# InternRobotics/InternNav

Hardware: NVIDIA H100
Metric: InternVLA-N1 policy-steps/sec (batch RGB-D+text->action) (higher is better)
Workload: dtype bf16

## Files before the change

### include/n1b200.h

```cpp
#ifndef N1B200_H_
#define N1B200_H_

#include <stddef.h>
#include <stdint.h>

#ifdef __cplusplus
extern "C" {
#endif

typedef struct n1_ctx* n1_handle;

enum {
  N1_OK = 0,
  N1_ERR_UNKNOWN = -1,
  N1_ERR_ARG = -2,
  N1_ERR_CUDA = -3,
  N1_ERR_NO_DEVICE = -4,
  N1_ERR_TMA = -5,
  N1_ERR_WEIGHT = -6,
  N1_ERR_WORKSPACE = -7,
  N1_ERR_KV_PAGES = -8
};

enum { N1_F32 = 0, N1_BF16 = 1 };

typedef struct {
  const char* name;
  const void* data;
  int32_t dtype;
  int32_t ndim;
  int64_t shape[4];
} n1_tensor_desc;

typedef struct {
  int32_t token_dim;
  int32_t heads;
  int32_t layers;
  int32_t predict_size;
  int32_t memory_size;
  int32_t vlm_token_dim;
  int32_t n_query;
} n1_s1_dims;

typedef struct {
  int32_t token_dim;
  int32_t heads;
  int32_t layers;
  int32_t predict_size;
  int32_t memory_size;
  int32_t depth_frames;
  int32_t goal_slots;
  int32_t ddpm_steps;
} n1_navdp_policy_dims;

const char* n1_version(void);
int n1_device_ok(int device);
int n1_create(n1_handle* out, int device);
void n1_destroy(n1_handle h);
const char* n1_last_error(void);

int n1_s1_load(n1_handle h, const n1_s1_dims* dims, const n1_tensor_desc* tensors, int n, void* stream);

enum { N1_OP_RGBD = 1, N1_OP_GOAL = 2, N1_OP_DENOISE = 3 };
size_t n1_workspace_bytes(n1_handle h, int op, int B, int Ns, int T);

int n1_rgbd_encode(n1_handle h, void* ws, size_t ws_bytes, const float* rgb, const float* depth, void* out_bf16, int B,
                   void* stream);

int n1_goal_compress(n1_handle h, void* ws, size_t ws_bytes, const void* latents_bf16, void* goal_bf16, int B,
                     void* stream);

int n1_navdp_eps(n1_handle h, void* ws, size_t ws_bytes, const float* x_t, const int32_t* timesteps, int t_scalar,
                 const void* goal_bf16, const void* rgbd_bf16, float* eps, int B, int Ns, int T, void* stream);

int n1_navdp_sample(n1_handle h, void* ws, size_t ws_bytes, const void* goal_bf16, const void* rgbd_bf16,
                    const float* x_init, const float* step_noise, float* traj_out, int B, int Ns, int T, int K,
                    void* stream);

int n1_navdp_policy_load(n1_handle h, const n1_navdp_policy_dims* dims, const n1_tensor_desc* tensors, int n, void* stream);
int n1_navdp_critic(n1_handle h, void* ws, size_t ws_bytes, const float* traj, const void* rgbd_bf16, float* critic, int B,
                    int Ns, int T, void* stream);
int n1_ddpm_tables(int K, float* out_host );

typedef struct {
  int32_t v_depth, v_hidden, v_heads, v_inter, v_patch, v_tpatch, v_merge, v_window, v_out;
  int32_t n_fullatt, fullatt[16];
  int32_t layers, hidden, heads, kv_heads, head_dim, inter, vocab;
  float rms_eps, rope_theta;
  int32_t mrope[3];
  int32_t n_query;
} n1_s2_dims;

typedef struct n1_vit_plan_s* n1_vit_plan;
typedef struct n1_llm_plan_s* n1_llm_plan;
typedef struct n1_kv_pool_s* n1_kv_pool;

int n1_s2_load(n1_handle h, const n1_s2_dims* dims, const n1_tensor_desc* tensors, int n, void* stream);
int n1_s2_has_latent_queries(n1_handle h);
int n1_s2_has_lm_head(n1_handle h);

int n1_vit_plan_create(n1_handle h, const int32_t* grid_thw_host, int n_img, n1_vit_plan* out, void* stream);
void n1_vit_plan_destroy(n1_vit_plan p);
int64_t n1_vit_plan_patches(n1_vit_plan p);
int n1_llm_plan_create(n1_handle h, const int32_t* input_ids_host, const int32_t* lens_host, int B,
                       const int32_t* grid_thw_host, int n_img, int max_new_tokens, n1_kv_pool pool,
                       const int32_t* reused_host, const int32_t* slots_host, n1_llm_plan* out, void* stream);
void n1_llm_plan_destroy(n1_llm_plan p);
int64_t n1_llm_plan_tokens(n1_llm_plan p);
int64_t n1_llm_plan_image_tokens(n1_llm_plan p);
int n1_llm_plan_positions(n1_llm_plan p, int32_t* pos3_host, int32_t* delta_host);

size_t n1_vit_workspace_bytes(n1_handle h, n1_vit_plan p);
size_t n1_llm_workspace_bytes(n1_handle h, n1_llm_plan p);

int n1_qwen_vit(n1_handle h, n1_vit_plan p, void* ws, size_t ws_bytes, const void* pixels_bf16, void* out_bf16,
                int64_t out_rows, const int32_t* dst_rows_host, int64_t n_rows, void* stream);
int n1_llm_prefill(n1_handle h, n1_llm_plan p, void* ws, size_t ws_bytes, const void* image_feats_bf16,
                   void* latents_bf16, void* stream);

int n1_llm_generate(n1_handle h, n1_llm_plan p, void* ws, size_t ws_bytes, const void* feats_bf16, int64_t feat_rows,
                    const int32_t* image_rows_host, int64_t n_rows, const int32_t* eos_ids_host, int n_eos, int32_t pad_id,
                    int32_t* tokens_host, int32_t* lens_host, void* latents_bf16, int32_t* passes_host, void* stream);

int n1_kv_pool_create(n1_handle h, int slots, int capacity, n1_kv_pool* out);
void n1_kv_pool_destroy(n1_kv_pool p);
size_t n1_kv_pool_bytes(n1_kv_pool p);
int n1_kv_pool_valid(n1_kv_pool p, int slot);
int n1_kv_pool_create_paged(n1_handle h, int slots, int pages, int max_tokens_per_slot, n1_kv_pool* out);
int n1_kv_pool_release(n1_kv_pool p, int slot);
int n1_kv_pool_free_pages(n1_kv_pool p);
int n1_kv_pool_slot_pages(n1_kv_pool p, int slot);
int n1_kv_pool_read(n1_kv_pool p, int layer, int slot, int row, int n, void* k_out, void* v_out, void* stream);
int n1_image_digest(const void* pixels_bf16, int64_t cols, const int64_t* row_off_dev, int n_img, uint64_t* digest_dev,
                    void* stream);

int n1_rope_index(const int32_t* input_ids_host, int len, const int32_t* grid_thw_host, int n_img, int merge,
                  int32_t* pos3_host , int32_t* delta_host);
int n1_plan_rows_host(const int32_t* input_ids_host, const int32_t* lens_host, int B, const int32_t* grid_thw_host,
                      int n_img, int merge, int vocab, int n_query, int max_new_tokens, int pool_slots, int pool_capacity,
                      const int32_t* reused_host, const int32_t* slots_host, int cap_rows, int32_t* n_rows,
                      int32_t* cu_host, int32_t* kind_host, int32_t* src_host, int32_t* dest_host, int32_t* k_len_host);
typedef struct n1_kv_pages_s* n1_kv_pages;
int n1_kv_pages_create(int slots, int max_tokens_per_slot, int pages, n1_kv_pages* out);
void n1_kv_pages_destroy(n1_kv_pages a);
int n1_kv_pages_prepare(n1_kv_pages a, int B, const int32_t* slots_host, const int32_t* keep_rows_host,
                        const int32_t* need_rows_host, int32_t* changed_host);
int n1_kv_pages_trim(n1_kv_pages a, int slot, int rows);
int n1_kv_pages_table(n1_kv_pages a, int32_t* table_host, int32_t* held_host, int32_t* free_host);
int n1_vit_window_index(const int32_t* grid_thw_host, int n_img, int merge, int window, int32_t* window_index_host,
                        int32_t* cu_window_host, int32_t* n_cu, int32_t* pos_hw_host );

typedef struct n1_resize_plan_s* n1_resize_plan;
int n1_resize_plan_create(int in_h, int in_w, int out_h, int out_w, n1_resize_plan* out, void* stream);
void n1_resize_plan_destroy(n1_resize_plan p);
size_t n1_resize_workspace_bytes(n1_resize_plan p, int n_frames, int is_float);
int n1_resize_rgb_u8(n1_resize_plan p, const void* src_u8, int n_frames, void* dst_f32, void* dst_u8, void* ws,
                     size_t ws_bytes, void* stream);
int n1_resize_f32(n1_resize_plan p, const void* src_f32, int n_frames, float mul, float clip_max, void* dst_f32,
                  void* ws, size_t ws_bytes, void* stream);
int n1_resize_coeffs(int in_size, int out_size, int capacity_k, int32_t* bounds_host, double* weights_host,
                     int32_t* fixed_host, int32_t* ksize);

typedef struct {
  const void* src_u8;
  int32_t h, w;
  int64_t row0;
} n1_vl_image;
size_t n1_vl_patchify_workspace_bytes(int n_img);
int n1_vl_patchify(const n1_vl_image* images_host, int n_img, const void* lut_bf16, void* out_bf16, int64_t n_rows,
                   void* ws, size_t ws_bytes, void* stream);

size_t n1_rgb_tokens_workspace_bytes(n1_handle h, int B);
int n1_rgb_tokens(n1_handle h, void* ws, size_t ws_bytes, const float* rgb, void* mem_bf16, int B, void* stream);
int n1_s2_set_latent_queries(n1_handle h, const void* latent_queries_bf16, void* stream);
size_t n1_s2_train_workspace_bytes(n1_handle h, n1_llm_plan plan);
int n1_s2_train_forward(n1_handle h, n1_llm_plan plan, void* ws, size_t ws_bytes, const void* image_feats_bf16,
                        void* states_bf16, void* stream);
int n1_s2_train_backward(n1_handle h, n1_llm_plan plan, void* ws, size_t ws_bytes, const void* grad_states_bf16,
                         void* grad_latent_queries_f32, void* stream);
int n1_op_transpose(const void* in_bf16, int rows, int cols, int ld_in, void* out_bf16, int ld_out, int rows_pad, void* stream);
int n1_op_colsum(const void* a_bf16, const void* b_bf16_or_null, int rows, int cols, int ld_a, int ld_b, void* out_f32,
                 int accumulate, void* stream);
int n1_op_norm_bwd(const void* dy_bf16, int ld_dy, const void* x_bf16, int ld_x, const void* w_f32, const void* residual_grad,
                   int ld_rg, void* dx_bf16, int ld_dx, void* dw_f32, void* db_f32, int rows, int D, float eps, int rms,
                   int accumulate, void* stream);
int n1_op_act_fwd(const void* pre_bf16, void* out_bf16, int64_t n, int act, void* stream);
int n1_op_act_bwd(const void* pre_bf16, const void* dy_bf16, void* out_bf16, int64_t n, int act, void* stream);
int n1_op_swiglu_bwd(const void* pre_bf16, const void* dact_bf16, void* dpre_bf16, int64_t rows, int inter, void* stream);
int n1_op_rope_transposed(void* x_bf16, int ld, const void* cos_sin_f32x2, int64_t rows, int heads, int head_dim, void* stream);
int n1_op_attention_bwd(const void* q, const void* k, const void* v, const void* o, const void* dout, void* dq, void* dk_f32,
                        void* dv_f32, int ldq, int ldk, int ldv, int ldo, int lddo, int lddq, int heads_q, int heads_kv,
                        int head_dim, int batch, int seq_q, int seq_k, const void* cu_q, const void* cu_k, int max_seq_q,
                        int kv_div, int causal, float scale, const void* k_len, int k_slot, void* stream);
int n1_traj_to_actions(const void* traj_f32, int B, int Ns, int T, double turn_angle_rad, double step_size, int lookahead,
                       int max_actions, int cap, int32_t* ids, int32_t* count, double* mean_path, void* stream);
int n1_traj_mean_path(const void* traj_f32, int B, int Ns, int T, double* mean_path, void* stream);
int n1_op_sgemm(const void* A_f32, int lda, int trans_a, const void* B_f32, int ldb, int trans_b, void* C_f32, int ldc, int M,
                int N, int K, int accumulate, void* stream);
size_t n1_op_wgrad_workspace_bytes(int M, int No, int Ko);
int n1_op_wgrad(const void* dy_bf16, int ld_dy, const void* x_bf16, int ld_x, int M, int No, int Ko, void* out_f32,
                int accumulate, void* ws, size_t ws_bytes, void* stream);
int n1_op_scale_cols(const void* x_bf16, int ld_x, const void* gamma_f32, const void* add_bf16_or_null, int ld_add,
                     void* out_bf16, int ld_out, int64_t rows, int cols, void* stream);
int n1_op_patchify_depth(const void* img_f32, void* out_bf16, int n_img, int ldk, void* stream);
int n1_op_adamw(void* master_f32, void* working_bf16_or_null, const void* grad_f32, void* m_f32, void* v_f32, int64_t n,
                float lr, float beta1, float beta2, float eps, float weight_decay, int step, void* stream);

void n1_prof_enable(int on);
void n1_prof_add(int64_t gemm_launches, int64_t total_launches);
int n1_prof_read(double* gemm_ms, double* gemm_flops, int64_t* gemm_launches, int64_t* total_launches);
int n1_prof_read_shapes(int32_t* mnk, int64_t* count, double* ms, int cap);

int n1_op_gemm(const void* A_bf16, int lda, const void* W_bf16, int ldw, void* out, int ldo, int M, int N, int K,
               const float* bias, const float* gamma, const void* residual_bf16, int ldr, int act, int out_fp32,
               void* stream);
int n1_op_ff_block(const void* x_bf16, int ldx, const float* ln_w, const float* ln_b, float eps, const void* w1_bf16,
                   const float* b1, const void* w2_bf16, const float* b2, void* out_bf16, int ldo, int M, void* stream);
int n1_op_dec_sa_block(void* x_bf16, int ldx, const float* ln_w, const float* ln_b, float eps, const void* w_qkv_bf16,
                       const float* b_qkv, const void* w_o_bf16, const float* b_o, int B, int Ns, int T, int causal,
                       void* stream);
int n1_op_dec_ca_block(void* x_bf16, int ldx, const float* ln_w, const float* ln_b, float eps, const void* w_q_bf16,
                       const float* b_q, const void* w_o_bf16, const float* b_o, const void* kv_bf16, int ldkv, int mtok,
                       int B, int Ns, int T, void* stream);
int n1_op_layernorm(const void* x_bf16, int ldx, void* y_bf16, int ldy, const float* w, const float* b, int rows, int D,
                    float eps, int rms, void* stream);
int n1_op_mod_norm(const void* x_bf16, int ldx, const float* w, const void* mod_bf16, int ld_mod, int rows_per_group,
                   const void* res_bf16, int ldr, void* out_bf16, int ldo, int64_t rows, int D, float eps, int mode,
                   void* stream);
int n1_op_add(const void* a_bf16, const void* b_bf16, void* out_bf16, int64_t n, void* stream);
int n1_op_action_embed(const float* lat, const float* w, const float* b, const float* pos, void* out_bf16, int64_t rows,
                       int T, int D, void* stream);
int n1_op_cfg_euler(const void* pred_bf16, int ld, int64_t n, int cfg, float scale, float dt, float* lat, void* stream);
int n1_op_attention(const void* q, const void* k, const void* v, void* o, int ldq, int ldk, int ldv, int ldo, int heads_q,
                    int heads_kv, int head_dim, int batch, int seq_q, int seq_k, const int32_t* cu_q,
                    const int32_t* cu_k, int max_seq_q, int kv_div, int causal, float scale, void* stream);

int n1_op_attention_ex(const void* q, const void* k, const void* v, void* o, int ldq, int ldk, int ldv, int ldo, int heads_q,
                       int heads_kv, int head_dim, int batch, const int32_t* cu_seqlens, int max_seq, int64_t total_rows,
                       int causal, float scale, int* used_tcgen05, void* stream);

int n1_op_attention_cache(const void* q, int ldq, int64_t q_rows, const void* k, const void* v, int ldkv, int64_t kv_rows,
                          void* o, int ldo, const int32_t* cu_q, const int32_t* ctx, const int32_t* row0, int batch,
                          int max_chunk, int heads_q, int heads_kv, float scale, void* stream);
int n1_op_attention_cache_paged(const void* q, int ldq, int64_t q_rows, const void* k, const void* v, int ldkv,
                                int64_t kv_rows, void* o, int ldo, const int32_t* cu_q, const int32_t* ctx,
                                const int32_t* row0, const int32_t* pages, int batch, int max_chunk, int heads_q,
                                int heads_kv, float scale, void* stream);

#ifdef __cplusplus
}
#endif
#endif
```

### internnav_b200/_lib.py

```python
import ctypes
import os
import threading

import torch

_HERE = os.path.dirname(os.path.abspath(__file__))
LIB_PATH = os.path.join(_HERE, "libn1b200.so")

_lib = None
_lock = threading.Lock()

c_void_p, c_int, c_size_t, c_float, c_char_p = (
    ctypes.c_void_p, ctypes.c_int, ctypes.c_size_t, ctypes.c_float, ctypes.c_char_p)
c_int32, c_int64, c_double = ctypes.c_int32, ctypes.c_int64, ctypes.c_double
i32p = ctypes.POINTER(c_int32)


class N1Error(RuntimeError):
    def __init__(self, code, msg):
        super().__init__("n1b200 error %d: %s" % (code, msg))
        self.code = code


class TensorDesc(ctypes.Structure):
    _fields_ = [("name", c_char_p), ("data", c_void_p), ("dtype", ctypes.c_int32), ("ndim", ctypes.c_int32),
                ("shape", ctypes.c_int64 * 4)]


class S1Dims(ctypes.Structure):
    _fields_ = [("token_dim", ctypes.c_int32), ("heads", ctypes.c_int32), ("layers", ctypes.c_int32),
                ("predict_size", ctypes.c_int32), ("memory_size", ctypes.c_int32),
                ("vlm_token_dim", ctypes.c_int32), ("n_query", ctypes.c_int32)]


class NavdpPolicyDims(ctypes.Structure):
    _fields_ = [(n, ctypes.c_int32) for n in ("token_dim", "heads", "layers", "predict_size", "memory_size", "depth_frames",
                                              "goal_slots", "ddpm_steps")]


class S2Dims(ctypes.Structure):
    _fields_ = [(n, ctypes.c_int32) for n in ("v_depth", "v_hidden", "v_heads", "v_inter", "v_patch", "v_tpatch",
                                              "v_merge", "v_window", "v_out", "n_fullatt")] + \
               [("fullatt", ctypes.c_int32 * 16)] + \
               [(n, ctypes.c_int32) for n in ("layers", "hidden", "heads", "kv_heads", "head_dim", "inter", "vocab")] + \
               [("rms_eps", ctypes.c_float), ("rope_theta", ctypes.c_float), ("mrope", ctypes.c_int32 * 3),
                ("n_query", ctypes.c_int32)]


class VlImage(ctypes.Structure):
    _fields_ = [("src_u8", c_void_p), ("h", ctypes.c_int32), ("w", ctypes.c_int32), ("row0", ctypes.c_int64)]


SYMBOLS = {
    "n1_version": (c_char_p, []),
    "n1_device_ok": (c_int, [c_int]),
    "n1_create": (c_int, [ctypes.POINTER(c_void_p), c_int]),
    "n1_destroy": (None, [c_void_p]),
    "n1_last_error": (c_char_p, []),
    "n1_s1_load": (c_int, [c_void_p, ctypes.POINTER(S1Dims), ctypes.POINTER(TensorDesc), c_int, c_void_p]),
    "n1_workspace_bytes": (c_size_t, [c_void_p, c_int, c_int, c_int, c_int]),
    "n1_rgbd_encode": (c_int, [c_void_p, c_void_p, c_size_t, c_void_p, c_void_p, c_void_p, c_int, c_void_p]),
    "n1_goal_compress": (c_int, [c_void_p, c_void_p, c_size_t, c_void_p, c_void_p, c_int, c_void_p]),
    "n1_navdp_eps": (c_int, [c_void_p, c_void_p, c_size_t, c_void_p, c_void_p, c_int, c_void_p, c_void_p, c_void_p,
                             c_int, c_int, c_int, c_void_p]),
    "n1_navdp_sample": (c_int, [c_void_p, c_void_p, c_size_t, c_void_p, c_void_p, c_void_p, c_void_p, c_void_p,
                                c_int, c_int, c_int, c_int, c_void_p]),
    "n1_navdp_policy_load": (c_int, [c_void_p, ctypes.POINTER(NavdpPolicyDims), ctypes.POINTER(TensorDesc), c_int,
                                     c_void_p]),
    "n1_navdp_critic": (c_int, [c_void_p, c_void_p, c_size_t, c_void_p, c_void_p, c_void_p, c_int, c_int, c_int, c_void_p]),
    "n1_ddpm_tables": (c_int, [c_int, ctypes.POINTER(c_float)]),
    "n1_s2_load": (c_int, [c_void_p, ctypes.POINTER(S2Dims), ctypes.POINTER(TensorDesc), c_int, c_void_p]),
    "n1_s2_has_latent_queries": (c_int, [c_void_p]),
    "n1_s2_has_lm_head": (c_int, [c_void_p]),
    "n1_vit_plan_create": (c_int, [c_void_p, i32p, c_int, ctypes.POINTER(c_void_p), c_void_p]),
    "n1_vit_plan_destroy": (None, [c_void_p]),
    "n1_vit_plan_patches": (c_int64, [c_void_p]),
    "n1_llm_plan_create": (c_int, [c_void_p, i32p, i32p, c_int, i32p, c_int, c_int, c_void_p, i32p, i32p,
                                   ctypes.POINTER(c_void_p), c_void_p]),
    "n1_llm_plan_destroy": (None, [c_void_p]),
    "n1_llm_plan_tokens": (c_int64, [c_void_p]),
    "n1_llm_plan_image_tokens": (c_int64, [c_void_p]),
    "n1_llm_plan_positions": (c_int, [c_void_p, i32p, i32p]),
    "n1_vit_workspace_bytes": (c_size_t, [c_void_p, c_void_p]),
    "n1_llm_workspace_bytes": (c_size_t, [c_void_p, c_void_p]),
    "n1_qwen_vit": (c_int, [c_void_p, c_void_p, c_void_p, c_size_t, c_void_p, c_void_p, c_int64, i32p, c_int64, c_void_p]),
    "n1_llm_prefill": (c_int, [c_void_p, c_void_p, c_void_p, c_size_t, c_void_p, c_void_p, c_void_p]),
    "n1_llm_generate": (c_int, [c_void_p, c_void_p, c_void_p, c_size_t, c_void_p, c_int64, i32p, c_int64, i32p, c_int,
                                c_int32, i32p, i32p, c_void_p, i32p, c_void_p]),
    "n1_kv_pool_create": (c_int, [c_void_p, c_int, c_int, ctypes.POINTER(c_void_p)]),
    "n1_kv_pool_destroy": (None, [c_void_p]),
    "n1_kv_pool_bytes": (c_size_t, [c_void_p]),
    "n1_kv_pool_valid": (c_int, [c_void_p, c_int]),
    "n1_kv_pool_read": (c_int, [c_void_p, c_int, c_int, c_int, c_int, c_void_p, c_void_p, c_void_p]),
    "n1_kv_pool_create_paged": (c_int, [c_void_p, c_int, c_int, c_int, ctypes.POINTER(c_void_p)]),
    "n1_kv_pool_release": (c_int, [c_void_p, c_int]),
    "n1_kv_pool_free_pages": (c_int, [c_void_p]),
    "n1_kv_pool_slot_pages": (c_int, [c_void_p, c_int]),
    "n1_kv_pages_create": (c_int, [c_int, c_int, c_int, ctypes.POINTER(c_void_p)]),
    "n1_kv_pages_destroy": (None, [c_void_p]),
    "n1_kv_pages_prepare": (c_int, [c_void_p, c_int, i32p, i32p, i32p, i32p]),
    "n1_kv_pages_trim": (c_int, [c_void_p, c_int, c_int]),
    "n1_kv_pages_table": (c_int, [c_void_p, i32p, i32p, i32p]),
    "n1_image_digest": (c_int, [c_void_p, c_int64, c_void_p, c_int, c_void_p, c_void_p]),
    "n1_rope_index": (c_int, [i32p, c_int, i32p, c_int, c_int, i32p, i32p]),
    "n1_plan_rows_host": (c_int, [i32p, i32p, c_int, i32p, c_int, c_int, c_int, c_int, c_int, c_int, c_int, i32p, i32p,
                                  c_int, i32p, i32p, i32p, i32p, i32p, i32p]),
    "n1_vit_window_index": (c_int, [i32p, c_int, c_int, c_int, i32p, i32p, i32p, i32p]),
    "n1_s2_set_latent_queries": (c_int, [c_void_p, c_void_p, c_void_p]),
    "n1_s2_train_workspace_bytes": (c_size_t, [c_void_p, c_void_p]),
    "n1_s2_train_forward": (c_int, [c_void_p, c_void_p, c_void_p, c_size_t, c_void_p, c_void_p, c_void_p]),
    "n1_s2_train_backward": (c_int, [c_void_p, c_void_p, c_void_p, c_size_t, c_void_p, c_void_p, c_void_p]),
    "n1_resize_plan_create": (c_int, [c_int, c_int, c_int, c_int, ctypes.POINTER(c_void_p), c_void_p]),
    "n1_resize_plan_destroy": (None, [c_void_p]),
    "n1_resize_workspace_bytes": (c_size_t, [c_void_p, c_int, c_int]),
    "n1_resize_rgb_u8": (c_int, [c_void_p, c_void_p, c_int, c_void_p, c_void_p, c_void_p, c_size_t, c_void_p]),
    "n1_resize_f32": (c_int, [c_void_p, c_void_p, c_int, c_float, c_float, c_void_p, c_void_p, c_size_t, c_void_p]),
    "n1_resize_coeffs": (c_int, [c_int, c_int, c_int, i32p, ctypes.POINTER(c_double), i32p, i32p]),
    "n1_vl_patchify_workspace_bytes": (c_size_t, [c_int]),
    "n1_vl_patchify": (c_int, [ctypes.POINTER(VlImage), c_int, c_void_p, c_void_p, c_int64, c_void_p, c_size_t, c_void_p]),
    "n1_op_transpose": (c_int, [c_void_p, c_int, c_int, c_int, c_void_p, c_int, c_int, c_void_p]),
    "n1_op_colsum": (c_int, [c_void_p, c_void_p, c_int, c_int, c_int, c_int, c_void_p, c_int, c_void_p]),
    "n1_op_norm_bwd": (c_int, [c_void_p, c_int, c_void_p, c_int, c_void_p, c_void_p, c_int, c_void_p, c_int, c_void_p,
                               c_void_p, c_int, c_int, c_float, c_int, c_int, c_void_p]),
    "n1_op_act_fwd": (c_int, [c_void_p, c_void_p, c_int64, c_int, c_void_p]),
    "n1_op_act_bwd": (c_int, [c_void_p, c_void_p, c_void_p, c_int64, c_int, c_void_p]),
    "n1_op_swiglu_bwd": (c_int, [c_void_p, c_void_p, c_void_p, c_int64, c_int, c_void_p]),
    "n1_op_rope_transposed": (c_int, [c_void_p, c_int, c_void_p, c_int64, c_int, c_int, c_void_p]),
    "n1_op_attention_bwd": (c_int, [c_void_p] * 8 + [c_int] * 12 + [c_void_p, c_void_p, c_int, c_int, c_int, c_float,
                                                                   c_void_p, c_int, c_void_p]),
    "n1_op_sgemm": (c_int, [c_void_p, c_int, c_int, c_void_p, c_int, c_int, c_void_p, c_int, c_int, c_int, c_int, c_int,
                            c_void_p]),
    "n1_op_wgrad_workspace_bytes": (c_size_t, [c_int, c_int, c_int]),
    "n1_op_wgrad": (c_int, [c_void_p, c_int, c_void_p, c_int, c_int, c_int, c_int, c_void_p, c_int, c_void_p, c_size_t,
                            c_void_p]),
    "n1_op_scale_cols": (c_int, [c_void_p, c_int, c_void_p, c_void_p, c_int, c_void_p, c_int, c_int64, c_int, c_void_p]),
    "n1_op_patchify_depth": (c_int, [c_void_p, c_void_p, c_int, c_int, c_void_p]),
    "n1_op_adamw": (c_int, [c_void_p, c_void_p, c_void_p, c_void_p, c_void_p, c_int64, c_float, c_float, c_float, c_float,
                            c_float, c_int, c_void_p]),
    "n1_rgb_tokens_workspace_bytes": (c_size_t, [c_void_p, c_int]),
    "n1_rgb_tokens": (c_int, [c_void_p, c_void_p, c_size_t, c_void_p, c_void_p, c_int, c_void_p]),
    "n1_traj_to_actions": (c_int, [c_void_p, c_int, c_int, c_int, ctypes.c_double, ctypes.c_double, c_int, c_int, c_int,
                                   c_void_p, c_void_p, c_void_p, c_void_p]),
    "n1_traj_mean_path": (c_int, [c_void_p, c_int, c_int, c_int, c_void_p, c_void_p]),
    "n1_prof_enable": (None, [c_int]),
    "n1_prof_add": (None, [ctypes.c_int64, ctypes.c_int64]),
    "n1_prof_read": (c_int, [ctypes.POINTER(ctypes.c_double), ctypes.POINTER(ctypes.c_double),
                             ctypes.POINTER(ctypes.c_int64), ctypes.POINTER(ctypes.c_int64)]),
    "n1_prof_read_shapes": (c_int, [ctypes.POINTER(ctypes.c_int32), ctypes.POINTER(ctypes.c_int64),
                                    ctypes.POINTER(ctypes.c_double), c_int]),
    "n1_op_gemm": (c_int, [c_void_p, c_int, c_void_p, c_int, c_void_p, c_int, c_int, c_int, c_int, c_void_p, c_void_p,
                           c_void_p, c_int, c_int, c_int, c_void_p]),
    "n1_op_ff_block": (c_int, [c_void_p, c_int, c_void_p, c_void_p, c_float, c_void_p, c_void_p, c_void_p, c_void_p, c_void_p,
                               c_int, c_int, c_void_p]),
    "n1_op_dec_sa_block": (c_int, [c_void_p, c_int, c_void_p, c_void_p, c_float, c_void_p, c_void_p, c_void_p, c_void_p,
                                   c_int, c_int, c_int, c_int, c_void_p]),
    "n1_op_dec_ca_block": (c_int, [c_void_p, c_int, c_void_p, c_void_p, c_float, c_void_p, c_void_p, c_void_p, c_void_p,
                                   c_void_p, c_int, c_int, c_int, c_int, c_int, c_void_p]),
    "n1_op_layernorm": (c_int, [c_void_p, c_int, c_void_p, c_int, c_void_p, c_void_p, c_int, c_int, c_float, c_int,
                                c_void_p]),
    "n1_op_mod_norm": (c_int, [c_void_p, c_int, c_void_p, c_void_p, c_int, c_int, c_void_p, c_int, c_void_p, c_int,
                               ctypes.c_int64, c_int, c_float, c_int, c_void_p]),
    "n1_op_add": (c_int, [c_void_p, c_void_p, c_void_p, ctypes.c_int64, c_void_p]),
    "n1_op_action_embed": (c_int, [c_void_p, c_void_p, c_void_p, c_void_p, c_void_p, ctypes.c_int64, c_int, c_int, c_void_p]),
    "n1_op_cfg_euler": (c_int, [c_void_p, c_int, ctypes.c_int64, c_int, c_float, c_float, c_void_p, c_void_p]),
    "n1_op_attention_ex": (c_int, [c_void_p, c_void_p, c_void_p, c_void_p, c_int, c_int, c_int, c_int, c_int, c_int, c_int,
                                   c_int, c_void_p, c_int, ctypes.c_int64, c_int, c_float, ctypes.POINTER(c_int), c_void_p]),
    "n1_op_attention": (c_int, [c_void_p, c_void_p, c_void_p, c_void_p, c_int, c_int, c_int, c_int, c_int, c_int, c_int,
                                c_int, c_int, c_int, c_void_p, c_void_p, c_int, c_int, c_int, c_float, c_void_p]),
    "n1_op_attention_cache": (c_int, [c_void_p, c_int, ctypes.c_int64, c_void_p, c_void_p, c_int, ctypes.c_int64, c_void_p,
                                      c_int, c_void_p, c_void_p, c_void_p, c_int, c_int, c_int, c_int, c_float, c_void_p]),
    "n1_op_attention_cache_paged": (c_int, [c_void_p, c_int, ctypes.c_int64, c_void_p, c_void_p, c_int, ctypes.c_int64,
                                            c_void_p, c_int, c_void_p, c_void_p, c_void_p, c_void_p, c_int, c_int, c_int,
                                            c_int, c_float, c_void_p]),
}

OP_RGBD, OP_GOAL, OP_DENOISE = 1, 2, 3
ACT_NONE, ACT_GELU, ACT_RELU, ACT_SWIGLU, ACT_GELU_TANH, ACT_SILU = 0, 1, 2, 3, 4, 5


def lib():
    global _lib
    with _lock:
        if _lib is None:
            if not os.path.exists(LIB_PATH):
                raise ImportError(
                    "%s not found: build it with `python -m internnav_b200.build` (nvcc, sm_90a). "
                    "There is no CPU/PyTorch fallback for the n1b200 hot path." % LIB_PATH)
            L = ctypes.CDLL(LIB_PATH)
            for name, (res, args) in SYMBOLS.items():
                fn = getattr(L, name)
                fn.restype = res
                fn.argtypes = args
            _lib = L
    return _lib


def check(code):
    if code != 0:
        raise N1Error(code, lib().n1_last_error().decode("utf-8", "replace"))


def ptr(t):
    if t is None:
        return None
    assert t.is_cuda and t.is_contiguous(), "n1b200 takes contiguous CUDA tensors"
    return c_void_p(t.data_ptr())


def stream_ptr():
    return c_void_p(torch.cuda.current_stream().cuda_stream)


def dtype_code(t):
    if t.dtype == torch.float32:
        return 0
    if t.dtype == torch.bfloat16:
        return 1
    raise TypeError("n1b200 takes fp32 or bf16 tensors, got %s" % t.dtype)


def prof_enable(on):
    lib().n1_prof_enable(1 if on else 0)


def prof_read():
    a, b = ctypes.c_double(), ctypes.c_double()
    c, d = ctypes.c_int64(), ctypes.c_int64()
    check(lib().n1_prof_read(ctypes.byref(a), ctypes.byref(b), ctypes.byref(c), ctypes.byref(d)))
    return {"gemm_ms": a.value, "gemm_flops": b.value, "gemm_launches": c.value, "total_launches": d.value}


def prof_read_shapes(cap=256):
    mnk = (ctypes.c_int32 * (3 * cap))()
    cnt = (ctypes.c_int64 * cap)()
    ms = (ctypes.c_double * cap)()
    n = lib().n1_prof_read_shapes(mnk, cnt, ms, cap)
    if n < 0:
        raise N1Error(n, lib().n1_last_error().decode("utf-8", "replace"))
    return [dict(M=mnk[3 * i], N=mnk[3 * i + 1], K=mnk[3 * i + 2], count=int(cnt[i]), ms=float(ms[i])) for i in range(n)]


def gemm(a, w, bias=None, gamma=None, residual=None, act=ACT_NONE, out_fp32=False, out=None):
    assert a.dtype == torch.bfloat16 and w.dtype == torch.bfloat16 and a.dim() == 2 and w.dim() == 2
    M, K = a.shape
    N = w.shape[0]
    n_out = N // 2 if act == ACT_SWIGLU else N
    if out is None:
        out = torch.empty(M, n_out, device=a.device, dtype=torch.float32 if out_fp32 else torch.bfloat16)
    assert a.stride(1) == 1 and w.stride(1) == 1 and out.stride(1) == 1
    check(lib().n1_op_gemm(c_void_p(a.data_ptr()), a.stride(0), c_void_p(w.data_ptr()), w.stride(0),
                           c_void_p(out.data_ptr()), out.stride(0), M, N, K, ptr(bias), ptr(gamma),
                           c_void_p(residual.data_ptr()) if residual is not None else None,
                           residual.stride(0) if residual is not None else 0, act, 1 if out_fp32 else 0, stream_ptr()))
    return out


def gemm_tile(a, w, out, bias=None, gamma=None, residual=None, act=ACT_NONE, rows_per_group=0, group_stride=0,
              group_offset=0, row_add=None, tile_n=0):
    fn = lib().n1_test_gemm
    fn.restype = c_int
    fn.argtypes = [c_void_p, c_int, c_void_p, c_int, c_void_p, c_int, c_int, c_int, c_int, c_void_p, c_void_p, c_void_p,
                   c_int, c_int, c_int, c_int, c_int, c_int, c_void_p, c_int, c_void_p]
    vp = lambda t: c_void_p(t.data_ptr()) if t is not None else None
    check(fn(vp(a), a.stride(0), vp(w), w.stride(0), vp(out), out.stride(0), a.shape[0], w.shape[0], a.shape[1],
             vp(bias), vp(gamma), vp(residual), residual.stride(0) if residual is not None else 0, act,
             1 if out.dtype == torch.float32 else 0, rows_per_group, group_stride, group_offset, vp(row_add), tile_n,
             stream_ptr()))
    return out


def layernorm(x, w, b=None, eps=1e-5, rms=False, out=None):
    assert x.dtype == torch.bfloat16 and x.dim() == 2 and x.stride(1) == 1
    y = torch.empty(x.shape, device=x.device, dtype=torch.bfloat16) if out is None else out
    assert y.stride(1) == 1 and y.shape == x.shape
    check(lib().n1_op_layernorm(c_void_p(x.data_ptr()), x.stride(0), c_void_p(y.data_ptr()), y.stride(0), ptr(w), ptr(b), x.shape[0],
                                x.shape[1], eps, 1 if rms else 0, stream_ptr()))
    return y


MOD_RMS_SCALE, MOD_LN_SCALE, MOD_GATED_RESIDUAL = 0, 1, 2


def mod_norm(x, w, mod, rows_per_group, eps, mode, residual=None, out=None):
    assert x.dtype == torch.bfloat16 and x.dim() == 2 and x.stride(1) == 1
    if out is None:
        out = torch.empty(x.shape, device=x.device, dtype=torch.bfloat16)
    if mod is not None:
        assert mod.dtype == torch.bfloat16 and mod.stride(1) == 1 and mod.shape[1] == x.shape[1]
        assert mod.shape[0] * rows_per_group == x.shape[0]
    check(lib().n1_op_mod_norm(c_void_p(x.data_ptr()), x.stride(0), ptr(w), c_void_p(mod.data_ptr()) if mod is not None else None,
                               mod.stride(0) if mod is not None else 0, int(rows_per_group),
                               c_void_p(residual.data_ptr()) if residual is not None else None,
                               residual.stride(0) if residual is not None else 0, c_void_p(out.data_ptr()), out.stride(0),
                               x.shape[0], x.shape[1], float(eps), int(mode), stream_ptr()))
    return out


def add(a, b, out=None):
    assert a.dtype == torch.bfloat16 and b.dtype == torch.bfloat16 and a.is_contiguous() and b.is_contiguous() and a.shape == b.shape
    if out is None:
        out = torch.empty_like(a)
    check(lib().n1_op_add(ptr(a), ptr(b), ptr(out), a.numel(), stream_ptr()))
    return out


def action_embed(lat, w, b, pos, out=None):
    assert lat.dtype == torch.float32 and lat.is_contiguous() and lat.shape[-1] == 3
    rows, (T, D) = lat.numel() // 3, pos.shape
    if out is None:
        out = torch.empty(rows, D, device=lat.device, dtype=torch.bfloat16)
    check(lib().n1_op_action_embed(ptr(lat), ptr(w), ptr(b), ptr(pos), ptr(out), rows, T, D, stream_ptr()))
    return out


def cfg_euler(pred, n, cfg, scale, dt, lat):
    assert pred.dtype == torch.bfloat16 and pred.stride(1) == 1 and lat.dtype == torch.float32 and lat.is_contiguous()
    assert pred.shape[0] == (2 if cfg else 1) * n and lat.numel() == 3 * n
    check(lib().n1_op_cfg_euler(c_void_p(pred.data_ptr()), pred.stride(0), n, 1 if cfg else 0, float(scale), float(dt), ptr(lat),
                                stream_ptr()))
    return lat


def attention(q, k, v, heads_q, heads_kv, head_dim, batch, seq_q, seq_k, cu_q=None, cu_k=None, max_seq_q=0, kv_div=1,
              causal=False, scale=None):
    assert q.dtype == torch.bfloat16 and q.stride(1) == 1 and k.stride(1) == 1 and v.stride(1) == 1
    o = torch.empty(q.shape[0], heads_q * head_dim, device=q.device, dtype=torch.bfloat16)
    if scale is None:
        scale = head_dim ** -0.5
    check(lib().n1_op_attention(c_void_p(q.data_ptr()), c_void_p(k.data_ptr()), c_void_p(v.data_ptr()), ptr(o),
                                q.stride(0), k.stride(0), v.stride(0), o.stride(0), heads_q, heads_kv, head_dim, batch,
                                seq_q, seq_k, ptr(cu_q), ptr(cu_k), max_seq_q, kv_div, 1 if causal else 0,
                                float(scale), stream_ptr()))
    return o


def attention_varlen(q, k, v, heads_q, heads_kv, head_dim, cu_seqlens, max_seq, causal=True, scale=None):
    assert q.dtype == torch.bfloat16 and q.stride(1) == 1 and k.stride(1) == 1 and v.stride(1) == 1
    o = torch.empty(q.shape[0], heads_q * head_dim, device=q.device, dtype=torch.bfloat16)
    if scale is None:
        scale = head_dim ** -0.5
    used = c_int(0)
    check(lib().n1_op_attention_ex(c_void_p(q.data_ptr()), c_void_p(k.data_ptr()), c_void_p(v.data_ptr()), ptr(o),
                                   q.stride(0), k.stride(0), v.stride(0), o.stride(0), heads_q, heads_kv, head_dim,
                                   cu_seqlens.numel() - 1, ptr(cu_seqlens), int(max_seq), q.shape[0], 1 if causal else 0,
                                   float(scale), ctypes.byref(used), stream_ptr()))
    return o, bool(used.value)


ATTN_KERNELS = {1: "short", 2: "generic", 3: "wgmma"}


def attention_test(q, k, v, o, heads_q, heads_kv, head_dim, batch, seq_q=0, seq_k=0, cu_q=None, cu_k=None, max_seq_q=0,
                   kv_div=1, causal=False, scale=None, k_len=None, k_slot=0, k_row0=None, total_rows=0):
    for t in (q, k, v, o):
        assert t.dtype == torch.bfloat16 and t.stride(1) == 1
    fn = lib().n1_test_attention
    fn.restype = c_int
    fn.argtypes = [c_void_p, c_void_p, c_void_p, c_void_p, c_int, c_int, c_int, c_int, c_int, c_int, c_int, c_int, c_int,
                   c_int, c_void_p, c_void_p, c_int, c_int, c_int, ctypes.c_float, c_void_p, c_int, c_void_p,
                   ctypes.c_int64, c_void_p, c_void_p]
    route = (c_int * 4)()
    vp = lambda t: c_void_p(t.data_ptr())
    check(fn(vp(q), vp(k), vp(v), vp(o), q.stride(0), k.stride(0), v.stride(0), o.stride(0), heads_q, heads_kv, head_dim,
             batch, seq_q, seq_k, ptr(cu_q), ptr(cu_k), int(max_seq_q), kv_div, 1 if causal else 0,
             float(head_dim ** -0.5 if scale is None else scale), ptr(k_len), int(k_slot), ptr(k_row0), int(total_rows),
             route, stream_ptr()))
    return ATTN_KERNELS[route[0]], route[1], route[2], route[3]


def attention_paged_test(q, k, v, o, heads_q, heads_kv, batch, seq_q, k_len, k_row0, pages, k_slot=0, scale=None):
    for t in (q, k, v, o):
        assert t.dtype == torch.bfloat16 and t.stride(1) == 1
    assert k.stride(0) == v.stride(0)
    fn = lib().n1_test_attention_paged
    fn.restype = c_int
    fn.argtypes = [c_void_p, c_void_p, c_void_p, c_void_p, c_int, c_int, c_int, c_int, c_int, c_int, c_int, c_void_p, c_int,
                   c_void_p, c_void_p, ctypes.c_float, c_void_p]
    vp = lambda t: c_void_p(t.data_ptr())
    check(fn(vp(q), vp(k), vp(v), vp(o), q.stride(0), k.stride(0), o.stride(0), heads_q, heads_kv, batch, seq_q,
             ptr(k_len), int(k_slot), ptr(k_row0), ptr(pages), float(128 ** -0.5 if scale is None else scale),
             stream_ptr()))


def attention_cache(q, k, v, heads_q, heads_kv, cu_q, ctx, row0, max_chunk, scale=None, out=None, pages=None):
    assert q.dtype == k.dtype == v.dtype == torch.bfloat16 and q.stride(1) == 1 and k.stride(1) == 1 and v.stride(1) == 1
    assert k.stride(0) == v.stride(0) and k.shape[0] == v.shape[0]
    for t in (cu_q, ctx, row0):
        assert t.dtype == torch.int32 and t.is_cuda and t.is_contiguous()
    o = torch.empty(q.shape[0], heads_q * 128, device=q.device, dtype=torch.bfloat16) if out is None else out
    assert o.dtype == torch.bfloat16 and o.stride(1) == 1 and o.is_cuda
    scale = float(128 ** -0.5 if scale is None else scale)
    if pages is None:
        check(lib().n1_op_attention_cache(c_void_p(q.data_ptr()), q.stride(0), q.shape[0], c_void_p(k.data_ptr()),
                                          c_void_p(v.data_ptr()), k.stride(0), k.shape[0], c_void_p(o.data_ptr()), o.stride(0), ptr(cu_q),
                                          ptr(ctx), ptr(row0), cu_q.numel() - 1, int(max_chunk), heads_q, heads_kv,
                                          scale, stream_ptr()))
        return o
    assert pages.dtype == torch.int32 and pages.is_cuda and pages.is_contiguous()
    check(lib().n1_op_attention_cache_paged(c_void_p(q.data_ptr()), q.stride(0), q.shape[0], c_void_p(k.data_ptr()),
                                            c_void_p(v.data_ptr()), k.stride(0), k.shape[0], c_void_p(o.data_ptr()),
                                            o.stride(0), ptr(cu_q), ptr(ctx), ptr(row0), ptr(pages), cu_q.numel() - 1,
                                            int(max_chunk), heads_q, heads_kv, scale, stream_ptr()))
    return o


def ff_block(x, ln_w, ln_b, w1, b1, w2, b2, eps=1e-5, out=None):
    assert x.dtype == torch.bfloat16 and x.shape[1] == 384 and w1.shape == (1536, 384) and w2.shape == (384, 1536)
    assert w1.is_contiguous() and w2.is_contiguous() and x.stride(1) == 1
    if out is None:
        out = torch.empty(x.shape[0], 384, device=x.device, dtype=torch.bfloat16)
    check(lib().n1_op_ff_block(c_void_p(x.data_ptr()), x.stride(0), ptr(ln_w), ptr(ln_b), eps, ptr(w1), ptr(b1), ptr(w2),
                               ptr(b2), c_void_p(out.data_ptr()), out.stride(0), x.shape[0], stream_ptr()))
    return out


def dec_sa_block(x, ln_w, ln_b, w_qkv, b_qkv, w_o, b_o, B, Ns, T, causal=True, eps=1e-5):
    assert x.dtype == torch.bfloat16 and x.shape == (B * Ns * T, 384) and x.stride(1) == 1
    assert w_qkv.shape == (1152, 384) and w_o.shape == (384, 384)
    check(lib().n1_op_dec_sa_block(c_void_p(x.data_ptr()), x.stride(0), ptr(ln_w), ptr(ln_b), float(eps), ptr(w_qkv),
                                   ptr(b_qkv), ptr(w_o), ptr(b_o), B, Ns, T, 1 if causal else 0, stream_ptr()))
    return x


def dec_ca_block(x, ln_w, ln_b, w_q, b_q, w_o, b_o, kv, mtok, B, Ns, T, eps=1e-5):
    assert x.dtype == torch.bfloat16 and x.shape == (B * Ns * T, 384) and x.stride(1) == 1
    assert w_q.shape == (384, 384) and w_o.shape == (384, 384) and kv.shape[0] == B * mtok and kv.stride(1) == 1
    check(lib().n1_op_dec_ca_block(c_void_p(x.data_ptr()), x.stride(0), ptr(ln_w), ptr(ln_b), float(eps), ptr(w_q), ptr(b_q),
                                   ptr(w_o), ptr(b_o), c_void_p(kv.data_ptr()), kv.stride(0), mtok, B, Ns, T, stream_ptr()))
    return x
```

### internnav_b200/csrc/api.cu

```cuda
#include <string.h>

#include <algorithm>
#include <string>
#include <vector>

#include "../../include/n1b200.h"
#include "n1_ops.h"
#include "resize.h"
#include "bwd_kernels.h"
#include "s1_model.h"
#include "s2_kernels.h"
#include "s2_model.h"
#include "weights.h"

using namespace n1;

struct n1_ctx {
  int device = 0;
  S1Model s1;
  S2Model s2;
};
struct n1_vit_plan_s {
  VitPlan* p;
};
struct n1_llm_plan_s {
  LlmPlan* p;
};
struct n1_kv_pool_s {
  KvPool* p;
};
struct n1_resize_plan_s {
  ResizePlan* p;
};
struct n1_kv_pages_s {
  PageAlloc a;
};

namespace {

thread_local std::string g_err;

template <typename F>
int guard(F&& f) {
  try {
    f();
    return N1_OK;
  } catch (const Error& e) {
    g_err = e.what();
    return e.code;
  } catch (const std::exception& e) {
    g_err = e.what();
    return N1_ERR_UNKNOWN;
  } catch (...) {
    g_err = "unknown error";
    return N1_ERR_UNKNOWN;
  }
}

void require_device(int device) {
  int n = 0;
  if (cudaGetDeviceCount(&n) != cudaSuccess || n <= 0) throw Error(N1_ERR_NO_DEVICE, "no CUDA device visible; n1b200 has no CPU fallback");
  if (device < 0 || device >= n) throw Error(N1_ERR_NO_DEVICE, "device index out of range");
  cudaDeviceProp p;
  N1_CUDA(cudaGetDeviceProperties(&p, device));
  if (p.major != 9) throw Error(N1_ERR_NO_DEVICE, std::string("device is sm_") + std::to_string(p.major) + std::to_string(p.minor) + "; n1b200 kernels are sm_90a only");
}

void use(n1_handle h) {
  if (!h) throw Error(N1_ERR_ARG, "null handle");
  N1_CUDA(cudaSetDevice(h->device));
}

WeightSource to_source(const n1_tensor_desc* t, int n) {
  WeightSource ws;
  for (int i = 0; i < n; ++i) {
    if (!t[i].name || !t[i].data) throw Error(N1_ERR_WEIGHT, "tensor descriptor with null name/data");
    SrcTensor s;
    s.data = t[i].data;
    s.dtype = t[i].dtype;
    if (s.dtype != N1_F32 && s.dtype != N1_BF16) throw Error(N1_ERR_WEIGHT, std::string("unsupported dtype for ") + t[i].name);
    for (int d = 0; d < t[i].ndim && d < 4; ++d) s.shape.push_back(t[i].shape[d]);
    ws.add(t[i].name, s);
  }
  return ws;
}

inline cudaStream_t S(void* s) { return static_cast<cudaStream_t>(s); }
inline const bf16* B16(const void* p) { return static_cast<const bf16*>(p); }
inline bf16* B16(void* p) { return static_cast<bf16*>(p); }

void check_rows(const char* fn, const void* pool, int64_t pool_rows, const int32_t* rows, int64_t n_rows, int64_t expect,
                bool distinct) {
  const std::string f(fn);
  if (expect == 0 && n_rows == 0) return;
  if (!rows) {
    if (n_rows != 0 || pool_rows != expect)
      throw Error(N1_ERR_ARG, f + ": without a row table n_rows must be 0 and the features " + std::to_string(expect) +
                                  " rows, got " + std::to_string(n_rows) + " and " + std::to_string(pool_rows));
    if (expect > 0 && !pool) throw Error(N1_ERR_ARG, f + ": null features");
    return;
  }
  if (!pool || pool_rows <= 0 || pool_rows > INT32_MAX) throw Error(N1_ERR_ARG, f + ": null feature pool or bad pool_rows");
  if (n_rows != expect)
    throw Error(N1_ERR_ARG, f + ": the row table has " + std::to_string(n_rows) + " entries, the plan needs " +
                                std::to_string(expect));
  std::vector<char> seen(distinct ? (size_t)pool_rows : 0, 0);
  for (int64_t i = 0; i < n_rows; ++i) {
    if (rows[i] < 0 || rows[i] >= pool_rows)
      throw Error(N1_ERR_ARG, f + ": row " + std::to_string(rows[i]) + " (entry " + std::to_string(i) +
                                  ") is outside the pool of " + std::to_string(pool_rows) + " rows");
    if (distinct && seen[rows[i]]++) throw Error(N1_ERR_ARG, f + ": row " + std::to_string(rows[i]) + " is written twice");
  }
}

}

extern "C" {

const char* n1_version(void) { return "n1b200 0.1 (sm_90a)"; }

const char* n1_last_error(void) { return g_err.c_str(); }

int n1_device_ok(int device) {
  try {
    require_device(device);
    return 1;
  } catch (const std::exception& e) {
    g_err = e.what();
    return 0;
  }
}

int n1_create(n1_handle* out, int device) {
  return guard([&] {
    if (!out) throw Error(N1_ERR_ARG, "null out pointer");
    require_device(device);
    N1_CUDA(cudaSetDevice(device));
    n1_ctx* c = new n1_ctx();
    c->device = device;
    *out = c;
  });
}

void n1_destroy(n1_handle h) {
  if (!h) return;
  cudaSetDevice(h->device);
  delete h;
}

int n1_s1_load(n1_handle h, const n1_s1_dims* d, const n1_tensor_desc* tensors, int n, void* stream) {
  return guard([&] {
    use(h);
    if (!d || !tensors || n <= 0) throw Error(N1_ERR_ARG, "n1_s1_load: null dims/tensors");
    S1Dims dims;
    dims.D = d->token_dim, dims.heads = d->heads, dims.layers = d->layers, dims.T = d->predict_size;
    dims.frames = d->memory_size, dims.vlm_dim = d->vlm_token_dim, dims.n_query = d->n_query;
    h->s1.load(to_source(tensors, n), dims, S(stream));
  });
}

int n1_navdp_policy_load(n1_handle h, const n1_navdp_policy_dims* d, const n1_tensor_desc* tensors, int n, void* stream) {
  return guard([&] {
    use(h);
    if (!d || !tensors || n <= 0) throw Error(N1_ERR_ARG, "n1_navdp_policy_load: null dims/tensors");
    S1Dims dims;
    dims.D = d->token_dim, dims.heads = d->heads, dims.layers = d->layers, dims.T = d->predict_size;
    dims.frames = d->memory_size, dims.frames_depth = d->depth_frames, dims.goal_slots = d->goal_slots;
    dims.ddpm_steps = d->ddpm_steps, dims.standalone = 1, dims.vlm_dim = 0, dims.n_query = 0;
    h->s1.load(to_source(tensors, n), dims, S(stream));
  });
}

int n1_navdp_critic(n1_handle h, void* ws, size_t ws_bytes, const float* traj, const void* rgbd, float* critic, int B, int Ns,
                    int T, void* stream) {
  return guard([&] {
    use(h);
    h->s1.navdp_critic(ws, ws_bytes, traj, B16(rgbd), critic, B, Ns, T, S(stream));
  });
}

size_t n1_workspace_bytes(n1_handle h, int op, int B, int Ns, int T) {
  size_t r = 0;
  guard([&] {
    if (!h) throw Error(N1_ERR_ARG, "null handle");
    switch (op) {
      case N1_OP_RGBD: r = h->s1.ws_rgbd(B); break;
      case N1_OP_GOAL: r = h->s1.ws_goal(B); break;
      case N1_OP_DENOISE: r = h->s1.ws_denoise(B, Ns, T); break;
      default: throw Error(N1_ERR_ARG, "unknown op");
    }
  });
  return r;
}

int n1_rgbd_encode(n1_handle h, void* ws, size_t ws_bytes, const float* rgb, const float* depth, void* out, int B,
                   void* stream) {
  return guard([&] {
    use(h);
    h->s1.rgbd_encode(ws, ws_bytes, rgb, depth, B16(out), B, S(stream));
  });
}

int n1_goal_compress(n1_handle h, void* ws, size_t ws_bytes, const void* latents, void* goal, int B, void* stream) {
  return guard([&] {
    use(h);
    h->s1.goal_compress(ws, ws_bytes, B16(latents), B16(goal), B, S(stream));
  });
}

int n1_navdp_eps(n1_handle h, void* ws, size_t ws_bytes, const float* x_t, const int32_t* timesteps, int t_scalar,
                 const void* goal, const void* rgbd, float* eps, int B, int Ns, int T, void* stream) {
  return guard([&] {
    use(h);
    h->s1.navdp_eps(ws, ws_bytes, x_t, timesteps, t_scalar, B16(goal), B16(rgbd), eps, B, Ns, T, S(stream));
  });
}

int n1_navdp_sample(n1_handle h, void* ws, size_t ws_bytes, const void* goal, const void* rgbd, const float* x_init,
                    const float* step_noise, float* traj_out, int B, int Ns, int T, int K, void* stream) {
  return guard([&] {
    use(h);
    h->s1.navdp_sample(ws, ws_bytes, B16(goal), B16(rgbd), x_init, step_noise, traj_out, B, Ns, T, K, S(stream));
  });
}

int n1_ddpm_tables(int K, float* out_host) {
  return guard([&] {
    if (K <= 0 || !out_host) throw Error(N1_ERR_ARG, "n1_ddpm_tables: bad arguments");
    std::vector<DdpmCoef> c;
    S1Model::ddpm_tables(K, c);
    for (int i = 0; i < K; ++i) {
      out_host[i * 5 + 0] = c[i].sqrt_one_minus_acp, out_host[i * 5 + 1] = c[i].inv_sqrt_acp;
      out_host[i * 5 + 2] = c[i].c0, out_host[i * 5 + 3] = c[i].c1, out_host[i * 5 + 4] = c[i].sigma;
    }
  });
}

int n1_s2_load(n1_handle h, const n1_s2_dims* d, const n1_tensor_desc* tensors, int n, void* stream) {
  return guard([&] {
    use(h);
    if (!d || !tensors || n <= 0) throw Error(N1_ERR_ARG, "n1_s2_load: null dims/tensors");
    S2Dims x;
    x.v_depth = d->v_depth, x.v_hidden = d->v_hidden, x.v_heads = d->v_heads, x.v_inter = d->v_inter;
    x.v_patch = d->v_patch, x.v_tpatch = d->v_tpatch, x.v_merge = d->v_merge, x.v_window = d->v_window, x.v_out = d->v_out;
    x.n_fullatt = d->n_fullatt;
    if (x.n_fullatt < 0 || x.n_fullatt > 16) throw Error(N1_ERR_ARG, "n_fullatt out of range");
    for (int i = 0; i < 16; ++i) x.fullatt[i] = d->fullatt[i];
    x.layers = d->layers, x.hidden = d->hidden, x.heads = d->heads, x.kv_heads = d->kv_heads, x.head_dim = d->head_dim;
    x.inter = d->inter, x.vocab = d->vocab, x.rms_eps = d->rms_eps, x.rope_theta = d->rope_theta;
    for (int i = 0; i < 3; ++i) x.mrope[i] = d->mrope[i];
    x.n_query = d->n_query;
    h->s2.load(to_source(tensors, n), x, S(stream));
  });
}

int n1_vit_plan_create(n1_handle h, const int32_t* grid, int n_img, n1_vit_plan* out, void* stream) {
  return guard([&] {
    use(h);
    if (!grid || n_img <= 0 || !out) throw Error(N1_ERR_ARG, "n1_vit_plan_create: bad arguments");
    n1_vit_plan_s* w = new n1_vit_plan_s();
    try {
      w->p = h->s2.make_vit_plan(grid, n_img, S(stream));
    } catch (...) {
      delete w;
      throw;
    }
    *out = w;
  });
}
void n1_vit_plan_destroy(n1_vit_plan p) {
  if (!p) return;
  delete p->p;
  delete p;
}
int64_t n1_vit_plan_patches(n1_vit_plan p) { return p ? p->p->host.n_patches : 0; }

int n1_llm_plan_create(n1_handle h, const int32_t* ids, const int32_t* lens, int B, const int32_t* grid, int n_img,
                       int max_new_tokens, n1_kv_pool pool, const int32_t* reused, const int32_t* slots, n1_llm_plan* out,
                       void* stream) {
  return guard([&] {
    use(h);
    if (!ids || !lens || B <= 0 || max_new_tokens < 0 || !out) throw Error(N1_ERR_ARG, "n1_llm_plan_create: bad arguments");
    n1_llm_plan_s* w = new n1_llm_plan_s();
    try {
      w->p = h->s2.make_llm_plan(ids, lens, B, grid, n_img, S(stream), max_new_tokens, reused, slots,
                                 pool ? pool->p : nullptr);
    } catch (...) {
      delete w;
      throw;
    }
    *out = w;
  });
}
void n1_llm_plan_destroy(n1_llm_plan p) {
  if (!p) return;
  delete p->p;
  delete p;
}
int64_t n1_llm_plan_tokens(n1_llm_plan p) { return p ? p->p->tokens : 0; }
int64_t n1_llm_plan_image_tokens(n1_llm_plan p) { return p ? p->p->n_image_tokens : 0; }
int n1_llm_plan_positions(n1_llm_plan p, int32_t* pos3, int32_t* delta) {
  return guard([&] {
    if (!p) throw Error(N1_ERR_ARG, "null plan");
    if (pos3) memcpy(pos3, p->p->h_pos3.data(), p->p->h_pos3.size() * sizeof(int32_t));
    if (delta) memcpy(delta, p->p->h_delta.data(), p->p->h_delta.size() * sizeof(int32_t));
  });
}

size_t n1_vit_workspace_bytes(n1_handle h, n1_vit_plan p) {
  size_t r = 0;
  guard([&] {
    if (!h || !p) throw Error(N1_ERR_ARG, "null handle/plan");
    r = h->s2.ws_vit(*p->p);
  });
  return r;
}
size_t n1_llm_workspace_bytes(n1_handle h, n1_llm_plan p) {
  size_t r = 0;
  guard([&] {
    if (!h || !p) throw Error(N1_ERR_ARG, "null handle/plan");
    r = p->p->max_new > 0 ? h->s2.ws_generate(*p->p) : h->s2.ws_llm(*p->p);
  });
  return r;
}

int n1_qwen_vit(n1_handle h, n1_vit_plan p, void* ws, size_t ws_bytes, const void* pixels, void* out, int64_t out_rows,
                const int32_t* dst_rows, int64_t n_rows, void* stream) {
  return guard([&] {
    if (!h || !p || !pixels) throw Error(N1_ERR_ARG, "n1_qwen_vit: null handle / plan / pixels");
    const VitPlan& vp = *p->p;
    const int unit = h->s2.dims.v_merge * h->s2.dims.v_merge;
    check_rows("n1_qwen_vit", out, out_rows, dst_rows, n_rows, vp.host.n_patches / unit, true);
    use(h);
    h->s2.vit_forward(vp, ws, ws_bytes, B16(pixels), B16(out), S(stream), dst_rows);
  });
}
int n1_llm_prefill(n1_handle h, n1_llm_plan p, void* ws, size_t ws_bytes, const void* image_feats, void* latents,
                   void* stream) {
  return guard([&] {
    use(h);
    if (!p) throw Error(N1_ERR_ARG, "null plan");
    h->s2.llm_prefill(*p->p, ws, ws_bytes, B16(image_feats), B16(latents), S(stream));
  });
}

int n1_s2_has_lm_head(n1_handle h) { return h && h->s2.has_lm_head() ? 1 : 0; }
int n1_s2_has_latent_queries(n1_handle h) { return h && h->s2.has_latent_queries() ? 1 : 0; }
int n1_llm_generate(n1_handle h, n1_llm_plan p, void* ws, size_t ws_bytes, const void* feats, int64_t feat_rows,
                    const int32_t* image_rows, int64_t n_rows, const int32_t* eos, int n_eos, int32_t pad_id,
                    int32_t* tokens, int32_t* lens, void* latents, int32_t* passes, void* stream) {
  return guard([&] {
    if (!h || !p) throw Error(N1_ERR_ARG, "n1_llm_generate: null handle / plan");
    if (n_eos < 0 || n_eos > 4 || (n_eos > 0 && !eos)) throw Error(N1_ERR_ARG, "n1_llm_generate: 0..4 eos ids");
    check_rows("n1_llm_generate", feats, feat_rows, image_rows, n_rows, p->p->n_image_tokens, false);
    use(h);
    GenResult r;
    r.tokens = tokens, r.lens = lens;
    h->s2.llm_generate(*p->p, ws, ws_bytes, B16(feats), eos, n_eos, pad_id, r, B16(latents), S(stream), image_rows);
    if (passes) *passes = r.steps;
  });
}

int n1_kv_pool_create(n1_handle h, int slots, int capacity, n1_kv_pool* out) {
  return guard([&] {
    use(h);
    if (!out || slots <= 0 || capacity <= 0) throw Error(N1_ERR_ARG, "n1_kv_pool_create: bad arguments");
    n1_kv_pool_s* w = new n1_kv_pool_s();
    try {
      w->p = h->s2.make_pool(slots, capacity);
    } catch (...) {
      delete w;
      throw;
    }
    *out = w;
  });
}
void n1_kv_pool_destroy(n1_kv_pool p) {
  if (!p) return;
  delete p->p;
  delete p;
}
int n1_kv_pool_create_paged(n1_handle h, int slots, int pages, int max_tokens_per_slot, n1_kv_pool* out) {
  return guard([&] {
    use(h);
    if (!out || slots <= 0 || pages <= 0 || max_tokens_per_slot <= 0)
      throw Error(N1_ERR_ARG, "n1_kv_pool_create_paged: bad arguments");
    n1_kv_pool_s* w = new n1_kv_pool_s();
    try {
      w->p = h->s2.make_paged_pool(slots, pages, max_tokens_per_slot);
    } catch (...) {
      delete w;
      throw;
    }
    *out = w;
  });
}
int n1_kv_pool_release(n1_kv_pool p, int slot) {
  return guard([&] {
    if (!p) throw Error(N1_ERR_ARG, "null pool");
    if (slot < 0 || slot >= p->p->slots) throw Error(N1_ERR_ARG, "n1_kv_pool_release: slot out of range");
    p->p->valid[slot] = 0;
    if (p->p->paged()) p->p->pages.trim(slot, 0);
  });
}
int n1_kv_pool_free_pages(n1_kv_pool p) {
  if (!p) return N1_ERR_ARG;
  return p->p->paged() ? p->p->pages.free_pages() : 0;
}
int n1_kv_pool_slot_pages(n1_kv_pool p, int slot) {
  if (!p || slot < 0 || slot >= p->p->slots) return N1_ERR_ARG;
  return p->p->paged() ? p->p->pages.held[slot] : 0;
}
size_t n1_kv_pool_bytes(n1_kv_pool p) { return p ? p->p->bytes() : 0; }
int n1_kv_pool_valid(n1_kv_pool p, int slot) {
  int r = 0;
  const int e = guard([&] {
    if (!p) throw Error(N1_ERR_ARG, "null pool");
    if (slot < 0 || slot >= p->p->slots) throw Error(N1_ERR_ARG, "n1_kv_pool_valid: slot out of range");
    r = p->p->valid[slot];
  });
  return e == N1_OK ? r : e;
}
int n1_kv_pool_read(n1_kv_pool p, int layer, int slot, int row, int n, void* k_out, void* v_out, void* stream) {
  return guard([&] {
    if (!p || !k_out || !v_out) throw Error(N1_ERR_ARG, "null pool / buffer");
    const KvPool& q = *p->p;
    if (layer < 0 || layer >= q.layers || slot < 0 || slot >= q.slots || row < 0 || n < 0 || row + n > q.cap)
      throw Error(N1_ERR_ARG, "n1_kv_pool_read: layer / slot / rows out of range");
    const long w = q.width;
    if (q.paged() && row + n > q.pages.held[slot] * kPageRows)
      throw Error(N1_ERR_ARG, "n1_kv_pool_read: rows past the " + std::to_string(q.pages.held[slot]) + " pages slot " +
                                  std::to_string(slot) + " holds");
    for (int r = row; r < row + n;) {
      const int run = q.paged() ? std::min(row + n, (r / kPageRows + 1) * kPageRows) - r : n;
      const long src = q.paged() ? (long)q.pages.table[(size_t)slot * q.pages.per_slot + r / kPageRows] * kPageRows +
                                       r % kPageRows
                                 : (long)slot * q.cap + r;
      const long off = layer * q.layer_stride + src * w, dst = (long)(r - row) * w;
      N1_CUDA(cudaMemcpyAsync(B16(k_out) + dst, q.k + off, (size_t)run * w * sizeof(bf16), cudaMemcpyDeviceToDevice,
                              S(stream)));
      N1_CUDA(cudaMemcpyAsync(B16(v_out) + dst, q.v + off, (size_t)run * w * sizeof(bf16), cudaMemcpyDeviceToDevice,
                              S(stream)));
      r += run;
    }
  });
}
int n1_image_digest(const void* pixels, int64_t cols, const int64_t* row_off, int n_img, uint64_t* digest, void* stream) {
  return guard([&] {
    if ((n_img > 0 && (!pixels || !row_off || !digest)) || n_img < 0 || cols <= 0)
      throw Error(N1_ERR_ARG, "n1_image_digest: bad arguments");
    image_digest(B16(pixels), cols, row_off, n_img, digest, S(stream));
  });
}

int n1_resize_plan_create(int in_h, int in_w, int out_h, int out_w, n1_resize_plan* out, void* stream) {
  return guard([&] {
    if (!out || in_h <= 0 || in_w <= 0 || out_h <= 0 || out_w <= 0) throw Error(N1_ERR_ARG, "n1_resize_plan_create: bad sizes");
    int dev = 0;
    if (cudaGetDevice(&dev) != cudaSuccess) throw Error(N1_ERR_NO_DEVICE, "no CUDA device visible; n1b200 has no CPU fallback");
    require_device(dev);
    n1_resize_plan_s* w = new n1_resize_plan_s();
    try {
      w->p = new ResizePlan(in_h, in_w, out_h, out_w, S(stream));
    } catch (...) {
      delete w;
      throw;
    }
    *out = w;
  });
}
void n1_resize_plan_destroy(n1_resize_plan p) {
  if (!p) return;
  delete p->p;
  delete p;
}
size_t n1_resize_workspace_bytes(n1_resize_plan p, int n, int is_float) {
  return p && n > 0 ? p->p->workspace_bytes(n, is_float ? 1 : 3, is_float != 0) : 0;
}
int n1_resize_rgb_u8(n1_resize_plan p, const void* src, int n, void* dst_f32, void* dst_u8, void* ws, size_t ws_bytes,
                     void* stream) {
  return guard([&] {
    if (!p) throw Error(N1_ERR_ARG, "null plan");
    if (ws_bytes < p->p->workspace_bytes(n, 3, false)) throw Error(N1_ERR_WORKSPACE, "n1_resize_rgb_u8: workspace too small");
    resize_rgb_u8(*p->p, static_cast<const uint8_t*>(src), n, static_cast<float*>(dst_f32), static_cast<uint8_t*>(dst_u8),
                  ws, S(stream));
  });
}
int n1_resize_f32(n1_resize_plan p, const void* src, int n, float mul, float clip_max, void* dst, void* ws,
                  size_t ws_bytes, void* stream) {
  return guard([&] {
    if (!p) throw Error(N1_ERR_ARG, "null plan");
    if (ws_bytes < p->p->workspace_bytes(n, 1, true)) throw Error(N1_ERR_WORKSPACE, "n1_resize_f32: workspace too small");
    resize_f32(*p->p, static_cast<const float*>(src), n, mul, clip_max, static_cast<float*>(dst), ws, S(stream));
  });
}
int n1_resize_coeffs(int in_size, int out_size, int capacity_k, int32_t* bounds, double* weights, int32_t* fixed,
                     int32_t* ksize) {
  return guard([&] {
    if (!bounds || !weights || !fixed || !ksize) throw Error(N1_ERR_ARG, "n1_resize_coeffs: null outputs");
    ResizeCoeffs c;
    resize_coeffs(in_size, out_size, c);
    if (c.ksize > capacity_k) throw Error(N1_ERR_ARG, "n1_resize_coeffs: capacity_k < " + std::to_string(c.ksize));
    *ksize = c.ksize;
    memcpy(bounds, c.bounds.data(), c.bounds.size() * sizeof(int32_t));
    memcpy(weights, c.weights.data(), c.weights.size() * sizeof(double));
    memcpy(fixed, c.fixed.data(), c.fixed.size() * sizeof(int32_t));
  });
}

static_assert(sizeof(n1_vl_image) == sizeof(VlImage) && offsetof(n1_vl_image, row0) == offsetof(VlImage, row0),
              "n1_vl_image and VlImage must share one layout");
size_t n1_vl_patchify_workspace_bytes(int n_img) { return vl_patchify_workspace_bytes(n_img); }
int n1_vl_patchify(const n1_vl_image* images, int n_img, const void* lut, void* out, int64_t n_rows, void* ws,
                   size_t ws_bytes, void* stream) {
  return guard([&] {
    if (!images || !lut || !out || !ws) throw Error(N1_ERR_ARG, "n1_vl_patchify: null arguments");
    if (ws_bytes < vl_patchify_workspace_bytes(n_img)) throw Error(N1_ERR_WORKSPACE, "n1_vl_patchify: workspace too small");
    vl_patchify(reinterpret_cast<const VlImage*>(images), n_img, B16(lut), B16(out), n_rows, ws, S(stream));
  });
}

size_t n1_rgb_tokens_workspace_bytes(n1_handle h, int B) {
  size_t r = 0;
  guard([&] {
    if (!h || B <= 0) throw Error(N1_ERR_ARG, "null handle / B <= 0");
    r = h->s1.ws_rgb_tokens(B);
  });
  return r;
}
int n1_rgb_tokens(n1_handle h, void* ws, size_t ws_bytes, const float* rgb, void* mem, int B, void* stream) {
  return guard([&] {
    use(h);
    h->s1.rgb_tokens(ws, ws_bytes, rgb, B16(mem), B, S(stream));
  });
}
int n1_s2_set_latent_queries(n1_handle h, const void* src, void* stream) {
  return guard([&] {
    use(h);
    h->s2.set_latent_queries(B16(src), S(stream));
  });
}
size_t n1_s2_train_workspace_bytes(n1_handle h, n1_llm_plan p) {
  size_t r = 0;
  guard([&] {
    if (!h || !p) throw Error(N1_ERR_ARG, "null handle/plan");
    r = h->s2.ws_train(*p->p);
  });
  return r;
}
int n1_s2_train_forward(n1_handle h, n1_llm_plan p, void* ws, size_t ws_bytes, const void* image_feats, void* states,
                        void* stream) {
  return guard([&] {
    use(h);
    if (!p) throw Error(N1_ERR_ARG, "null plan");
    h->s2.train_forward(*p->p, ws, ws_bytes, B16(image_feats), B16(states), S(stream));
  });
}
int n1_s2_train_backward(n1_handle h, n1_llm_plan p, void* ws, size_t ws_bytes, const void* grad_states, void* grad_latent,
                         void* stream) {
  return guard([&] {
    use(h);
    if (!p) throw Error(N1_ERR_ARG, "null plan");
    h->s2.train_backward(*p->p, ws, ws_bytes, B16(grad_states), static_cast<float*>(grad_latent), S(stream));
  });
}
int n1_op_transpose(const void* in, int rows, int cols, int ld_in, void* out, int ld_out, int rows_pad, void* stream) {
  return guard([&] { transpose_bf16(B16(in), rows, cols, ld_in, B16(out), ld_out, rows_pad, S(stream)); });
}
int n1_op_colsum(const void* a, const void* b, int rows, int cols, int ld_a, int ld_b, void* out, int accumulate, void* stream) {
  return guard([&] { colsum_bf16(B16(a), B16(b), rows, cols, ld_a, ld_b, static_cast<float*>(out), accumulate, S(stream)); });
}
int n1_op_norm_bwd(const void* dy, int ld_dy, const void* x, int ld_x, const void* w, const void* rg, int ld_rg, void* dx,
                   int ld_dx, void* dw, void* db, int rows, int D, float eps, int rms, int accumulate, void* stream) {
  return guard([&] {
    norm_bwd(B16(dy), ld_dy, B16(x), ld_x, static_cast<const float*>(w), B16(rg), ld_rg, B16(dx), ld_dx,
             static_cast<float*>(dw), static_cast<float*>(db), rows, D, eps, rms, accumulate, S(stream));
  });
}
int n1_op_act_fwd(const void* pre, void* out, int64_t n, int act, void* stream) {
  return guard([&] { act_fwd(B16(pre), B16(out), n, act, S(stream)); });
}
int n1_op_act_bwd(const void* pre, const void* dy, void* out, int64_t n, int act, void* stream) {
  return guard([&] { act_bwd(B16(pre), B16(dy), B16(out), n, act, S(stream)); });
}
int n1_op_swiglu_bwd(const void* pre, const void* dact, void* dpre, int64_t rows, int inter, void* stream) {
  return guard([&] { swiglu_bwd(B16(pre), B16(dact), B16(dpre), rows, inter, S(stream)); });
}
int n1_op_rope_transposed(void* x, int ld, const void* cs, int64_t rows, int heads, int head_dim, void* stream) {
  return guard([&] { rope_transposed(B16(x), ld, static_cast<const float2*>(cs), rows, heads, head_dim, S(stream)); });
}
int n1_op_attention_bwd(const void* q, const void* k, const void* v, const void* o, const void* dout, void* dq, void* dk,
                        void* dv, int ldq, int ldk, int ldv, int ldo, int lddo, int lddq, int heads_q, int heads_kv, int hd,
                        int batch, int seq_q, int seq_k, const void* cu_q, const void* cu_k, int max_seq_q, int kv_div,
                        int causal, float scale, const void* k_len, int k_slot, void* stream) {
  return guard([&] {
    AttnBwdParams p = {};
    p.f.q = B16(q), p.f.k = B16(k), p.f.v = B16(v), p.f.o = const_cast<bf16*>(B16(o));
    p.f.ldq = ldq, p.f.ldk = ldk, p.f.ldv = ldv, p.f.ldo = ldo;
    p.f.heads_q = heads_q, p.f.heads_kv = heads_kv, p.f.hd = hd, p.f.batch = batch, p.f.seq_q = seq_q, p.f.seq_k = seq_k;
    p.f.cu_q = static_cast<const int*>(cu_q), p.f.cu_k = static_cast<const int*>(cu_k), p.f.max_seq_q = max_seq_q;
    p.f.kv_div = kv_div, p.f.causal = causal, p.f.scale = scale;
    p.f.k_len = static_cast<const int*>(k_len), p.f.k_slot = k_slot;
    p.dout = B16(dout), p.lddo = lddo, p.dq = B16(dq), p.lddq = lddq;
    p.dk = static_cast<float*>(dk), p.dv = static_cast<float*>(dv);
    attention_bwd(p, S(stream));
  });
}
int n1_traj_to_actions(const void* traj, int B, int Ns, int T, double turn_angle_rad, double step_size, int lookahead,
                       int max_actions, int cap, int32_t* ids, int32_t* count, double* mean_path, void* stream) {
  return guard([&] {
    traj_to_actions(static_cast<const float*>(traj), B, Ns, T, turn_angle_rad, step_size, lookahead, max_actions, cap, ids,
                    count, mean_path, S(stream));
  });
}
int n1_traj_mean_path(const void* traj, int B, int Ns, int T, double* mean_path, void* stream) {
  return guard([&] { traj_mean_path(static_cast<const float*>(traj), B, Ns, T, mean_path, S(stream)); });
}
int n1_op_sgemm(const void* A, int lda, int trans_a, const void* B, int ldb, int trans_b, void* C, int ldc, int M, int N, int K,
                int accumulate, void* stream) {
  return guard([&] {
    sgemm_small(static_cast<const float*>(A), lda, trans_a, static_cast<const float*>(B), ldb, trans_b, static_cast<float*>(C),
                ldc, M, N, K, accumulate, S(stream));
  });
}
size_t n1_op_wgrad_workspace_bytes(int M, int No, int Ko) { return wgrad_tn_workspace_bytes(M, No, Ko); }
int n1_op_wgrad(const void* dy, int ld_dy, const void* x, int ld_x, int M, int No, int Ko, void* out, int accumulate, void* ws,
                size_t ws_bytes, void* stream) {
  return guard([&] {
    wgrad_tn(B16(dy), ld_dy, B16(x), ld_x, M, No, Ko, static_cast<float*>(out), accumulate, ws, ws_bytes, S(stream));
  });
}
int n1_op_scale_cols(const void* x, int ld_x, const void* gamma, const void* add, int ld_add, void* out, int ld_out,
                     int64_t rows, int cols, void* stream) {
  return guard([&] {
    scale_cols(B16(x), ld_x, static_cast<const float*>(gamma), B16(add), ld_add, B16(out), ld_out, rows, cols, S(stream));
  });
}
int n1_op_patchify_depth(const void* img, void* out, int n_img, int ldk, void* stream) {
  return guard([&] {
    if (!img || !out || n_img <= 0 || ldk < 196 || ldk % 8) throw Error(N1_ERR_ARG, "n1_op_patchify_depth: bad arguments");
    patchify_depth(static_cast<const float*>(img), B16(out), n_img, ldk, S(stream));
  });
}
int n1_op_adamw(void* master, void* working, const void* grad, void* m, void* v, int64_t n, float lr, float beta1,
                float beta2, float eps, float weight_decay, int step, void* stream) {
  return guard([&] {
    adamw_step(static_cast<float*>(master), B16(working), static_cast<const float*>(grad), static_cast<float*>(m),
               static_cast<float*>(v), n, lr, beta1, beta2, eps, weight_decay, step, S(stream));
  });
}

int n1_plan_rows_host(const int32_t* ids, const int32_t* lens, int B, const int32_t* grid, int n_img, int merge, int vocab,
                      int n_query, int max_new_tokens, int pool_slots, int pool_capacity, const int32_t* reused,
                      const int32_t* slots, int cap_rows, int32_t* n_rows, int32_t* cu, int32_t* kind, int32_t* src,
                      int32_t* dest, int32_t* k_len) {
  return guard([&] {
    if (!ids || !lens || B <= 0 || max_new_tokens < 1 || !n_rows || !cu || !kind || !src || !dest || !k_len ||
        (!reused) != (!slots))
      throw Error(N1_ERR_ARG, "n1_plan_rows_host: bad arguments");
    PlanArgs a;
    a.merge = merge, a.vocab = vocab, a.n_query = n_query, a.max_new = max_new_tokens;
    a.ctx = reused, a.slots = slots, a.pool_slots = pool_slots, a.pool_cap = pool_capacity;
    PlanRows r;
    plan_rows(ids, lens, B, grid, n_img, a, r);
    const int rows = r.cu.back();
    if (rows > cap_rows) throw Error(N1_ERR_ARG, "n1_plan_rows_host: cap_rows < " + std::to_string(rows));
    *n_rows = rows;
    std::copy(r.cu.begin(), r.cu.end(), cu);
    std::copy(r.kind.begin(), r.kind.end(), kind), std::copy(r.src.begin(), r.src.end(), src);
    std::copy(r.dest.begin(), r.dest.end(), dest), std::copy(r.len.begin(), r.len.end(), k_len);
  });
}
int n1_kv_pages_create(int slots, int max_tokens_per_slot, int pages, n1_kv_pages* out) {
  return guard([&] {
    if (!out || max_tokens_per_slot <= 0) throw Error(N1_ERR_ARG, "n1_kv_pages_create: bad arguments");
    n1_kv_pages_s* w = new n1_kv_pages_s();
    try {
      w->a.init(slots, (max_tokens_per_slot + kPageRows - 1) / kPageRows, pages);
    } catch (...) {
      delete w;
      throw;
    }
    *out = w;
  });
}
void n1_kv_pages_destroy(n1_kv_pages a) { delete a; }
int n1_kv_pages_prepare(n1_kv_pages a, int B, const int32_t* slots, const int32_t* keep_rows, const int32_t* need_rows,
                        int32_t* changed) {
  return guard([&] {
    if (!a || B <= 0 || !slots || !keep_rows || !need_rows) throw Error(N1_ERR_ARG, "n1_kv_pages_prepare: bad arguments");
    const std::pair<int, int> ch = a->a.prepare(B, slots, keep_rows, need_rows);
    if (changed) changed[0] = ch.first, changed[1] = ch.second;
  });
}
int n1_kv_pages_trim(n1_kv_pages a, int slot, int rows) {
  return guard([&] {
    if (!a) throw Error(N1_ERR_ARG, "null page allocator");
    a->a.trim(slot, rows);
  });
}
int n1_kv_pages_table(n1_kv_pages a, int32_t* table, int32_t* held, int32_t* free_list) {
  const int e = guard([&] {
    if (!a) throw Error(N1_ERR_ARG, "null page allocator");
    if (table) std::copy(a->a.table.begin(), a->a.table.end(), table);
    if (held) std::copy(a->a.held.begin(), a->a.held.end(), held);
    if (free_list) std::copy(a->a.free.begin(), a->a.free.end(), free_list);
  });
  return e == N1_OK ? a->a.free_pages() : e;
}
int n1_rope_index(const int32_t* ids, int len, const int32_t* grid, int n_img, int merge, int32_t* pos3,
                  int32_t* delta) {
  return guard([&] {
    if (!ids || len <= 0 || !pos3) throw Error(N1_ERR_ARG, "n1_rope_index: bad arguments");
    std::vector<int> p;
    int cursor = 0, d = 0;
    rope_index_one(ids, len, grid, n_img, merge, cursor, p, d);
    memcpy(pos3, p.data(), p.size() * sizeof(int32_t));
    if (delta) *delta = d;
  });
}
int n1_vit_window_index(const int32_t* grid, int n_img, int merge, int window, int32_t* widx, int32_t* cu, int32_t* n_cu,
                        int32_t* pos_hw) {
  return guard([&] {
    if (!grid || n_img <= 0) throw Error(N1_ERR_ARG, "n1_vit_window_index: bad arguments");
    VitIndex v;
    vit_index(grid, n_img, merge, window, v);
    if (widx) memcpy(widx, v.window_index.data(), v.window_index.size() * sizeof(int32_t));
    if (cu) memcpy(cu, v.cu_window.data(), v.cu_window.size() * sizeof(int32_t));
    if (n_cu) *n_cu = (int32_t)v.cu_window.size();
    if (pos_hw) memcpy(pos_hw, v.pos_hw.data(), v.pos_hw.size() * sizeof(int32_t));
  });
}

void n1_prof_enable(int on) { prof_enable(on != 0); }

void n1_prof_add(int64_t gemm_launches, int64_t total_launches) {
  prof_count_launch((int)(total_launches - gemm_launches));
  for (int64_t i = 0; i < gemm_launches; ++i) prof_count_gemm(0.0);
}

int n1_prof_read_shapes(int32_t* mnk, int64_t* count, double* ms, int cap) {
  int n = -1;
  guard([&] {
    if (!mnk || !count || !ms || cap <= 0) throw Error(N1_ERR_ARG, "n1_prof_read_shapes: bad arguments");
    n = prof_read_shapes(mnk, reinterpret_cast<long*>(count), ms, cap);
  });
  return n;
}

int n1_prof_read(double* gemm_ms, double* gemm_flops, int64_t* gemm_launches, int64_t* total_launches) {
  return guard([&] {
    ProfStats st = prof_read_and_reset();
    if (gemm_ms) *gemm_ms = st.gemm_ms;
    if (gemm_flops) *gemm_flops = st.gemm_flops;
    if (gemm_launches) *gemm_launches = st.gemm_launches;
    if (total_launches) *total_launches = st.total_launches;
  });
}

int n1_op_gemm(const void* A, int lda, const void* W, int ldw, void* out, int ldo, int M, int N, int K,
               const float* bias, const float* gamma, const void* residual, int ldr, int act, int out_fp32,
               void* stream) {
  return guard([&] {
    GemmEpilogue e;
    e.bias = bias, e.gamma = gamma, e.residual = B16(residual), e.ldr = ldr, e.act = act, e.out_fp32 = out_fp32;
    gemm_bf16(B16(A), lda, B16(W), ldw, out, ldo, M, N, K, e, S(stream));
  });
}

int n1_test_gemm(const void* A, int lda, const void* W, int ldw, void* out, int ldo, int M, int N, int K, const float* bias,
                 const float* gamma, const void* residual, int ldr, int act, int out_fp32, int rows_per_group,
                 int group_stride, int group_offset, const float* row_add, int tile_n, void* stream) {
  return guard([&] {
    GemmEpilogue e;
    e.bias = bias, e.gamma = gamma, e.residual = B16(residual), e.ldr = ldr, e.act = act, e.out_fp32 = out_fp32;
    e.rows_per_group = rows_per_group, e.group_stride = group_stride, e.group_offset = group_offset, e.row_add = row_add;
    gemm_bf16(B16(A), lda, B16(W), ldw, out, ldo, M, N, K, e, S(stream), tile_n);
  });
}

int n1_op_ff_block(const void* x, int ldx, const float* ln_w, const float* ln_b, float eps, const void* w1, const float* b1,
                   const void* w2, const float* b2, void* out, int ldo, int M, void* stream) {
  return guard([&] {
    ff_block_384(B16(x), ldx, ln_w, ln_b, eps, B16(w1), b1, B16(w2), b2, B16(out), ldo, M, S(stream));
  });
}

int n1_op_dec_sa_block(void* x, int ldx, const float* ln_w, const float* ln_b, float eps, const void* w_qkv,
                       const float* b_qkv, const void* w_o, const float* b_o, int B, int Ns, int T, int causal, void* stream) {
  return guard([&] {
    dec_sa_block(B16(x), ldx, ln_w, ln_b, eps, B16(w_qkv), b_qkv, B16(w_o), b_o, B, Ns, T, causal, S(stream));
  });
}
int n1_op_dec_ca_block(void* x, int ldx, const float* ln_w, const float* ln_b, float eps, const void* w_q, const float* b_q,
                       const void* w_o, const float* b_o, const void* kv, int ldkv, int mtok, int B, int Ns, int T,
                       void* stream) {
  return guard([&] {
    dec_ca_block(B16(x), ldx, ln_w, ln_b, eps, B16(w_q), b_q, B16(w_o), b_o, B16(kv), ldkv, mtok, B, Ns, T, S(stream));
  });
}

int n1_op_mod_norm(const void* x, int ldx, const float* w, const void* mod, int ld_mod, int rows_per_group, const void* res,
                   int ldr, void* out, int ldo, int64_t rows, int D, float eps, int mode, void* stream) {
  return guard([&] {
    mod_norm(B16(x), ldx, w, B16(mod), ld_mod, rows_per_group, B16(res), ldr, B16(out), ldo, rows, D, eps, mode, S(stream));
  });
}
int n1_op_add(const void* a, const void* b, void* out, int64_t n, void* stream) {
  return guard([&] { add_bf16(B16(a), B16(b), B16(out), n, S(stream)); });
}
int n1_op_action_embed(const float* lat, const float* w, const float* b, const float* pos, void* out, int64_t rows, int T, int D,
                       void* stream) {
  return guard([&] { action_embed(lat, w, b, pos, B16(out), rows, T, D, S(stream)); });
}
int n1_op_cfg_euler(const void* pred, int ld, int64_t n, int cfg, float scale, float dt, float* lat, void* stream) {
  return guard([&] { cfg_euler(B16(pred), ld, n, cfg, scale, dt, lat, S(stream)); });
}
int n1_op_layernorm(const void* x, int ldx, void* y, int ldy, const float* w, const float* b, int rows, int D, float eps,
                    int rms, void* stream) {
  return guard([&] { layernorm(B16(x), ldx, B16(y), ldy, w, b, rows, D, eps, rms, S(stream)); });
}

int n1_op_attention(const void* q, const void* k, const void* v, void* o, int ldq, int ldk, int ldv, int ldo, int heads_q,
                    int heads_kv, int head_dim, int batch, int seq_q, int seq_k, const int32_t* cu_q,
                    const int32_t* cu_k, int max_seq_q, int kv_div, int causal, float scale, void* stream) {
  return guard([&] {
    AttnParams p = {};
    p.q = B16(q), p.k = B16(k), p.v = B16(v), p.o = B16(o);
    p.ldq = ldq, p.ldk = ldk, p.ldv = ldv, p.ldo = ldo;
    p.heads_q = heads_q, p.heads_kv = heads_kv, p.hd = head_dim, p.batch = batch;
    p.seq_q = seq_q, p.seq_k = seq_k, p.cu_q = cu_q, p.cu_k = cu_k, p.max_seq_q = max_seq_q;
    p.kv_div = kv_div < 1 ? 1 : kv_div, p.causal = causal, p.scale = scale;
    attention(p, S(stream));
  });
}

int n1_op_attention_ex(const void* q, const void* k, const void* v, void* o, int ldq, int ldk, int ldv, int ldo, int heads_q,
                       int heads_kv, int head_dim, int batch, const int32_t* cu_seqlens, int max_seq, int64_t total_rows,
                       int causal, float scale, int* used_tcgen05, void* stream) {
  return guard([&] {
    AttnParams p = {};
    p.q = B16(q), p.k = B16(k), p.v = B16(v), p.o = B16(o);
    p.ldq = ldq, p.ldk = ldk, p.ldv = ldv, p.ldo = ldo;
    p.heads_q = heads_q, p.heads_kv = heads_kv, p.hd = head_dim, p.batch = batch;
    p.cu_q = p.cu_k = cu_seqlens, p.max_seq_q = max_seq, p.total_rows = total_rows;
    p.kv_div = 1, p.causal = causal, p.scale = scale;
    if (used_tcgen05) *used_tcgen05 = attention_uses_tc(p) ? 1 : 0;
    attention(p, S(stream));
  });
}

int n1_test_attention(const void* q, const void* k, const void* v, void* o, int ldq, int ldk, int ldv, int ldo, int heads_q,
                      int heads_kv, int head_dim, int batch, int seq_q, int seq_k, const int32_t* cu_q, const int32_t* cu_k,
                      int max_seq_q, int kv_div, int causal, float scale, const int32_t* k_len, int k_slot,
                      const int32_t* k_row0, int64_t total_rows, int* route, void* stream) {
  return guard([&] {
    if (!route) throw Error(N1_ERR_ARG, "n1_test_attention: null route");
    AttnParams p = {};
    p.q = B16(q), p.k = B16(k), p.v = B16(v), p.o = B16(o);
    p.ldq = ldq, p.ldk = ldk, p.ldv = ldv, p.ldo = ldo;
    p.heads_q = heads_q, p.heads_kv = heads_kv, p.hd = head_dim, p.batch = batch;
    p.seq_q = seq_q, p.seq_k = seq_k, p.cu_q = cu_q, p.cu_k = cu_k, p.max_seq_q = max_seq_q;
    p.kv_div = kv_div, p.causal = causal, p.scale = scale;
    p.k_len = k_len, p.k_slot = k_slot, p.k_row0 = k_row0, p.total_rows = total_rows;
    const AttnRoute r = attention_route(p);
    route[0] = r.kernel, route[1] = r.hd, route[2] = r.nkp, route[3] = r.group;
    attention(p, S(stream));
  });
}

int n1_op_attention_cache(const void* q, int ldq, int64_t q_rows, const void* k, const void* v, int ldkv, int64_t kv_rows,
                          void* o, int ldo, const int32_t* cu_q, const int32_t* ctx, const int32_t* row0, int batch,
                          int max_chunk, int heads_q, int heads_kv, float scale, void* stream) {
  return n1_op_attention_cache_paged(q, ldq, q_rows, k, v, ldkv, kv_rows, o, ldo, cu_q, ctx, row0, nullptr, batch,
                                     max_chunk, heads_q, heads_kv, scale, stream);
}
int n1_op_attention_cache_paged(const void* q, int ldq, int64_t q_rows, const void* k, const void* v, int ldkv,
                                int64_t kv_rows, void* o, int ldo, const int32_t* cu_q, const int32_t* ctx,
                                const int32_t* row0, const int32_t* pages, int batch, int max_chunk, int heads_q,
                                int heads_kv, float scale, void* stream) {
  return guard([&] {
    if (!q || !k || !v || !o || !cu_q || !ctx || !row0) throw Error(N1_ERR_ARG, "n1_op_attention_cache: null pointer");
    CacheAttnParams a = {};
    a.q = B16(q), a.ldq = ldq, a.q_rows = q_rows, a.k = B16(k), a.v = B16(v), a.ldkv = ldkv, a.kv_rows = kv_rows;
    a.o = B16(o), a.ldo = ldo, a.cu_q = cu_q, a.ctx = ctx, a.row0 = row0, a.pages = pages;
    a.batch = batch, a.max_chunk = max_chunk, a.heads_q = heads_q, a.heads_kv = heads_kv, a.scale = scale;
    attention_cache(a, S(stream));
  });
}

int n1_test_attention_paged(const void* q, const void* k, const void* v, void* o, int ldq, int ldkv, int ldo, int heads_q,
                            int heads_kv, int batch, int seq_q, const int32_t* k_len, int k_slot, const int32_t* k_row0,
                            const int32_t* pages, float scale, void* stream) {
  return guard([&] {
    if (!pages || !k_len) throw Error(N1_ERR_ARG, "n1_test_attention_paged: null page table / k_len");
    AttnParams p = {};
    p.q = B16(q), p.k = B16(k), p.v = B16(v), p.o = B16(o);
    p.ldq = ldq, p.ldk = p.ldv = ldkv, p.ldo = ldo;
    p.heads_q = heads_q, p.heads_kv = heads_kv, p.hd = 128, p.batch = batch, p.seq_q = seq_q;
    p.kv_div = 1, p.causal = 1, p.scale = scale;
    p.k_len = k_len, p.k_slot = k_slot, p.k_row0 = k_row0, p.k_pages = pages;
    attention(p, S(stream));
  });
}

}
```

### internnav_b200/csrc/dec_attn_block.cu

```cuda
#include <mutex>

#include "dec_tile.cuh"

namespace n1 {
namespace {

constexpr int D = 384, HD = 48, BM = 64;
constexpr int kABytes = BM * D * 2;
constexpr int kSlots = 2, kSlotBytes = D * 64 * 2;
constexpr int kKvRow = 112;
constexpr int kKvBytes = BM * kKvRow;
constexpr int kConsumerWarps = 8;
constexpr int kThreads = 32 * kConsumerWarps + 128;
constexpr int kSmem = 2 * kABytes + kSlots * kSlotBytes + 2 * 2 * kKvBytes + 256 + 1024;
static_assert(kSmem <= 232448, "dec_attn_block: shared memory budget (227 KB per block)");

struct DecAttnArgs {
  bf16* x;
  int ldx;
  const float* ln_w;
  const float* ln_b;
  float eps;
  const float* b_in;
  const float* b_o;
  const bf16* kv;
  int ldkv;
  int mtok;
  int Ns, T, tpt, tiles_per_env, tiles;
  int causal;
};

__device__ __forceinline__ void warpgroup_barrier(int g) { asm volatile("bar.sync %0, 128;" ::"r"(2 + g) : "memory"); }

template <bool kSelf>
__global__ void __launch_bounds__(kThreads, 1)
dec_attn_kernel(const __grid_constant__ CUtensorMap tmIn, const __grid_constant__ CUtensorMap tmO, const DecAttnArgs args) {
  constexpr int NP = kSelf ? 3 * HD : HD;
  constexpr int kHeadBytes = NP * 64 * 2;
  extern __shared__ uint8_t smem_raw[];
  uint8_t* smem = reinterpret_cast<uint8_t*>((reinterpret_cast<uintptr_t>(smem_raw) + 1023) & ~uintptr_t(1023));
  uint8_t* sA = smem;
  uint8_t* sO = smem + kABytes;
  uint8_t* sW = sO + kABytes;
  uint8_t* sKV = sW + kSlots * kSlotBytes;
  uint64_t* bars = reinterpret_cast<uint64_t*>(sKV + 4 * kKvBytes);
  uint64_t* full = bars;
  uint64_t* empty = bars + kSlots;

  const int warp = threadIdx.x >> 5, lane = threadIdx.x & 31;
  if (threadIdx.x == 0) {
    tma_prefetch_desc(&tmIn), tma_prefetch_desc(&tmO);
    for (int s = 0; s < kSlots; ++s) mbar_init(&full[s], 1), mbar_init(&empty[s], kConsumerWarps);
    fence_mbar_init();
  }
  __syncthreads();

  if (warp >= kConsumerWarps) {
    setmaxnreg_dec<kProducerRegs>();
    if (warp == kConsumerWarps && lane == 0) {
      Ring<kSlots> r;
      for (int t = blockIdx.x; t < args.tiles; t += gridDim.x) {
        for (int hp = 0; hp < 4; ++hp)
          for (int kb = 0; kb < D / 64; ++kb) {
            mbar_wait(&empty[r.slot], r.phase ^ 1);
            mbar_arrive_expect_tx(&full[r.slot], 2 * kHeadBytes);
            uint8_t* dst = sW + r.slot * kSlotBytes;
#pragma unroll
            for (int g = 0; g < 2; ++g) {
              const int h = 4 * g + hp;
#pragma unroll
              for (int part = 0; part < NP / HD; ++part)
                tma_load_2d(dst + g * kHeadBytes + part * HD * 128, &tmIn, &full[r.slot], kb * 64, part * D + h * HD);
            }
            r.advance();
          }
        for (int kb = 0; kb < D / 64; ++kb) {
          mbar_wait(&empty[r.slot], r.phase ^ 1);
          mbar_arrive_expect_tx(&full[r.slot], kSlotBytes);
          uint8_t* dst = sW + r.slot * kSlotBytes;
          tma_load_2d(dst, &tmO, &full[r.slot], kb * 64, 0);
          tma_load_2d(dst + kSlotBytes / 2, &tmO, &full[r.slot], kb * 64, 192);
          r.advance();
        }
      }
    }
  } else {
    setmaxnreg_inc<kConsumerRegs>();
    const int cw = warp;
    const int g = cw >> 2;
    const int wtid = threadIdx.x & 127;
    const int quad = lane & 3;
    const int r0 = (cw & 3) * 16 + (lane >> 2);
    uint8_t* sK = sKV + g * 2 * kKvBytes;
    uint8_t* sV = sK + kKvBytes;
    const float sl2 = 0.14433756729740643f * 1.4426950408889634f;
    Ring<kSlots> ring;
    for (int t = blockIdx.x; t < args.tiles; t += gridDim.x) {
      const int env = t / args.tiles_per_env;
      const int traj0 = (t - env * args.tiles_per_env) * args.tpt;
      const int ntraj = min(args.tpt, args.Ns - traj0);
      const long row0 = ((long)env * args.Ns + traj0) * args.T;
      const int nrows = ntraj * args.T;
      consumer_barrier();
      ln384_to_tile<false>(sA, args.x, args.ldx, row0, nrows, args.ln_w, args.ln_b, args.eps, cw, lane);
      fence_proxy_async_smem();
      consumer_barrier();

      for (int hp = 0; hp < 4; ++hp) {
        const int h = 4 * g + hp;
        warpgroup_barrier(g);
        if (!kSelf) {
          const bf16* kb0 = args.kv + (long)env * args.mtok * args.ldkv + h * HD;
          for (int c = wtid; c < 2 * BM * 6; c += 128) {
            const int v = c / (BM * 6), j = (c / 6) % BM, ch = c % 6;
            uint4 val = make_uint4(0u, 0u, 0u, 0u);
            if (j < args.mtok) val = __ldg(reinterpret_cast<const uint4*>(kb0 + (long)j * args.ldkv + v * D + ch * 8));
            *reinterpret_cast<uint4*>((v ? sV : sK) + j * kKvRow + ch * 16) = val;
          }
        }
        float acc[NP / 2];
        mma_k384(acc, sA, sW, full, empty, ring, kSlotBytes, g * kHeadBytes, lane, [] {});
        uint32_t qf[3][4];
#pragma unroll
        for (int j = 0; j < NP / 8; ++j) {
          const int part = j / 6, c = (j % 6) * 8 + quad * 2;
          const float2 b = __ldg(reinterpret_cast<const float2*>(args.b_in + part * D + h * HD + c));
          const uint32_t lo = pack_bf16(acc[4 * j] + b.x, acc[4 * j + 1] + b.y);
          const uint32_t hi = pack_bf16(acc[4 * j + 2] + b.x, acc[4 * j + 3] + b.y);
          if (part == 0) {
            qf[j >> 1][(j & 1) * 2] = lo, qf[j >> 1][(j & 1) * 2 + 1] = hi;
          } else {
            uint8_t* buf = part == 1 ? sK : sV;
            *reinterpret_cast<uint32_t*>(buf + r0 * kKvRow + c * 2) = lo;
            *reinterpret_cast<uint32_t*>(buf + (r0 + 8) * kKvRow + c * 2) = hi;
          }
        }
        warpgroup_barrier(g);
        int lo_key[2], hi_key[2];
#pragma unroll
        for (int r = 0; r < 2; ++r) {
          const int qi = r0 + 8 * r;
          if (kSelf) {
            lo_key[r] = qi / args.T * args.T;
            hi_key[r] = args.causal ? qi : lo_key[r] + args.T - 1;
          } else {
            lo_key[r] = 0, hi_key[r] = args.mtok - 1;
          }
        }
        float o[6][4], inv0, inv1;
        attn_hd48_16rows<4>(qf, sK, sV, kKvRow, lo_key, hi_key, sl2, lane, o, inv0, inv1);
#pragma unroll
        for (int i = 0; i < 6; ++i) {
          const int col = h * HD + i * 8 + quad * 2;
          *reinterpret_cast<uint32_t*>(sO + sw128_offset(r0, col)) = pack_bf16(o[i][0] * inv0, o[i][1] * inv0);
          *reinterpret_cast<uint32_t*>(sO + sw128_offset(r0 + 8, col)) = pack_bf16(o[i][2] * inv1, o[i][3] * inv1);
        }
      }
      fence_proxy_async_smem();
      consumer_barrier();
      float y[96] = {};
      mma_k384(y, sO, sW, full, empty, ring, kSlotBytes, g * (kSlotBytes / 2), lane, [] {});
      residual_epilogue_192<false>(y, args.x, args.ldx, args.x, args.ldx, args.b_o, row0, nrows, g, r0, quad);
    }
  }
}

template <bool kSelf>
void launch_dec_attn(const bf16* w_in, const bf16* w_o, const DecAttnArgs& a, long rows, cudaStream_t stream) {
  static std::once_flag once;
  std::call_once(once, [] { cudaFuncSetAttribute(dec_attn_kernel<kSelf>, cudaFuncAttributeMaxDynamicSharedMemorySize, kSmem); });
  const CUtensorMap tmIn = tma_map_2d(w_in, kSelf ? 3 * D : D, D, D, HD, 64, true);
  const CUtensorMap tmO = tma_map_2d(w_o, D, D, D, 192, 64, true);
  const int sms = device_sm_count();
  const int grid = a.tiles < sms ? a.tiles : sms;
  const int N = kSelf ? 4 * D : 2 * D;
  const double flops = 2.0 * rows * (double)N * D;
  const int ticket = prof_begin(flops, (int)rows, N, D, stream);
  dec_attn_kernel<kSelf><<<grid, kThreads, kSmem, stream>>>(tmIn, tmO, a);
  prof_end(ticket, stream);
  prof_count_gemm(flops);
  N1_CUDA(cudaGetLastError());
}

DecAttnArgs dec_args(bf16* x, int ldx, const float* ln_w, const float* ln_b, float eps, const float* b_in, const float* b_o,
                     int B, int Ns, int T) {
  N1_CHECK(x && ln_w && ln_b && b_in && b_o, "dec_attn_block: null pointer");
  N1_CHECK((reinterpret_cast<uintptr_t>(x) & 15) == 0 && ldx % 8 == 0 && ldx >= D, "dec_attn_block: misaligned x");
  N1_CHECK(B >= 1 && Ns >= 1 && T >= 1 && T <= BM, "dec_attn_block: needs B, Ns >= 1 and 1 <= T <= 64");
  DecAttnArgs a = {};
  a.x = x, a.ldx = ldx, a.ln_w = ln_w, a.ln_b = ln_b, a.eps = eps, a.b_in = b_in, a.b_o = b_o;
  a.Ns = Ns, a.T = T, a.tpt = BM / T;
  a.tiles_per_env = (Ns + a.tpt - 1) / a.tpt;
  const long tiles = (long)B * a.tiles_per_env;
  N1_CHECK(tiles < (1L << 31), "dec_attn_block: too many tiles");
  a.tiles = (int)tiles;
  return a;
}

}

void dec_sa_block(bf16* x, int ldx, const float* ln_w, const float* ln_b, float eps, const bf16* w_qkv, const float* b_qkv,
                  const bf16* w_o, const float* b_o, int B, int Ns, int T, int causal, cudaStream_t stream) {
  N1_CHECK(w_qkv && w_o, "dec_sa_block: null weights");
  DecAttnArgs a = dec_args(x, ldx, ln_w, ln_b, eps, b_qkv, b_o, B, Ns, T);
  a.causal = causal ? 1 : 0;
  launch_dec_attn<true>(w_qkv, w_o, a, (long)B * Ns * T, stream);
}

void dec_ca_block(bf16* x, int ldx, const float* ln_w, const float* ln_b, float eps, const bf16* w_q, const float* b_q,
                  const bf16* w_o, const float* b_o, const bf16* kv, int ldkv, int mtok, int B, int Ns, int T,
                  cudaStream_t stream) {
  N1_CHECK(w_q && w_o && kv, "dec_ca_block: null weights or K / V");
  N1_CHECK(mtok >= 1 && mtok <= BM, "dec_ca_block: needs 1 <= condition tokens <= 64");
  N1_CHECK((reinterpret_cast<uintptr_t>(kv) & 15) == 0 && ldkv % 8 == 0 && ldkv >= 2 * D, "dec_ca_block: misaligned K / V");
  DecAttnArgs a = dec_args(x, ldx, ln_w, ln_b, eps, b_q, b_o, B, Ns, T);
  a.kv = kv, a.ldkv = ldkv, a.mtok = mtok;
  launch_dec_attn<false>(w_q, w_o, a, (long)B * Ns * T, stream);
}

}
```

### internnav_b200/csrc/dec_tile.cuh

```cuda
#pragma once
#include "n1_ops.h"
#include "n1_ptx.cuh"

namespace n1 {

__device__ __forceinline__ int sw128_offset(int row, int col) {
  return (col >> 6) * 8192 + (row >> 3) * 1024 + (row & 7) * 128 + ((((col & 63) >> 3) ^ (row & 7)) << 4) + (col & 7) * 2;
}

template <int kS>
struct Ring {
  int slot = 0;
  uint32_t phase = 0;
  __device__ __forceinline__ void advance() {
    if (++slot == kS) slot = 0, phase ^= 1;
  }
};

template <bool kNc>
__device__ __forceinline__ void ln384_to_tile(uint8_t* sA, const bf16* x, long ldx, long row0, int nrows, const float* ln_w,
                                              const float* ln_b, float eps, int cw, int lane) {
  constexpr int D = 384;
  uint2 q[8][3];
#pragma unroll
  for (int rr = 0; rr < 8; ++rr) {
    const int r = cw * 8 + rr;
    const uint2* xr = reinterpret_cast<const uint2*>(x + (row0 + r) * ldx);
#pragma unroll
    for (int i = 0; i < 3; ++i)
      q[rr][i] = r < nrows ? (kNc ? __ldg(xr + lane + i * 32) : xr[lane + i * 32]) : make_uint2(0u, 0u);
  }
  float s[8], sq[8];
#pragma unroll
  for (int rr = 0; rr < 8; ++rr) {
    s[rr] = 0.f;
#pragma unroll
    for (int i = 0; i < 3; ++i)
      s[rr] += bf16_lo(q[rr][i].x) + bf16_hi(q[rr][i].x) + bf16_lo(q[rr][i].y) + bf16_hi(q[rr][i].y);
  }
#pragma unroll
  for (int o = 16; o > 0; o >>= 1)
#pragma unroll
    for (int rr = 0; rr < 8; ++rr) s[rr] += __shfl_xor_sync(0xffffffffu, s[rr], o);
#pragma unroll
  for (int rr = 0; rr < 8; ++rr) {
    const float mu = s[rr] * (1.0f / D);
    s[rr] = mu;
    sq[rr] = 0.f;
#pragma unroll
    for (int i = 0; i < 3; ++i) {
      const float a = bf16_lo(q[rr][i].x) - mu, b = bf16_hi(q[rr][i].x) - mu;
      const float c = bf16_lo(q[rr][i].y) - mu, d = bf16_hi(q[rr][i].y) - mu;
      sq[rr] += a * a + b * b + c * c + d * d;
    }
  }
#pragma unroll
  for (int o = 16; o > 0; o >>= 1)
#pragma unroll
    for (int rr = 0; rr < 8; ++rr) sq[rr] += __shfl_xor_sync(0xffffffffu, sq[rr], o);
#pragma unroll
  for (int i = 0; i < 3; ++i) {
    const int col = (lane + i * 32) * 4;
    const float4 lw = __ldg(reinterpret_cast<const float4*>(ln_w + col));
    const float4 lb = __ldg(reinterpret_cast<const float4*>(ln_b + col));
#pragma unroll
    for (int rr = 0; rr < 8; ++rr) {
      const float mu = s[rr], rstd = rsqrtf(sq[rr] * (1.0f / D) + eps);
      const float y0 = (bf16_lo(q[rr][i].x) - mu) * rstd * lw.x + lb.x, y1 = (bf16_hi(q[rr][i].x) - mu) * rstd * lw.y + lb.y;
      const float y2 = (bf16_lo(q[rr][i].y) - mu) * rstd * lw.z + lb.z, y3 = (bf16_hi(q[rr][i].y) - mu) * rstd * lw.w + lb.w;
      *reinterpret_cast<uint2*>(sA + sw128_offset(cw * 8 + rr, col)) = make_uint2(pack_bf16(y0, y1), pack_bf16(y2, y3));
    }
  }
}

template <int N, int kS, typename AfterFirst>
__device__ __forceinline__ void mma_k384(float (&acc)[N], const uint8_t* sA, const uint8_t* ring, uint64_t* full,
                                         uint64_t* empty, Ring<kS>& rs, int slot_bytes, int b_offset, int lane,
                                         AfterFirst after_first) {
  int prev = -1;
#pragma unroll 1
  for (int kb = 0; kb < 6; ++kb) {
    mbar_wait(&full[rs.slot], rs.phase);
    const uint64_t ad = wgmma_desc_sw128(smem_u32(sA + kb * 8192));
    const uint64_t bd = wgmma_desc_sw128(smem_u32(ring + rs.slot * slot_bytes + b_offset));
    wgmma_fence();
#pragma unroll
    for (int k = 0; k < 4; ++k) wgmma_ss<0, 0>(acc, ad + 2 * k, bd + 2 * k, (kb | k) != 0 ? 1u : 0u);
    wgmma_commit();
    wgmma_wait<1>();
    if (kb == 0) after_first();
    if (lane == 0 && prev >= 0) mbar_arrive(&empty[prev]);
    prev = rs.slot;
    rs.advance();
  }
  wgmma_wait<0>();
  if (lane == 0) mbar_arrive(&empty[prev]);
}

template <bool kNc>
__device__ __forceinline__ void residual_epilogue_192(const float (&y)[96], const bf16* x, long ldx, bf16* out, long ldo,
                                                      const float* bias, long row0, int nrows, int g, int r0, int quad) {
#pragma unroll
  for (int hh = 0; hh < 2; ++hh) {
    const int r = r0 + hh * 8;
    if (r >= nrows) continue;
    const bf16* xr = x + (row0 + r) * ldx + g * 192 + quad * 2;
    bf16* orow = out + (row0 + r) * ldo + g * 192 + quad * 2;
#pragma unroll
    for (int jj = 0; jj < 24; ++jj) {
      const uint32_t* xp = reinterpret_cast<const uint32_t*>(xr + jj * 8);
      const uint32_t xv = kNc ? __ldg(xp) : *xp;
      const float2 b = __ldg(reinterpret_cast<const float2*>(bias + g * 192 + jj * 8 + quad * 2));
      *reinterpret_cast<uint32_t*>(orow + jj * 8) =
          pack_bf16(y[jj * 4 + 2 * hh] + bf16_lo(xv) + b.x, y[jj * 4 + 2 * hh + 1] + bf16_hi(xv) + b.y);
    }
  }
}

template <int NKP>
__device__ __forceinline__ void attn_hd48_16rows(const uint32_t (&qf)[3][4], const uint8_t* sK, const uint8_t* sV,
                                                 int row_bytes, const int (&lo_key)[2], const int (&hi_key)[2], float sl2,
                                                 int lane, float (&o)[6][4], float& inv0, float& inv1) {
  const int lm = lane >> 3, lr = lane & 7;
  float s[2 * NKP][4];
#pragma unroll
  for (int i = 0; i < 2 * NKP; ++i) s[i][0] = s[i][1] = s[i][2] = s[i][3] = 0.f;
#pragma unroll
  for (int ks = 0; ks < 3; ++ks)
#pragma unroll
    for (int np = 0; np < NKP; ++np) {
      uint32_t b0, b1, b2, b3;
      ldsm_x4(smem_u32(sK + (np * 16 + (lm >> 1) * 8 + lr) * row_bytes + (ks * 16 + (lm & 1) * 8) * 2), b0, b1, b2, b3);
      mma_bf16(s[2 * np], qf[ks], b0, b1);
      mma_bf16(s[2 * np + 1], qf[ks], b2, b3);
    }
  float mx[2] = {-INFINITY, -INFINITY};
#pragma unroll
  for (int i = 0; i < 2 * NKP; ++i)
#pragma unroll
    for (int e = 0; e < 4; ++e) {
      const int key = i * 8 + (lane & 3) * 2 + (e & 1), r = e >> 1;
      const bool vis = key >= lo_key[r] && key <= hi_key[r];
      s[i][e] = vis ? s[i][e] * sl2 : -INFINITY;
      mx[r] = fmaxf(mx[r], s[i][e]);
    }
  float sum[2] = {0.f, 0.f};
#pragma unroll
  for (int r = 0; r < 2; ++r) {
    mx[r] = fmaxf(mx[r], __shfl_xor_sync(0xffffffffu, mx[r], 1));
    mx[r] = fmaxf(mx[r], __shfl_xor_sync(0xffffffffu, mx[r], 2));
    if (mx[r] == -INFINITY) mx[r] = 0.f;
  }
  uint32_t pf[NKP][4];
#pragma unroll
  for (int i = 0; i < 2 * NKP; ++i) {
    const float p0 = exp2f(s[i][0] - mx[0]), p1 = exp2f(s[i][1] - mx[0]);
    const float p2 = exp2f(s[i][2] - mx[1]), p3 = exp2f(s[i][3] - mx[1]);
    sum[0] += p0 + p1, sum[1] += p2 + p3;
    pf[i >> 1][(i & 1) * 2 + 0] = pack_bf16(p0, p1);
    pf[i >> 1][(i & 1) * 2 + 1] = pack_bf16(p2, p3);
  }
#pragma unroll
  for (int r = 0; r < 2; ++r) {
    sum[r] += __shfl_xor_sync(0xffffffffu, sum[r], 1);
    sum[r] += __shfl_xor_sync(0xffffffffu, sum[r], 2);
  }
#pragma unroll
  for (int i = 0; i < 6; ++i) o[i][0] = o[i][1] = o[i][2] = o[i][3] = 0.f;
#pragma unroll
  for (int kk = 0; kk < NKP; ++kk)
#pragma unroll
    for (int np = 0; np < 3; ++np) {
      uint32_t b0, b1, b2, b3;
      ldsm_x4_t(smem_u32(sV + (kk * 16 + (lm & 1) * 8 + lr) * row_bytes + (np * 16 + (lm >> 1) * 8) * 2), b0, b1, b2, b3);
      mma_bf16(o[2 * np], pf[kk], b0, b1);
      mma_bf16(o[2 * np + 1], pf[kk], b2, b3);
    }
  inv0 = sum[0] > 0.f ? 1.f / sum[0] : 0.f;
  inv1 = sum[1] > 0.f ? 1.f / sum[1] : 0.f;
}

}
```

### internnav_b200/csrc/n1_ops.h

```cpp
#pragma once
#include <cuda.h>
#include <cuda_bf16.h>
#include <cuda_runtime.h>
#include <stdint.h>

#include <stdexcept>
#include <string>

namespace n1 {

typedef __nv_bfloat16 bf16;

struct Error : std::runtime_error {
  int code;
  Error(int c, const std::string& m) : std::runtime_error(m), code(c) {}
};

#define N1_CHECK(cond, msg)                                                                       \
  do {                                                                                            \
    if (!(cond)) throw ::n1::Error(-2, std::string(__FILE__) + ":" + std::to_string(__LINE__) + \
                                           ": " + (msg));                                         \
  } while (0)

#define N1_CUDA(call)                                                                              \
  do {                                                                                             \
    cudaError_t e__ = (call);                                                                      \
    if (e__ != cudaSuccess)                                                                        \
      throw ::n1::Error(-3, std::string(__FILE__) + ":" + std::to_string(__LINE__) + ": " + #call + \
                                ": " + cudaGetErrorString(e__));                                   \
  } while (0)

enum GemmAct { ACT_NONE = 0, ACT_GELU = 1, ACT_RELU = 2, ACT_SWIGLU = 3, ACT_GELU_TANH = 4, ACT_SILU = 5 };

struct GemmEpilogue {
  const float* bias = nullptr;
  const float* gamma = nullptr;
  const bf16* residual = nullptr;
  int ldr = 0;
  int act = ACT_NONE;
  int out_fp32 = 0;
  int rows_per_group = 0, group_stride = 0, group_offset = 0;
  const float* row_add = nullptr;
};

void gemm_bf16(const bf16* A, int lda, const bf16* W, int ldw, void* out, int ldo, int M, int N, int K,
               const GemmEpilogue& epi, cudaStream_t stream, int tile_n = 0);

int device_sm_count();

CUtensorMap tma_map_2d(const bf16* ptr, long rows, long cols, long ld, int box_rows, int box_cols, bool swizzle);
CUtensorMap tma_map_3d_sw128(const bf16* ptr, const long dims[3], const long strides[2], const int box[3]);
void prof_count_gemm(double flops);

struct ProfStats {
  double gemm_ms = 0, gemm_flops = 0;
  long gemm_launches = 0, total_launches = 0;
};
void prof_enable(bool on);
void prof_count_launch(int n = 1);
int prof_begin(double flops, int M, int N, int K, cudaStream_t s);
void prof_end(int ticket, cudaStream_t s);
ProfStats prof_read_and_reset();
int prof_read_shapes(int* mnk, long* count, double* ms, int cap);

void layernorm(const bf16* x, int ldx, bf16* y, int ldy, const float* w, const float* b, int rows, int D,
               float eps, int rms, cudaStream_t stream);

struct AttnParams {
  const bf16* q;
  const bf16* k;
  const bf16* v;
  bf16* o;
  int ldq, ldk, ldv, ldo;
  int heads_q, heads_kv, hd;
  int batch;
  int seq_q, seq_k;
  const int* cu_q;
  const int* cu_k;
  int kv_div;
  int causal;
  float scale;
  int max_seq_q;
  const int* k_len;
  int k_slot;
  long total_rows;
  const int* k_row0;
  const int* k_pages;
};
void attention(const AttnParams& p, cudaStream_t stream);
enum AttnKernel { ATTN_SHORT = 1, ATTN_GENERIC = 2, ATTN_WGMMA = 3 };
struct AttnRoute {
  int kernel;
  int hd;
  int nkp;
  int group;
};
AttnRoute attention_route(const AttnParams& p);
bool attention_tc_supported(const AttnParams& p);
bool attention_uses_tc(const AttnParams& p);
void attention_tc128(const AttnParams& p, cudaStream_t stream);

struct CacheAttnParams {
  const bf16* q;
  int ldq;
  long q_rows;
  const bf16 *k, *v;
  int ldkv;
  long kv_rows;
  bf16* o;
  int ldo;
  const int *cu_q, *ctx, *row0;
  int batch, max_chunk, heads_q, heads_kv;
  float scale;
  const int* pages;
};
void attention_cache(const CacheAttnParams& p, cudaStream_t stream);

void ff_block_384(const bf16* x, int ldx, const float* ln_w, const float* ln_b, float eps, const bf16* w1, const float* b1,
                  const bf16* w2, const float* b2, bf16* out, int ldo, int M, cudaStream_t stream);
void dec_sa_block(bf16* x, int ldx, const float* ln_w, const float* ln_b, float eps, const bf16* w_qkv, const float* b_qkv,
                  const bf16* w_o, const float* b_o, int B, int Ns, int T, int causal, cudaStream_t stream);
void dec_ca_block(bf16* x, int ldx, const float* ln_w, const float* ln_b, float eps, const bf16* w_q, const float* b_q,
                  const bf16* w_o, const float* b_o, const bf16* kv, int ldkv, int mtok, int B, int Ns, int T,
                  cudaStream_t stream);

void mod_norm(const bf16* x, int ldx, const float* w, const bf16* mod, int ld_mod, int rows_per_group, const bf16* res, int ldr,
              bf16* out, int ldo, long rows, int D, float eps, int mode, cudaStream_t stream);
void add_bf16(const bf16* a, const bf16* b, bf16* out, long n, cudaStream_t stream);
void action_embed(const float* lat, const float* w, const float* b, const float* pos, bf16* out, long rows, int T, int D,
                  cudaStream_t stream);
void cfg_euler(const bf16* pred, int ld, long n, int cfg, float scale, float dt, float* lat, cudaStream_t stream);

void traj_to_actions(const float* traj, int B, int Ns, int T, double turn_rad, double step_size, int lookahead,
                     int max_actions, int cap, int* ids, int* count, double* mean_out, cudaStream_t s);
void traj_mean_path(const float* traj, int B, int Ns, int T, double* mean_out, cudaStream_t s);

}
```

### internnav_b200/csrc/n1_ptx.cuh

```cuda
#pragma once
#include <cuda.h>
#include <cuda_bf16.h>
#include <cuda_runtime.h>
#include <stdint.h>
#include <stdio.h>

namespace n1 {

__device__ __forceinline__ uint32_t smem_u32(const void* p) {
  return static_cast<uint32_t>(__cvta_generic_to_shared(p));
}

template <int N>
__device__ __forceinline__ void setmaxnreg_inc() {
  asm volatile("setmaxnreg.inc.sync.aligned.u32 %0;" ::"n"(N));
}
template <int N>
__device__ __forceinline__ void setmaxnreg_dec() {
  asm volatile("setmaxnreg.dec.sync.aligned.u32 %0;" ::"n"(N));
}
constexpr int kProducerRegs = 40, kConsumerRegs = 232;
__device__ __forceinline__ void consumer_barrier() { asm volatile("bar.sync 1, 256;" ::: "memory"); }

__device__ __forceinline__ void mbar_init(uint64_t* bar, uint32_t count) {
  asm volatile("mbarrier.init.shared::cta.b64 [%0], %1;" ::"r"(smem_u32(bar)), "r"(count));
}
__device__ __forceinline__ void fence_mbar_init() {
  asm volatile("fence.mbarrier_init.release.cluster;" ::: "memory");
}
__device__ __forceinline__ void mbar_arrive_expect_tx(uint64_t* bar, uint32_t bytes) {
  asm volatile("mbarrier.arrive.expect_tx.shared::cta.b64 _, [%0], %1;" ::"r"(smem_u32(bar)), "r"(bytes)
               : "memory");
}
__device__ __forceinline__ void mbar_arrive(uint64_t* bar) {
  asm volatile("mbarrier.arrive.shared::cta.b64 _, [%0];" ::"r"(smem_u32(bar)) : "memory");
}
__device__ __forceinline__ bool mbar_try_wait(uint64_t* bar, uint32_t parity) {
  uint32_t ok;
  asm volatile(
      "{\n\t"
      ".reg .pred P1;\n\t"
      "mbarrier.try_wait.parity.shared::cta.b64 P1, [%1], %2;\n\t"
      "selp.b32 %0, 1, 0, P1;\n\t"
      "}"
      : "=r"(ok)
      : "r"(smem_u32(bar)), "r"(parity)
      : "memory");
  return ok != 0;
}
static __device__ __noinline__ void mbar_timeout(uint32_t bar, uint32_t parity) {
#ifdef N1_MBAR_DEBUG
  printf("n1: mbarrier timeout block=(%d,%d) thread=%d bar=0x%x parity=%u\n", blockIdx.x, blockIdx.y, threadIdx.x, bar,
         parity);
#endif
  __trap();
}
__device__ __forceinline__ void mbar_wait(uint64_t* bar, uint32_t parity) {
  if (mbar_try_wait(bar, parity)) return;
  const long long t0 = clock64();
  uint32_t spins = 0;
  while (!mbar_try_wait(bar, parity)) {
    if ((++spins & 1023u) == 0 && clock64() - t0 > 4000000000LL) mbar_timeout(smem_u32(bar), parity);
  }
}

__device__ __forceinline__ void fence_proxy_async_smem() {
  asm volatile("fence.proxy.async.shared::cta;" ::: "memory");
}

__device__ __forceinline__ void tma_prefetch_desc(const CUtensorMap* m) {
  asm volatile("prefetch.tensormap [%0];" ::"l"(reinterpret_cast<uint64_t>(m)) : "memory");
}
__device__ __forceinline__ void tma_load_2d(void* smem_dst, const CUtensorMap* m, uint64_t* bar, int32_t c0,
                                            int32_t c1) {
  asm volatile(
      "cp.async.bulk.tensor.2d.shared::cluster.global.mbarrier::complete_tx::bytes [%0], [%1, {%3, %4}], [%2];"
      :
      : "r"(smem_u32(smem_dst)), "l"(reinterpret_cast<uint64_t>(m)), "r"(smem_u32(bar)), "r"(c0), "r"(c1)
      : "memory");
}
__device__ __forceinline__ void tma_load_3d(void* smem_dst, const CUtensorMap* m, uint64_t* bar, int32_t c0, int32_t c1,
                                            int32_t c2) {
  asm volatile(
      "cp.async.bulk.tensor.3d.shared::cluster.global.mbarrier::complete_tx::bytes [%0], [%1, {%3, %4, %5}], [%2];"
      :
      : "r"(smem_u32(smem_dst)), "l"(reinterpret_cast<uint64_t>(m)), "r"(smem_u32(bar)), "r"(c0), "r"(c1), "r"(c2)
      : "memory");
}
__device__ __forceinline__ void tma_store_2d(const CUtensorMap* m, const void* smem_src, int32_t c0, int32_t c1) {
  asm volatile("cp.async.bulk.tensor.2d.global.shared::cta.bulk_group [%0, {%2, %3}], [%1];"
               :
               : "l"(reinterpret_cast<uint64_t>(m)), "r"(smem_u32(smem_src)), "r"(c0), "r"(c1)
               : "memory");
}
__device__ __forceinline__ void tma_store_commit() { asm volatile("cp.async.bulk.commit_group;" ::: "memory"); }
template <int N>
__device__ __forceinline__ void tma_store_wait_read() {
  asm volatile("cp.async.bulk.wait_group.read %0;" ::"n"(N) : "memory");
}
template <int N>
__device__ __forceinline__ void tma_store_wait() {
  asm volatile("cp.async.bulk.wait_group %0;" ::"n"(N) : "memory");
}

__device__ __forceinline__ void wgmma_fence() { asm volatile("wgmma.fence.sync.aligned;" ::: "memory"); }
__device__ __forceinline__ void wgmma_commit() { asm volatile("wgmma.commit_group.sync.aligned;" ::: "memory"); }
template <int N>
__device__ __forceinline__ void wgmma_wait() {
  asm volatile("wgmma.wait_group.sync.aligned %0;" ::"n"(N) : "memory");
}
template <int TA, int TB>
__device__ __forceinline__ void wgmma_ss(float (&d)[32], uint64_t adesc, uint64_t bdesc, uint32_t accumulate) {
  asm volatile(
      "{\n\t.reg .pred p;\n\tsetp.ne.b32 p, %34, 0;\n\t"
      "wgmma.mma_async.sync.aligned.m64n64k16.f32.bf16.bf16 {%0, %1, %2, %3, %4, %5, %6, %7, %8, %9, %10, %11, %12, %13, %14, %15, %16, %17, %18, %19, %20, %21, %22, %23, %24, %25, %26, %27, %28, %29, %30, %31}, %32, %33, p, 1, 1, %35, %36;\n\t}"
      : "+f"(d[0]), "+f"(d[1]), "+f"(d[2]), "+f"(d[3]), "+f"(d[4]), "+f"(d[5]), "+f"(d[6]), "+f"(d[7]), "+f"(d[8]), "+f"(d[9]), "+f"(d[10]), "+f"(d[11]), "+f"(d[12]), "+f"(d[13]), "+f"(d[14]), "+f"(d[15]), "+f"(d[16]), "+f"(d[17]), "+f"(d[18]), "+f"(d[19]), "+f"(d[20]), "+f"(d[21]), "+f"(d[22]), "+f"(d[23]), "+f"(d[24]), "+f"(d[25]), "+f"(d[26]), "+f"(d[27]), "+f"(d[28]), "+f"(d[29]), "+f"(d[30]), "+f"(d[31])
      : "l"(adesc), "l"(bdesc), "r"(accumulate), "n"(TA), "n"(TB));
}
template <int TA, int TB>
__device__ __forceinline__ void wgmma_ss(float (&d)[64], uint64_t adesc, uint64_t bdesc, uint32_t accumulate) {
  asm volatile(
      "{\n\t.reg .pred p;\n\tsetp.ne.b32 p, %66, 0;\n\t"
      "wgmma.mma_async.sync.aligned.m64n128k16.f32.bf16.bf16 {%0, %1, %2, %3, %4, %5, %6, %7, %8, %9, %10, %11, %12, %13, %14, %15, %16, %17, %18, %19, %20, %21, %22, %23, %24, %25, %26, %27, %28, %29, %30, %31, %32, %33, %34, %35, %36, %37, %38, %39, %40, %41, %42, %43, %44, %45, %46, %47, %48, %49, %50, %51, %52, %53, %54, %55, %56, %57, %58, %59, %60, %61, %62, %63}, %64, %65, p, 1, 1, %67, %68;\n\t}"
      : "+f"(d[0]), "+f"(d[1]), "+f"(d[2]), "+f"(d[3]), "+f"(d[4]), "+f"(d[5]), "+f"(d[6]), "+f"(d[7]), "+f"(d[8]), "+f"(d[9]), "+f"(d[10]), "+f"(d[11]), "+f"(d[12]), "+f"(d[13]), "+f"(d[14]), "+f"(d[15]), "+f"(d[16]), "+f"(d[17]), "+f"(d[18]), "+f"(d[19]), "+f"(d[20]), "+f"(d[21]), "+f"(d[22]), "+f"(d[23]), "+f"(d[24]), "+f"(d[25]), "+f"(d[26]), "+f"(d[27]), "+f"(d[28]), "+f"(d[29]), "+f"(d[30]), "+f"(d[31]), "+f"(d[32]), "+f"(d[33]), "+f"(d[34]), "+f"(d[35]), "+f"(d[36]), "+f"(d[37]), "+f"(d[38]), "+f"(d[39]), "+f"(d[40]), "+f"(d[41]), "+f"(d[42]), "+f"(d[43]), "+f"(d[44]), "+f"(d[45]), "+f"(d[46]), "+f"(d[47]), "+f"(d[48]), "+f"(d[49]), "+f"(d[50]), "+f"(d[51]), "+f"(d[52]), "+f"(d[53]), "+f"(d[54]), "+f"(d[55]), "+f"(d[56]), "+f"(d[57]), "+f"(d[58]), "+f"(d[59]), "+f"(d[60]), "+f"(d[61]), "+f"(d[62]), "+f"(d[63])
      : "l"(adesc), "l"(bdesc), "r"(accumulate), "n"(TA), "n"(TB));
}
template <int TA, int TB>
__device__ __forceinline__ void wgmma_ss(float (&d)[96], uint64_t adesc, uint64_t bdesc, uint32_t accumulate) {
  asm volatile(
      "{\n\t.reg .pred p;\n\tsetp.ne.b32 p, %98, 0;\n\t"
      "wgmma.mma_async.sync.aligned.m64n192k16.f32.bf16.bf16 {%0, %1, %2, %3, %4, %5, %6, %7, %8, %9, %10, %11, %12, %13, %14, %15, %16, %17, %18, %19, %20, %21, %22, %23, %24, %25, %26, %27, %28, %29, %30, %31, %32, %33, %34, %35, %36, %37, %38, %39, %40, %41, %42, %43, %44, %45, %46, %47, %48, %49, %50, %51, %52, %53, %54, %55, %56, %57, %58, %59, %60, %61, %62, %63, %64, %65, %66, %67, %68, %69, %70, %71, %72, %73, %74, %75, %76, %77, %78, %79, %80, %81, %82, %83, %84, %85, %86, %87, %88, %89, %90, %91, %92, %93, %94, %95}, %96, %97, p, 1, 1, %99, %100;\n\t}"
      : "+f"(d[0]), "+f"(d[1]), "+f"(d[2]), "+f"(d[3]), "+f"(d[4]), "+f"(d[5]), "+f"(d[6]), "+f"(d[7]), "+f"(d[8]), "+f"(d[9]), "+f"(d[10]), "+f"(d[11]), "+f"(d[12]), "+f"(d[13]), "+f"(d[14]), "+f"(d[15]), "+f"(d[16]), "+f"(d[17]), "+f"(d[18]), "+f"(d[19]), "+f"(d[20]), "+f"(d[21]), "+f"(d[22]), "+f"(d[23]), "+f"(d[24]), "+f"(d[25]), "+f"(d[26]), "+f"(d[27]), "+f"(d[28]), "+f"(d[29]), "+f"(d[30]), "+f"(d[31]), "+f"(d[32]), "+f"(d[33]), "+f"(d[34]), "+f"(d[35]), "+f"(d[36]), "+f"(d[37]), "+f"(d[38]), "+f"(d[39]), "+f"(d[40]), "+f"(d[41]), "+f"(d[42]), "+f"(d[43]), "+f"(d[44]), "+f"(d[45]), "+f"(d[46]), "+f"(d[47]), "+f"(d[48]), "+f"(d[49]), "+f"(d[50]), "+f"(d[51]), "+f"(d[52]), "+f"(d[53]), "+f"(d[54]), "+f"(d[55]), "+f"(d[56]), "+f"(d[57]), "+f"(d[58]), "+f"(d[59]), "+f"(d[60]), "+f"(d[61]), "+f"(d[62]), "+f"(d[63]), "+f"(d[64]), "+f"(d[65]), "+f"(d[66]), "+f"(d[67]), "+f"(d[68]), "+f"(d[69]), "+f"(d[70]), "+f"(d[71]), "+f"(d[72]), "+f"(d[73]), "+f"(d[74]), "+f"(d[75]), "+f"(d[76]), "+f"(d[77]), "+f"(d[78]), "+f"(d[79]), "+f"(d[80]), "+f"(d[81]), "+f"(d[82]), "+f"(d[83]), "+f"(d[84]), "+f"(d[85]), "+f"(d[86]), "+f"(d[87]), "+f"(d[88]), "+f"(d[89]), "+f"(d[90]), "+f"(d[91]), "+f"(d[92]), "+f"(d[93]), "+f"(d[94]), "+f"(d[95])
      : "l"(adesc), "l"(bdesc), "r"(accumulate), "n"(TA), "n"(TB));
}
template <int TA, int TB>
__device__ __forceinline__ void wgmma_ss(float (&d)[128], uint64_t adesc, uint64_t bdesc, uint32_t accumulate) {
  asm volatile(
      "{\n\t.reg .pred p;\n\tsetp.ne.b32 p, %130, 0;\n\t"
      "wgmma.mma_async.sync.aligned.m64n256k16.f32.bf16.bf16 {%0, %1, %2, %3, %4, %5, %6, %7, %8, %9, %10, %11, %12, %13, %14, %15, %16, %17, %18, %19, %20, %21, %22, %23, %24, %25, %26, %27, %28, %29, %30, %31, %32, %33, %34, %35, %36, %37, %38, %39, %40, %41, %42, %43, %44, %45, %46, %47, %48, %49, %50, %51, %52, %53, %54, %55, %56, %57, %58, %59, %60, %61, %62, %63, %64, %65, %66, %67, %68, %69, %70, %71, %72, %73, %74, %75, %76, %77, %78, %79, %80, %81, %82, %83, %84, %85, %86, %87, %88, %89, %90, %91, %92, %93, %94, %95, %96, %97, %98, %99, %100, %101, %102, %103, %104, %105, %106, %107, %108, %109, %110, %111, %112, %113, %114, %115, %116, %117, %118, %119, %120, %121, %122, %123, %124, %125, %126, %127}, %128, %129, p, 1, 1, %131, %132;\n\t}"
      : "+f"(d[0]), "+f"(d[1]), "+f"(d[2]), "+f"(d[3]), "+f"(d[4]), "+f"(d[5]), "+f"(d[6]), "+f"(d[7]), "+f"(d[8]), "+f"(d[9]), "+f"(d[10]), "+f"(d[11]), "+f"(d[12]), "+f"(d[13]), "+f"(d[14]), "+f"(d[15]), "+f"(d[16]), "+f"(d[17]), "+f"(d[18]), "+f"(d[19]), "+f"(d[20]), "+f"(d[21]), "+f"(d[22]), "+f"(d[23]), "+f"(d[24]), "+f"(d[25]), "+f"(d[26]), "+f"(d[27]), "+f"(d[28]), "+f"(d[29]), "+f"(d[30]), "+f"(d[31]), "+f"(d[32]), "+f"(d[33]), "+f"(d[34]), "+f"(d[35]), "+f"(d[36]), "+f"(d[37]), "+f"(d[38]), "+f"(d[39]), "+f"(d[40]), "+f"(d[41]), "+f"(d[42]), "+f"(d[43]), "+f"(d[44]), "+f"(d[45]), "+f"(d[46]), "+f"(d[47]), "+f"(d[48]), "+f"(d[49]), "+f"(d[50]), "+f"(d[51]), "+f"(d[52]), "+f"(d[53]), "+f"(d[54]), "+f"(d[55]), "+f"(d[56]), "+f"(d[57]), "+f"(d[58]), "+f"(d[59]), "+f"(d[60]), "+f"(d[61]), "+f"(d[62]), "+f"(d[63]), "+f"(d[64]), "+f"(d[65]), "+f"(d[66]), "+f"(d[67]), "+f"(d[68]), "+f"(d[69]), "+f"(d[70]), "+f"(d[71]), "+f"(d[72]), "+f"(d[73]), "+f"(d[74]), "+f"(d[75]), "+f"(d[76]), "+f"(d[77]), "+f"(d[78]), "+f"(d[79]), "+f"(d[80]), "+f"(d[81]), "+f"(d[82]), "+f"(d[83]), "+f"(d[84]), "+f"(d[85]), "+f"(d[86]), "+f"(d[87]), "+f"(d[88]), "+f"(d[89]), "+f"(d[90]), "+f"(d[91]), "+f"(d[92]), "+f"(d[93]), "+f"(d[94]), "+f"(d[95]), "+f"(d[96]), "+f"(d[97]), "+f"(d[98]), "+f"(d[99]), "+f"(d[100]), "+f"(d[101]), "+f"(d[102]), "+f"(d[103]), "+f"(d[104]), "+f"(d[105]), "+f"(d[106]), "+f"(d[107]), "+f"(d[108]), "+f"(d[109]), "+f"(d[110]), "+f"(d[111]), "+f"(d[112]), "+f"(d[113]), "+f"(d[114]), "+f"(d[115]), "+f"(d[116]), "+f"(d[117]), "+f"(d[118]), "+f"(d[119]), "+f"(d[120]), "+f"(d[121]), "+f"(d[122]), "+f"(d[123]), "+f"(d[124]), "+f"(d[125]), "+f"(d[126]), "+f"(d[127])
      : "l"(adesc), "l"(bdesc), "r"(accumulate), "n"(TA), "n"(TB));
}
template <int TA, int TB>
__device__ __forceinline__ void wgmma_ss(float (&d)[24], uint64_t adesc, uint64_t bdesc, uint32_t accumulate) {
  asm volatile(
      "{\n\t.reg .pred p;\n\tsetp.ne.b32 p, %26, 0;\n\t"
      "wgmma.mma_async.sync.aligned.m64n48k16.f32.bf16.bf16 {%0, %1, %2, %3, %4, %5, %6, %7, %8, %9, %10, %11, %12, %13, %14, %15, %16, %17, %18, %19, %20, %21, %22, %23}, %24, %25, p, 1, 1, %27, %28;\n\t}"
      : "+f"(d[0]), "+f"(d[1]), "+f"(d[2]), "+f"(d[3]), "+f"(d[4]), "+f"(d[5]), "+f"(d[6]), "+f"(d[7]), "+f"(d[8]), "+f"(d[9]), "+f"(d[10]), "+f"(d[11]), "+f"(d[12]), "+f"(d[13]), "+f"(d[14]), "+f"(d[15]), "+f"(d[16]), "+f"(d[17]), "+f"(d[18]), "+f"(d[19]), "+f"(d[20]), "+f"(d[21]), "+f"(d[22]), "+f"(d[23])
      : "l"(adesc), "l"(bdesc), "r"(accumulate), "n"(TA), "n"(TB));
}
template <int TA, int TB>
__device__ __forceinline__ void wgmma_ss(float (&d)[72], uint64_t adesc, uint64_t bdesc, uint32_t accumulate) {
  asm volatile(
      "{\n\t.reg .pred p;\n\tsetp.ne.b32 p, %74, 0;\n\t"
      "wgmma.mma_async.sync.aligned.m64n144k16.f32.bf16.bf16 {%0, %1, %2, %3, %4, %5, %6, %7, %8, %9, %10, %11, %12, %13, %14, %15, %16, %17, %18, %19, %20, %21, %22, %23, %24, %25, %26, %27, %28, %29, %30, %31, %32, %33, %34, %35, %36, %37, %38, %39, %40, %41, %42, %43, %44, %45, %46, %47, %48, %49, %50, %51, %52, %53, %54, %55, %56, %57, %58, %59, %60, %61, %62, %63, %64, %65, %66, %67, %68, %69, %70, %71}, %72, %73, p, 1, 1, %75, %76;\n\t}"
      : "+f"(d[0]), "+f"(d[1]), "+f"(d[2]), "+f"(d[3]), "+f"(d[4]), "+f"(d[5]), "+f"(d[6]), "+f"(d[7]), "+f"(d[8]), "+f"(d[9]), "+f"(d[10]), "+f"(d[11]), "+f"(d[12]), "+f"(d[13]), "+f"(d[14]), "+f"(d[15]), "+f"(d[16]), "+f"(d[17]), "+f"(d[18]), "+f"(d[19]), "+f"(d[20]), "+f"(d[21]), "+f"(d[22]), "+f"(d[23]), "+f"(d[24]), "+f"(d[25]), "+f"(d[26]), "+f"(d[27]), "+f"(d[28]), "+f"(d[29]), "+f"(d[30]), "+f"(d[31]), "+f"(d[32]), "+f"(d[33]), "+f"(d[34]), "+f"(d[35]), "+f"(d[36]), "+f"(d[37]), "+f"(d[38]), "+f"(d[39]), "+f"(d[40]), "+f"(d[41]), "+f"(d[42]), "+f"(d[43]), "+f"(d[44]), "+f"(d[45]), "+f"(d[46]), "+f"(d[47]), "+f"(d[48]), "+f"(d[49]), "+f"(d[50]), "+f"(d[51]), "+f"(d[52]), "+f"(d[53]), "+f"(d[54]), "+f"(d[55]), "+f"(d[56]), "+f"(d[57]), "+f"(d[58]), "+f"(d[59]), "+f"(d[60]), "+f"(d[61]), "+f"(d[62]), "+f"(d[63]), "+f"(d[64]), "+f"(d[65]), "+f"(d[66]), "+f"(d[67]), "+f"(d[68]), "+f"(d[69]), "+f"(d[70]), "+f"(d[71])
      : "l"(adesc), "l"(bdesc), "r"(accumulate), "n"(TA), "n"(TB));
}
template <int TB>
__device__ __forceinline__ void wgmma_rs(float (&d)[64], const uint32_t (&a)[4], uint64_t bdesc, uint32_t accumulate) {
  asm volatile(
      "{\n\t.reg .pred p;\n\tsetp.ne.b32 p, %69, 0;\n\t"
      "wgmma.mma_async.sync.aligned.m64n128k16.f32.bf16.bf16 {%0, %1, %2, %3, %4, %5, %6, %7, %8, %9, %10, %11, %12, %13, %14, %15, %16, %17, %18, %19, %20, %21, %22, %23, %24, %25, %26, %27, %28, %29, %30, %31, %32, %33, %34, %35, %36, %37, %38, %39, %40, %41, %42, %43, %44, %45, %46, %47, %48, %49, %50, %51, %52, %53, %54, %55, %56, %57, %58, %59, %60, %61, %62, %63}, {%64, %65, %66, %67}, %68, p, 1, 1, %70;\n\t}"
      : "+f"(d[0]), "+f"(d[1]), "+f"(d[2]), "+f"(d[3]), "+f"(d[4]), "+f"(d[5]), "+f"(d[6]), "+f"(d[7]), "+f"(d[8]), "+f"(d[9]), "+f"(d[10]), "+f"(d[11]), "+f"(d[12]), "+f"(d[13]), "+f"(d[14]), "+f"(d[15]), "+f"(d[16]), "+f"(d[17]), "+f"(d[18]), "+f"(d[19]), "+f"(d[20]), "+f"(d[21]), "+f"(d[22]), "+f"(d[23]), "+f"(d[24]), "+f"(d[25]), "+f"(d[26]), "+f"(d[27]), "+f"(d[28]), "+f"(d[29]), "+f"(d[30]), "+f"(d[31]), "+f"(d[32]), "+f"(d[33]), "+f"(d[34]), "+f"(d[35]), "+f"(d[36]), "+f"(d[37]), "+f"(d[38]), "+f"(d[39]), "+f"(d[40]), "+f"(d[41]), "+f"(d[42]), "+f"(d[43]), "+f"(d[44]), "+f"(d[45]), "+f"(d[46]), "+f"(d[47]), "+f"(d[48]), "+f"(d[49]), "+f"(d[50]), "+f"(d[51]), "+f"(d[52]), "+f"(d[53]), "+f"(d[54]), "+f"(d[55]), "+f"(d[56]), "+f"(d[57]), "+f"(d[58]), "+f"(d[59]), "+f"(d[60]), "+f"(d[61]), "+f"(d[62]), "+f"(d[63])
      : "r"(a[0]), "r"(a[1]), "r"(a[2]), "r"(a[3]), "l"(bdesc), "r"(accumulate), "n"(TB));
}
__device__ __forceinline__ uint64_t wgmma_desc_sw128(uint32_t smem_addr, uint32_t lbo_bytes = 16) {
  uint64_t d = 0;
  d |= static_cast<uint64_t>((smem_addr & 0x3FFFF) >> 4);
  d |= static_cast<uint64_t>((lbo_bytes >> 4) & 0x3FFF) << 16;
  d |= static_cast<uint64_t>(1024 >> 4) << 32;
  d |= static_cast<uint64_t>(1) << 62;
  return d;
}

__device__ __forceinline__ void ldsm_x4(uint32_t addr, uint32_t& r0, uint32_t& r1, uint32_t& r2, uint32_t& r3) {
  asm volatile("ldmatrix.sync.aligned.m8n8.x4.shared.b16 {%0,%1,%2,%3}, [%4];"
               : "=r"(r0), "=r"(r1), "=r"(r2), "=r"(r3)
               : "r"(addr));
}
__device__ __forceinline__ void ldsm_x4_t(uint32_t addr, uint32_t& r0, uint32_t& r1, uint32_t& r2, uint32_t& r3) {
  asm volatile("ldmatrix.sync.aligned.m8n8.x4.trans.shared.b16 {%0,%1,%2,%3}, [%4];"
               : "=r"(r0), "=r"(r1), "=r"(r2), "=r"(r3)
               : "r"(addr));
}
__device__ __forceinline__ void mma_bf16(float (&c)[4], const uint32_t (&a)[4], uint32_t b0, uint32_t b1) {
  asm volatile(
      "mma.sync.aligned.m16n8k16.row.col.f32.bf16.bf16.f32 {%0,%1,%2,%3}, {%4,%5,%6,%7}, {%8,%9}, {%0,%1,%2,%3};"
      : "+f"(c[0]), "+f"(c[1]), "+f"(c[2]), "+f"(c[3])
      : "r"(a[0]), "r"(a[1]), "r"(a[2]), "r"(a[3]), "r"(b0), "r"(b1));
}

__device__ __forceinline__ uint32_t pack_bf16(float lo, float hi) {
  __nv_bfloat162 v = __floats2bfloat162_rn(lo, hi);
  return *reinterpret_cast<uint32_t*>(&v);
}
__device__ __forceinline__ float bf16_lo(uint32_t v) { return __uint_as_float(v << 16); }
__device__ __forceinline__ float bf16_hi(uint32_t v) { return __uint_as_float(v & 0xFFFF0000u); }

__device__ __forceinline__ float warp_sum(float v) {
#pragma unroll
  for (int o = 16; o > 0; o >>= 1) v += __shfl_xor_sync(0xffffffffu, v, o);
  return v;
}
__device__ __forceinline__ float gelu_erf(float x) {
  const float z = fabsf(x) * 0.70710678118654752f;
  float d = fmaf(0.0000430638f, z, 0.0002765672f);
  d = fmaf(d, z, 0.0001520143f);
  d = fmaf(d, z, 0.0092705272f);
  d = fmaf(d, z, 0.0422820123f);
  d = fmaf(d, z, 0.0705230784f);
  d = fmaf(d, z, 1.0f);
  float r = __fdividef(1.0f, d);
  r *= r, r *= r, r *= r, r *= r;
  return 0.5f * x * (1.0f + copysignf(1.0f - r, x));
}
__device__ __forceinline__ void gelu_erf8(float (&x)[8]) {
  float z[8], d[8];
#pragma unroll
  for (int i = 0; i < 8; ++i) z[i] = fabsf(x[i]) * 0.70710678118654752f;
#pragma unroll
  for (int i = 0; i < 8; ++i) d[i] = fmaf(0.0000430638f, z[i], 0.0002765672f);
#pragma unroll
  for (int i = 0; i < 8; ++i) d[i] = fmaf(d[i], z[i], 0.0001520143f);
#pragma unroll
  for (int i = 0; i < 8; ++i) d[i] = fmaf(d[i], z[i], 0.0092705272f);
#pragma unroll
  for (int i = 0; i < 8; ++i) d[i] = fmaf(d[i], z[i], 0.0422820123f);
#pragma unroll
  for (int i = 0; i < 8; ++i) d[i] = fmaf(d[i], z[i], 0.0705230784f);
#pragma unroll
  for (int i = 0; i < 8; ++i) d[i] = fmaf(d[i], z[i], 1.0f);
#pragma unroll
  for (int i = 0; i < 8; ++i) asm("rcp.approx.ftz.f32 %0, %1;" : "=f"(d[i]) : "f"(d[i]));
#pragma unroll
  for (int i = 0; i < 8; ++i) d[i] *= d[i];
#pragma unroll
  for (int i = 0; i < 8; ++i) d[i] *= d[i];
#pragma unroll
  for (int i = 0; i < 8; ++i) d[i] *= d[i];
#pragma unroll
  for (int i = 0; i < 8; ++i) d[i] *= d[i];
#pragma unroll
  for (int i = 0; i < 8; ++i) {
    const float h = 0.5f * x[i];
    x[i] = fmaf(h, copysignf(1.0f - d[i], x[i]), h);
  }
}
__device__ __forceinline__ float silu(float x) { return __fdividef(x, 1.0f + __expf(-x)); }

}
```

### internnav_b200/csrc/s1_model.cu

```cuda
#include "s1_model.h"

#include <math.h>

#include <vector>

namespace n1 {

namespace {

Lin load_lin(Arena& a, const WeightSource& ws, const std::string& wname, const std::string& bname, long row0, long rows,
             long cols, cudaStream_t s) {
  Lin L;
  L.N = (int)rows;
  L.K = (int)((cols + 7) & ~7L);
  L.w = ws.mat(a, wname, row0, rows, cols, &L.ldw, s);
  if (!bname.empty()) L.b = ws.f32_rows(a, bname, row0, rows, 1, s);
  N1_CHECK(L.N % 8 == 0, "linear " + wname + ": N must be a multiple of 8");
  return L;
}
LNp load_ln(Arena& a, const WeightSource& ws, const std::string& prefix, cudaStream_t s) {
  LNp p;
  p.w = ws.f32(a, prefix + ".weight", s);
  p.b = ws.f32(a, prefix + ".bias", s);
  return p;
}

void bicubic_resample(const std::vector<float>& src, int G, int g, int D, float scale_factor, std::vector<float>& dst) {
  dst.assign((size_t)g * g * D, 0.f);
  const float rscale = (float)(1.0 / (double)scale_factor);
  const float A = -0.75f;
  auto cc1 = [&](float x) { return ((A + 2.f) * x - (A + 3.f)) * x * x + 1.f; };
  auto cc2 = [&](float x) { return ((A * x - 5.f * A) * x + 8.f * A) * x - 4.f * A; };
  auto coeffs = [&](float t, float* c) {
    c[0] = cc2(t + 1.f), c[1] = cc1(t), c[2] = cc1(1.f - t), c[3] = cc2(2.f - t);
  };
  auto clampi = [&](int v) { return v < 0 ? 0 : (v > G - 1 ? G - 1 : v); };
  for (int oy = 0; oy < g; ++oy) {
    const float sy = rscale * (oy + 0.5f) - 0.5f;
    const int iy = (int)floorf(sy);
    float cy[4];
    coeffs(sy - iy, cy);
    for (int ox = 0; ox < g; ++ox) {
      const float sx = rscale * (ox + 0.5f) - 0.5f;
      const int ix = (int)floorf(sx);
      float cx[4];
      coeffs(sx - ix, cx);
      float* o = &dst[((size_t)oy * g + ox) * D];
      for (int i = 0; i < 4; ++i) {
        const int yy = clampi(iy - 1 + i);
        for (int j = 0; j < 4; ++j) {
          const int xx = clampi(ix - 1 + j);
          const float w = cy[i] * cx[j];
          const float* sp = &src[((size_t)yy * G + xx) * D];
          for (int d = 0; d < D; ++d) o[d] += w * sp[d];
        }
      }
    }
  }
}

}

S1Model::Vit S1Model::load_vit(const WeightSource& ws, bool depth, cudaStream_t s) {
  const int D = dims.D;
  Vit v;
  if (!depth) {
    v.patch = load_lin(arena_, ws, "patch_embed.proj.weight", "patch_embed.proj.bias", 0, D, 588, s);
  } else {
    const SrcTensor& w = ws.get("patch_embed.proj.weight");
    float* folded = arena_.alloc_n<float>((size_t)D * 196);
    fold_groups(w.data, w.dtype, D, 3, 196, folded, s);
    v.patch.N = D, v.patch.K = 200, v.patch.ldw = 200;
    v.patch.w = arena_.alloc_n<bf16>((size_t)D * 200);
    pack2d(folded, 0, 196, 0, D, 196, v.patch.w, 1, 200, s);
    v.patch.b = ws.f32(arena_, "patch_embed.proj.bias", s);
  }
  {
    const SrcTensor& pe = ws.get("pos_embed");
    const long ntok = pe.numel() / D;
    const int G = (int)lround(sqrt((double)(ntok - 1)));
    N1_CHECK((long)G * G + 1 == ntok, "pos_embed is not 1 + G*G tokens");
    float* dev = ws.f32(arena_, "pos_embed", s);
    float* cls = ws.f32(arena_, "cls_token", s);
    std::vector<float> host((size_t)ntok * D), hcls(D);
    N1_CUDA(cudaStreamSynchronize(s));
    N1_CUDA(cudaMemcpy(host.data(), dev, host.size() * 4, cudaMemcpyDeviceToHost));
    N1_CUDA(cudaMemcpy(hcls.data(), cls, D * 4, cudaMemcpyDeviceToHost));
    std::vector<float> grid(host.begin() + D, host.end()), out;
    if (G == 16) {
      out = grid;
    } else {
      const float sf = (float)((16 + 0.1) / (double)G);
      bicubic_resample(grid, G, 16, D, sf, out);
    }
    v.pos_patch = arena_.alloc_n<float>(256 * D);
    N1_CUDA(cudaMemcpy(v.pos_patch, out.data(), out.size() * 4, cudaMemcpyHostToDevice));
    for (int d = 0; d < D; ++d) hcls[d] += host[d];
    v.cls_pos = arena_.alloc_n<float>(D);
    N1_CUDA(cudaMemcpy(v.cls_pos, hcls.data(), D * 4, cudaMemcpyHostToDevice));
  }
  v.blk.resize(12);
  for (int i = 0; i < 12; ++i) {
    const WeightSource b = ws.sub("blocks." + std::to_string(i) + ".");
    VitBlock& k = v.blk[i];
    k.n1 = load_ln(arena_, b, "norm1", s);
    k.n2 = load_ln(arena_, b, "norm2", s);
    k.qkv = load_lin(arena_, b, "attn.qkv.weight", "attn.qkv.bias", 0, 3 * D, D, s);
    k.proj = load_lin(arena_, b, "attn.proj.weight", "attn.proj.bias", 0, D, D, s);
    k.fc1 = load_lin(arena_, b, "mlp.fc1.weight", "mlp.fc1.bias", 0, 4 * D, D, s);
    k.fc2 = load_lin(arena_, b, "mlp.fc2.weight", "mlp.fc2.bias", 0, D, 4 * D, s);
    k.ls1 = b.f32(arena_, "ls1.gamma", s);
    k.ls2 = b.f32(arena_, "ls2.gamma", s);
  }
  v.norm = load_ln(arena_, ws, "norm", s);
  return v;
}

S1Model::DecLayer S1Model::load_dec_layer(const WeightSource& ws, bool with_kv, cudaStream_t s) {
  const int D = dims.D;
  DecLayer L;
  L.n1 = load_ln(arena_, ws, "norm1", s);
  L.n2 = load_ln(arena_, ws, "norm2", s);
  L.n3 = load_ln(arena_, ws, "norm3", s);
  L.sa_qkv = load_lin(arena_, ws, "self_attn.in_proj_weight", "self_attn.in_proj_bias", 0, 3 * D, D, s);
  L.sa_out = load_lin(arena_, ws, "self_attn.out_proj.weight", "self_attn.out_proj.bias", 0, D, D, s);
  L.ca_q = load_lin(arena_, ws, "multihead_attn.in_proj_weight", "multihead_attn.in_proj_bias", 0, D, D, s);
  if (with_kv)
    L.ca_kv = load_lin(arena_, ws, "multihead_attn.in_proj_weight", "multihead_attn.in_proj_bias", D, 2 * D, D, s);
  L.ca_out = load_lin(arena_, ws, "multihead_attn.out_proj.weight", "multihead_attn.out_proj.bias", 0, D, D, s);
  const long ff = ws.get("linear1.bias").numel();
  L.ff1 = load_lin(arena_, ws, "linear1.weight", "linear1.bias", 0, ff, D, s);
  L.ff2 = load_lin(arena_, ws, "linear2.weight", "linear2.bias", 0, D, ff, s);
  return L;
}

void S1Model::load(const WeightSource& ws, const S1Dims& d, cudaStream_t s) {
  dims = d;
  const int D = dims.D;
  N1_CHECK(D == 384, "System-1 kernels are specialised for token_dim 384");
  N1_CHECK(D / dims.heads == 48, "System-1 decoder head_dim must be 48");
  const int Mq = dims.mem_tokens();
  const long slots = dims.frames + dims.depth_frames();
  rgb_ = load_vit(ws.sub("rgbd_encoder.rgb_model."), false, s);
  depth_ = load_vit(ws.sub("rgbd_encoder.depth_model."), true, s);
  const WeightSource enc = ws.sub("rgbd_encoder.");
  {
    const long pe_rows = enc.get("former_pe.weight").numel() / D;
    N1_CHECK(pe_rows >= slots * 256, "former_pe too small (needs navdp_version > 0 layout)");
    former_pe_ = enc.f32_rows(arena_, "former_pe.weight", 0, slots * 256, D, s);
    int ld;
    former_query_ = enc.mat(arena_, "former_query.weight", 0, Mq, D, &ld, s);
  }
  former_.clear();
  for (int i = 0; i < 2; ++i)
    former_.push_back(load_dec_layer(enc.sub("former_net.layers." + std::to_string(i) + "."), true, s));
  project_ = load_lin(arena_, enc, "project_layer.weight", "project_layer.bias", 0, D, D, s);

  if (!dims.standalone) {
  vlm0_ = load_lin(arena_, ws, "vlm_embed_mlp.0.weight", "vlm_embed_mlp.0.bias", 0, dims.vlm_dim / 4, dims.vlm_dim, s);
  vlm1_ = load_lin(arena_, ws, "vlm_embed_mlp.2.weight", "vlm_embed_mlp.2.bias", 0, dims.vlm_dim / 8, dims.vlm_dim / 4, s);
  vlm2_ = load_lin(arena_, ws, "vlm_embed_mlp.4.weight", "vlm_embed_mlp.4.bias", 0, D, dims.vlm_dim / 8, s);
  const WeightSource gc = ws.sub("goal_compressor.");
  token_pe_ = gc.f32_rows(arena_, "token_positional_encoding.position_embedding.weight", 0, dims.n_query, D, s);
  goal_kv_ = load_lin(arena_, gc, "cross_attention.in_proj_weight", "cross_attention.in_proj_bias", D, 2 * D, D, s);
  goal_out_ = load_lin(arena_, gc, "cross_attention.out_proj.weight", "cross_attention.out_proj.bias", 0, D, D, s);
  {
    Lin gq = load_lin(arena_, gc, "cross_attention.in_proj_weight", "cross_attention.in_proj_bias", 0, D, D, s);
    float* te = gc.f32_rows(arena_, "target_embedding.weight", 0, 1, D, s);
    float* qp = gc.f32_rows(arena_, "query_positional_encoding.position_embedding.weight", 0, 1, D, s);
    std::vector<float> a(D), b(D);
    N1_CUDA(cudaStreamSynchronize(s));
    N1_CUDA(cudaMemcpy(a.data(), te, D * 4, cudaMemcpyDeviceToHost));
    N1_CUDA(cudaMemcpy(b.data(), qp, D * 4, cudaMemcpyDeviceToHost));
    for (int i = 0; i < D; ++i) a[i] += b[i];
    N1_CUDA(cudaMemcpy(te, a.data(), D * 4, cudaMemcpyHostToDevice));
    bf16* qin = arena_.alloc_n<bf16>(8 * D);
    N1_CUDA(cudaMemsetAsync(qin, 0, 8 * D * sizeof(bf16), s));
    f32_to_bf16(te, qin, D, s);
    goal_q_ = arena_.alloc_n<bf16>(D);
    linear(gq, qin, D, goal_q_, D, 1, GemmEpilogue(), s);
  }
  }

  in_w_ = ws.f32(arena_, "input_embed.weight", s);
  in_b_ = ws.f32(arena_, "input_embed.bias", s);
  out_pos_ = ws.f32_rows(arena_, "out_pos_embed", 0, dims.T, D, s);
  cond_pos_ = ws.f32_rows(arena_, "cond_pos_embed", 0, dims.cond_tokens(), D, s);
  if (dims.standalone) {
    critic_w_ = ws.f32(arena_, "critic_head.weight", s);
    critic_b_ = ws.f32(arena_, "critic_head.bias", s);
  }
  dec_.clear();
  kv_all_.N = dims.layers * 2 * D, kv_all_.K = D, kv_all_.ldw = D;
  kv_all_.w = arena_.alloc_n<bf16>((size_t)kv_all_.N * D);
  kv_all_.b = arena_.alloc_n<float>(kv_all_.N);
  for (int i = 0; i < dims.layers; ++i) {
    const WeightSource lw = ws.sub("decoder.layers." + std::to_string(i) + ".");
    dec_.push_back(load_dec_layer(lw, false, s));
    const SrcTensor& w = lw.get("multihead_attn.in_proj_weight");
    const SrcTensor& b = lw.get("multihead_attn.in_proj_bias");
    pack2d(w.data, w.dtype, D, D, 2 * D, D, kv_all_.w + (size_t)i * 2 * D * D, 1, D, s);
    pack2d(b.data, b.dtype, 1, D, 2 * D, 1, kv_all_.b + (size_t)i * 2 * D, 0, 1, s);
  }
  final_ln_ = load_ln(arena_, ws, "layernorm", s);
  head_w_ = ws.f32(arena_, "action_head.weight", s);
  head_b_ = ws.f32(arena_, "action_head.bias", s);
  N1_CUDA(cudaStreamSynchronize(s));
  loaded_ = true;
}

size_t S1Model::vit_forward(const Vit& v, Carver c, const float* img, bool depth, int n_img, bf16* mem, int slot_base,
                            cudaStream_t s, bool with_pe, int frames_per_env) const {
  if (frames_per_env <= 0) frames_per_env = dims.frames;
  const int D = dims.D;
  const long rows = (long)n_img * 257;
  const int ldk = v.patch.K;
  bf16* col = c.take<bf16>((size_t)n_img * 256 * ldk);
  bf16* x = c.take<bf16>(rows * D);
  bf16* ln = c.take<bf16>(rows * D);
  bf16* qkv = c.take<bf16>(rows * 3 * D);
  bf16* att = c.take<bf16>(rows * D);
  bf16* hid = c.take<bf16>(rows * 4 * D);
  if (c.dry()) return c.used();

  if (depth)
    patchify_depth(img, col, n_img, ldk, s);
  else
    patchify_rgb(img, col, n_img, ldk, s, dims.standalone != 0);
  {
    GemmEpilogue e;
    e.rows_per_group = 256, e.group_stride = 257, e.group_offset = 1, e.row_add = v.pos_patch;
    linear(v.patch, col, ldk, x, D, n_img * 256, e, s);
  }
  fill_cls(x, v.cls_pos, n_img, 257, D, s);
  for (const VitBlock& b : v.blk) {
    layernorm(x, D, ln, D, b.n1.w, b.n1.b, (int)rows, D, 1e-6f, 0, s);
    linear(b.qkv, ln, D, qkv, 3 * D, (int)rows, GemmEpilogue(), s);
    AttnParams p = {};
    p.q = qkv, p.k = qkv + D, p.v = qkv + 2 * D, p.o = att;
    p.ldq = p.ldk = p.ldv = 3 * D, p.ldo = D;
    p.heads_q = p.heads_kv = 6, p.hd = 64, p.batch = n_img, p.seq_q = p.seq_k = 257, p.kv_div = 1;
    p.scale = 0.125f;
    attention(p, s);
    GemmEpilogue e1;
    e1.gamma = b.ls1, e1.residual = x, e1.ldr = D;
    linear(b.proj, att, D, x, D, (int)rows, e1, s);
    layernorm(x, D, ln, D, b.n2.w, b.n2.b, (int)rows, D, 1e-6f, 0, s);
    GemmEpilogue e2;
    e2.act = ACT_GELU;
    linear(b.fc1, ln, D, hid, 4 * D, (int)rows, e2, s);
    GemmEpilogue e3;
    e3.gamma = b.ls2, e3.residual = x, e3.ldr = D;
    linear(b.fc2, hid, 4 * D, x, D, (int)rows, e3, s);
  }
  vit_out(x, mem, v.norm.w, v.norm.b, with_pe ? former_pe_ : nullptr, n_img, frames_per_env, slot_base,
          dims.frames + dims.depth_frames(), s);
  return c.used();
}

size_t S1Model::rgbd_impl(Carver c, const float* rgb, const float* depth, bf16* out, int B, cudaStream_t s) const {
  const int D = dims.D, F = dims.frames, Fd = dims.depth_frames(), Mq = dims.mem_tokens();
  const long mrows = (long)B * (F + Fd) * 256;
  bf16* mem = c.take<bf16>(mrows * D);
  const long qrows = (long)B * Mq;
  bf16* x = c.take<bf16>(qrows * D);
  bf16* y = c.take<bf16>(qrows * D);
  bf16* qkv = c.take<bf16>(qrows * 3 * D);
  bf16* att = c.take<bf16>(qrows * D);
  bf16* hid = c.take<bf16>(qrows * 2048);
  bf16* kv = c.take<bf16>(mrows * 2 * D);
  const size_t hi_rgb = vit_forward(rgb_, c, rgb, false, B * F, mem, 0, s);
  const size_t hi_dep = vit_forward(depth_, c, depth, true, B * Fd, mem, F, s, true, Fd);
  const size_t hi = hi_rgb > hi_dep ? hi_rgb : hi_dep;
  if (c.dry()) return hi;

  bcast_rows(former_query_, x, qrows, Mq, D, s);
  const float scale48 = 1.0f / sqrtf(48.f);
  for (const DecLayer& L : former_) {
    linear(L.sa_qkv, x, D, qkv, 3 * D, (int)qrows, GemmEpilogue(), s);
    AttnParams p = {};
    p.q = qkv, p.k = qkv + D, p.v = qkv + 2 * D, p.o = att;
    p.ldq = p.ldk = p.ldv = 3 * D, p.ldo = D;
    p.heads_q = p.heads_kv = dims.heads, p.hd = 48, p.batch = B, p.seq_q = p.seq_k = Mq, p.kv_div = 1;
    p.scale = scale48;
    attention(p, s);
    GemmEpilogue e;
    e.residual = x, e.ldr = D;
    linear(L.sa_out, att, D, y, D, (int)qrows, e, s);
    layernorm(y, D, x, D, L.n1.w, L.n1.b, (int)qrows, D, 1e-5f, 0, s);

    linear(L.ca_q, x, D, qkv, D, (int)qrows, GemmEpilogue(), s);
    linear(L.ca_kv, mem, D, kv, 2 * D, (int)mrows, GemmEpilogue(), s);
    AttnParams pc = {};
    pc.q = qkv, pc.k = kv, pc.v = kv + D, pc.o = att;
    pc.ldq = D, pc.ldk = pc.ldv = 2 * D, pc.ldo = D;
    pc.heads_q = pc.heads_kv = dims.heads, pc.hd = 48, pc.batch = B, pc.seq_q = Mq, pc.seq_k = (F + Fd) * 256;
    pc.kv_div = 1, pc.scale = scale48;
    attention(pc, s);
    linear(L.ca_out, att, D, y, D, (int)qrows, e, s);
    layernorm(y, D, x, D, L.n2.w, L.n2.b, (int)qrows, D, 1e-5f, 0, s);

    GemmEpilogue er;
    er.act = ACT_RELU;
    linear(L.ff1, x, D, hid, L.ff1.N, (int)qrows, er, s);
    linear(L.ff2, hid, L.ff1.N, y, D, (int)qrows, e, s);
    layernorm(y, D, x, D, L.n3.w, L.n3.b, (int)qrows, D, 1e-5f, 0, s);
  }
  linear(project_, x, D, out, D, (int)qrows, GemmEpilogue(), s);
  return hi;
}

size_t S1Model::ws_rgbd(int B) const { return rgbd_impl(Carver(nullptr, 0), nullptr, nullptr, nullptr, B, nullptr); }
void S1Model::rgbd_encode(void* ws, size_t ws_bytes, const float* rgb, const float* depth, bf16* out, int B,
                          cudaStream_t s) const {
  N1_CHECK(loaded_, "System-1 weights not loaded");
  N1_CHECK(ws != nullptr, "null workspace");
  if (ws_bytes < ws_rgbd(B)) throw Error(-7, "rgbd_encode: workspace too small");
  rgbd_impl(Carver(ws, ws_bytes), rgb, depth, out, B, s);
}

size_t S1Model::goal_impl(Carver c, const bf16* latents, bf16* goal, int B, cudaStream_t s) const {
  const int D = dims.D, nq = dims.n_query;
  const long rows = (long)B * nq;
  bf16* h1 = c.take<bf16>(rows * vlm0_.N);
  bf16* h2 = c.take<bf16>(rows * vlm1_.N);
  bf16* tok = c.take<bf16>(rows * D);
  bf16* kv = c.take<bf16>(rows * 2 * D);
  bf16* q = c.take<bf16>((long)B * D);
  bf16* att = c.take<bf16>((long)B * D);
  if (c.dry()) return c.used();
  GemmEpilogue relu;
  relu.act = ACT_RELU;
  linear(vlm0_, latents, dims.vlm_dim, h1, vlm0_.N, (int)rows, relu, s);
  linear(vlm1_, h1, vlm0_.N, h2, vlm1_.N, (int)rows, relu, s);
  GemmEpilogue pe;
  pe.rows_per_group = nq, pe.group_stride = nq, pe.group_offset = 0, pe.row_add = token_pe_;
  linear(vlm2_, h2, vlm1_.N, tok, D, (int)rows, pe, s);
  linear(goal_kv_, tok, D, kv, 2 * D, (int)rows, GemmEpilogue(), s);
  bcast_rows(goal_q_, q, B, 1, D, s);
  AttnParams p = {};
  p.q = q, p.k = kv, p.v = kv + D, p.o = att;
  p.ldq = D, p.ldk = p.ldv = 2 * D, p.ldo = D;
  p.heads_q = p.heads_kv = dims.heads, p.hd = 48, p.batch = B, p.seq_q = 1, p.seq_k = nq, p.kv_div = 1;
  p.scale = 1.0f / sqrtf(48.f);
  attention(p, s);
  linear(goal_out_, att, D, goal, D, B, GemmEpilogue(), s);
  return c.used();
}
size_t S1Model::ws_goal(int B) const { return goal_impl(Carver(nullptr, 0), nullptr, nullptr, B, nullptr); }
void S1Model::goal_compress(void* ws, size_t ws_bytes, const bf16* latents, bf16* goal, int B, cudaStream_t s) const {
  N1_CHECK(loaded_, "System-1 weights not loaded");
  N1_CHECK(ws != nullptr, "null workspace");
  if (ws_bytes < ws_goal(B)) throw Error(-7, "goal_compress: workspace too small");
  goal_impl(Carver(ws, ws_bytes), latents, goal, B, s);
}

struct S1Model::DenoiseBufs {
  bf16 *x, *x2, *ln, *qkv, *att, *hid, *cond, *ckv;
  int* klen;
};

bool S1Model::fused_attn(int T) const {
  const int D = dims.D;
  if (!loaded_ || T > 32 || dims.cond_tokens() > 64) return false;
  for (const DecLayer& L : dec_)
    if (L.sa_qkv.ldw != D || L.sa_out.ldw != D || L.ca_q.ldw != D || L.ca_out.ldw != D || L.ff1.N != 1536 ||
        L.ff1.ldw != D || L.ff2.ldw != 1536)
      return false;
  return true;
}

S1Model::DenoiseBufs S1Model::carve_denoise(Carver& c, int B, int Ns, int T) const {
  const int D = dims.D, Mtok = dims.cond_tokens();
  const long R = (long)B * Ns * T;
  DenoiseBufs d = {};
  d.x = c.take<bf16>(R * D);
  d.x2 = c.take<bf16>(R * D);
  if (!fused_attn(T) || dims.standalone) {
    d.ln = c.take<bf16>(R * D);
    d.qkv = c.take<bf16>(R * 3 * D);
    d.att = c.take<bf16>(R * D);
  }
  d.hid = c.take<bf16>(R * 4 * D);
  d.cond = c.take<bf16>((long)B * Mtok * D);
  d.ckv = c.take<bf16>((long)B * Mtok * kv_all_.N);
  d.klen = c.take<int>(B);
  return d;
}

void S1Model::decoder_pass(const DenoiseBufs& d, const float* x_t, const int* tsteps, int t_scalar, bool cond_full,
                           const bf16* goal, const bf16* rgbd, int B, int Ns, int T, int mode, float* x_io,
                           const float* noise, float* eps, const DdpmCoef& cf, cudaStream_t s) const {
  const int D = dims.D, Mtok = dims.cond_tokens();
  const long R = (long)B * Ns * T;
  const int ldkv = kv_all_.N;
  const bool critic = mode == 2;
  const int kv_first = critic ? 1 + dims.goal_slots : 0, kv_len = Mtok - kv_first;
  embed_actions(x_t, in_w_, in_b_, out_pos_, d.x, R, T, s);
  if (cond_full) {
    build_cond(tsteps, t_scalar, goal, rgbd, cond_pos_, d.cond, B, Mtok, 0, Mtok, s, dims.goal_slots);
    linear(kv_all_, d.cond, D, d.ckv, ldkv, B * Mtok, GemmEpilogue(), s);
  } else {
    build_cond(tsteps, t_scalar, goal, rgbd, cond_pos_, d.cond, B, Mtok, 0, 1, s, dims.goal_slots);
    linear(kv_all_, d.cond, Mtok * D, d.ckv, Mtok * ldkv, B, GemmEpilogue(), s);
  }
  bf16* xc = d.x;
  if (!critic && fused_attn(T)) {
    for (int l = 0; l < dims.layers; ++l) {
      const DecLayer& L = dec_[l];
      dec_sa_block(xc, D, L.n1.w, L.n1.b, 1e-5f, L.sa_qkv.w, L.sa_qkv.b, L.sa_out.w, L.sa_out.b, B, Ns, T, 1, s);
      dec_ca_block(xc, D, L.n2.w, L.n2.b, 1e-5f, L.ca_q.w, L.ca_q.b, L.ca_out.w, L.ca_out.b, d.ckv + (long)l * 2 * D, ldkv,
                   Mtok, B, Ns, T, s);
      ff_block_384(xc, D, L.n3.w, L.n3.b, 1e-5f, L.ff1.w, L.ff1.b, L.ff2.w, L.ff2.b, xc, D, (int)R, s);
    }
    head_ddpm(xc, final_ln_.w, final_ln_.b, head_w_, head_b_, R, mode, x_io, noise, eps, cf, s);
    return;
  }
  const float scale48 = 1.0f / sqrtf(48.f);
  auto res_gemm_ln = [&](const Lin& W, const bf16* A, int lda, const LNp* ln) {
    GemmEpilogue res;
    res.residual = xc, res.ldr = D;
    linear(W, A, lda, xc, D, (int)R, res, s);
    if (ln) layernorm(xc, D, d.ln, D, ln->w, ln->b, (int)R, D, 1e-5f, 0, s);
  };
  layernorm(xc, D, d.ln, D, dec_[0].n1.w, dec_[0].n1.b, (int)R, D, 1e-5f, 0, s);
  for (int l = 0; l < dims.layers; ++l) {
    const DecLayer& L = dec_[l];
    linear(L.sa_qkv, d.ln, D, d.qkv, 3 * D, (int)R, GemmEpilogue(), s);
    AttnParams p = {};
    p.q = d.qkv, p.k = d.qkv + D, p.v = d.qkv + 2 * D, p.o = d.att;
    p.ldq = p.ldk = p.ldv = 3 * D, p.ldo = D;
    p.heads_q = p.heads_kv = dims.heads, p.hd = 48, p.batch = B * Ns, p.seq_q = p.seq_k = T, p.kv_div = 1;
    p.causal = critic ? 0 : 1, p.scale = scale48;
    attention(p, s);
    res_gemm_ln(L.sa_out, d.att, D, &L.n2);

    linear(L.ca_q, d.ln, D, d.qkv, D, (int)R, GemmEpilogue(), s);
    AttnParams pc = {};
    pc.q = d.qkv, pc.k = d.ckv + (long)l * 2 * D, pc.v = d.ckv + (long)l * 2 * D + D, pc.o = d.att;
    pc.ldq = D, pc.ldk = pc.ldv = ldkv, pc.ldo = D;
    pc.heads_q = pc.heads_kv = dims.heads, pc.hd = 48, pc.batch = B * Ns, pc.seq_q = T, pc.seq_k = Mtok;
    pc.kv_div = Ns, pc.scale = scale48;
    if (kv_first > 0) {
      pc.k += (long)kv_first * ldkv, pc.v += (long)kv_first * ldkv;
      pc.k_len = d.klen, pc.k_slot = Mtok, pc.seq_k = kv_len;
    }
    attention(pc, s);
    const bool ffb = L.ff1.N == 1536 && L.ff1.ldw == D && L.ff2.ldw == 1536;
    res_gemm_ln(L.ca_out, d.att, D, ffb ? nullptr : &L.n3);

    const LNp* next_ln = l + 1 < dims.layers ? &dec_[l + 1].n1 : nullptr;
    if (ffb) {
      ff_block_384(xc, D, L.n3.w, L.n3.b, 1e-5f, L.ff1.w, L.ff1.b, L.ff2.w, L.ff2.b, xc, D, (int)R, s);
      if (next_ln) layernorm(xc, D, d.ln, D, next_ln->w, next_ln->b, (int)R, D, 1e-5f, 0, s);
    } else {
      GemmEpilogue gelu;
      gelu.act = ACT_GELU;
      linear(L.ff1, d.ln, D, d.hid, 4 * D, (int)R, gelu, s);
      res_gemm_ln(L.ff2, d.hid, 4 * D, next_ln);
    }
  }
  if (critic) {
    critic_head(xc, final_ln_.w, final_ln_.b, critic_w_, critic_b_, (long)B * Ns, T, eps, s);
    return;
  }
  head_ddpm(xc, final_ln_.w, final_ln_.b, head_w_, head_b_, R, mode, x_io, noise, eps, cf, s);
}

size_t S1Model::ws_denoise(int B, int Ns, int T) const {
  Carver c(nullptr, 0);
  carve_denoise(c, B, Ns, T);
  return c.used();
}

void S1Model::navdp_eps(void* ws, size_t ws_bytes, const float* x_t, const int* tsteps, int t_scalar, const bf16* goal,
                        const bf16* rgbd, float* eps, int B, int Ns, int T, cudaStream_t s) const {
  N1_CHECK(loaded_, "System-1 weights not loaded");
  N1_CHECK(ws != nullptr, "null workspace");
  N1_CHECK(T >= 1 && T <= dims.T, "predict horizon exceeds out_pos_embed");
  Carver c(ws, ws_bytes);
  DenoiseBufs d = carve_denoise(c, B, Ns, T);
  decoder_pass(d, x_t, tsteps, t_scalar, true, goal, rgbd, B, Ns, T, 0, nullptr, nullptr, eps, DdpmCoef(), s);
}

void S1Model::navdp_critic(void* ws, size_t ws_bytes, const float* traj, const bf16* rgbd, float* critic, int B, int Ns, int T,
                           cudaStream_t s) const {
  N1_CHECK(loaded_ && dims.standalone && critic_w_, "navdp_critic: needs the stand-alone NavDP policy weights");
  N1_CHECK(ws != nullptr && traj && rgbd && critic, "navdp_critic: null buffers");
  N1_CHECK(T >= 1 && T <= dims.T, "predict horizon exceeds out_pos_embed");
  Carver c(ws, ws_bytes);
  DenoiseBufs d = carve_denoise(c, B, Ns, T);
  fill_int(d.klen, dims.mem_tokens(), B, s);
  decoder_pass(d, traj, nullptr, 0, true, nullptr, rgbd, B, Ns, T, 2, nullptr, nullptr, critic, DdpmCoef(), s);
}

void S1Model::ddpm_tables(int N, std::vector<DdpmCoef>& coef) {
  auto abar = [](double u) {
    const double c = cos((u + 0.008) / 1.008 * M_PI / 2.0);
    return c * c;
  };
  std::vector<float> acp(N);
  float prod = 1.f;
  for (int i = 0; i < N; ++i) {
    double beta = 1.0 - abar((double)(i + 1) / N) / abar((double)i / N);
    if (beta > 0.999) beta = 0.999;
    const float alpha = 1.0f - (float)beta;
    prod *= alpha;
    acp[i] = prod;
  }
  coef.resize(N);
  for (int t = 0; t < N; ++t) {
    const float a_t = acp[t], a_prev = t > 0 ? acp[t - 1] : 1.0f;
    const float beta_prod_t = 1.f - a_t, beta_prod_prev = 1.f - a_prev;
    const float cur_alpha = a_t / a_prev, cur_beta = 1.f - cur_alpha;
    DdpmCoef c;
    c.sqrt_one_minus_acp = sqrtf(beta_prod_t);
    c.inv_sqrt_acp = 1.0f / sqrtf(a_t);
    c.c0 = sqrtf(a_prev) * cur_beta / beta_prod_t;
    c.c1 = sqrtf(cur_alpha) * beta_prod_prev / beta_prod_t;
    float var = beta_prod_prev / beta_prod_t * cur_beta;
    if (var < 1e-20f) var = 1e-20f;
    c.sigma = t > 0 ? sqrtf(var) : 0.f;
    coef[t] = c;
  }
}

void S1Model::navdp_sample(void* ws, size_t ws_bytes, const bf16* goal, const bf16* rgbd, const float* x_init,
                           const float* step_noise, float* traj_out, int B, int Ns, int T, int K,
                           cudaStream_t s) const {
  N1_CHECK(loaded_, "System-1 weights not loaded");
  N1_CHECK(ws != nullptr, "null workspace");
  N1_CHECK(T >= 1 && T <= dims.T, "predict horizon exceeds out_pos_embed");
  N1_CHECK(K >= 1, "need at least one denoising step");
  Carver c(ws, ws_bytes);
  DenoiseBufs d = carve_denoise(c, B, Ns, T);
  std::vector<DdpmCoef> coef;
  ddpm_tables(K, coef);
  const long n = (long)B * Ns * T * 3;
  if (traj_out != x_init) N1_CUDA(cudaMemcpyAsync(traj_out, x_init, n * sizeof(float), cudaMemcpyDeviceToDevice, s));
  for (int i = 0; i < K; ++i) {
    const int t = K - 1 - i;
    const float* noise = (t > 0 && step_noise) ? step_noise + (long)i * n : nullptr;
    decoder_pass(d, traj_out, nullptr, t, i == 0, goal, rgbd, B, Ns, T, 1, traj_out, noise, nullptr, coef[t], s);
  }
}

}
```

Measured before the change: 71.12.

## Add paired-tile decoder attention kernel sharing weight stream across two warpgroups

Adds a paired variant of the fused decoder self/cross-attention block in which two consumer warpgroups each process a tile while sharing one TMA-streamed weight ring, so each weight k-block is loaded once per pair instead of once per tile. Attention outputs stay in registers and feed the output projection through register-sourced wgmma (new m64n64/m64n96 RS variants). Cross-attention K/V is staged with cp.async double buffering. The paired form is picked automatically when the number of pairs is at least the SM count, trading less weight traffic for higher register pressure and fewer CTAs.

```diff
diff --git a/include/n1b200.h b/include/n1b200.h
--- a/include/n1b200.h
+++ b/include/n1b200.h
@@ -218,10 +218,10 @@
                    const float* b1, const void* w2_bf16, const float* b2, void* out_bf16, int ldo, int M, void* stream);
 int n1_op_dec_sa_block(void* x_bf16, int ldx, const float* ln_w, const float* ln_b, float eps, const void* w_qkv_bf16,
                        const float* b_qkv, const void* w_o_bf16, const float* b_o, int B, int Ns, int T, int causal,
-                       void* stream);
+                       int form, void* stream);
 int n1_op_dec_ca_block(void* x_bf16, int ldx, const float* ln_w, const float* ln_b, float eps, const void* w_q_bf16,
                        const float* b_q, const void* w_o_bf16, const float* b_o, const void* kv_bf16, int ldkv, int mtok,
-                       int B, int Ns, int T, void* stream);
+                       int B, int Ns, int T, int form, void* stream);
 int n1_op_layernorm(const void* x_bf16, int ldx, void* y_bf16, int ldy, const float* w, const float* b, int rows, int D,
                     float eps, int rms, void* stream);
 int n1_op_mod_norm(const void* x_bf16, int ldx, const float* w, const void* mod_bf16, int ld_mod, int rows_per_group,
diff --git a/internnav_b200/_lib.py b/internnav_b200/_lib.py
--- a/internnav_b200/_lib.py
+++ b/internnav_b200/_lib.py
@@ -153,9 +153,9 @@
     "n1_op_ff_block": (c_int, [c_void_p, c_int, c_void_p, c_void_p, c_float, c_void_p, c_void_p, c_void_p, c_void_p, c_void_p,
                                c_int, c_int, c_void_p]),
     "n1_op_dec_sa_block": (c_int, [c_void_p, c_int, c_void_p, c_void_p, c_float, c_void_p, c_void_p, c_void_p, c_void_p,
-                                   c_int, c_int, c_int, c_int, c_void_p]),
+                                   c_int, c_int, c_int, c_int, c_int, c_void_p]),
     "n1_op_dec_ca_block": (c_int, [c_void_p, c_int, c_void_p, c_void_p, c_float, c_void_p, c_void_p, c_void_p, c_void_p,
-                                   c_void_p, c_int, c_int, c_int, c_int, c_int, c_void_p]),
+                                   c_void_p, c_int, c_int, c_int, c_int, c_int, c_int, c_void_p]),
     "n1_op_layernorm": (c_int, [c_void_p, c_int, c_void_p, c_int, c_void_p, c_void_p, c_int, c_int, c_float, c_int,
                                 c_void_p]),
     "n1_op_mod_norm": (c_int, [c_void_p, c_int, c_void_p, c_void_p, c_int, c_int, c_void_p, c_int, c_void_p, c_int,
@@ -414,17 +414,22 @@
     return out
 
 
-def dec_sa_block(x, ln_w, ln_b, w_qkv, b_qkv, w_o, b_o, B, Ns, T, causal=True, eps=1e-5):
+DEC_FORMS = {"auto": 0, "single": 1, "pair": 2}
+
+
+def dec_sa_block(x, ln_w, ln_b, w_qkv, b_qkv, w_o, b_o, B, Ns, T, causal=True, eps=1e-5, form="auto"):
     assert x.dtype == torch.bfloat16 and x.shape == (B * Ns * T, 384) and x.stride(1) == 1
     assert w_qkv.shape == (1152, 384) and w_o.shape == (384, 384)
     check(lib().n1_op_dec_sa_block(c_void_p(x.data_ptr()), x.stride(0), ptr(ln_w), ptr(ln_b), float(eps), ptr(w_qkv),
-                                   ptr(b_qkv), ptr(w_o), ptr(b_o), B, Ns, T, 1 if causal else 0, stream_ptr()))
+                                   ptr(b_qkv), ptr(w_o), ptr(b_o), B, Ns, T, 1 if causal else 0, DEC_FORMS[form],
+                                   stream_ptr()))
     return x
 
 
-def dec_ca_block(x, ln_w, ln_b, w_q, b_q, w_o, b_o, kv, mtok, B, Ns, T, eps=1e-5):
+def dec_ca_block(x, ln_w, ln_b, w_q, b_q, w_o, b_o, kv, mtok, B, Ns, T, eps=1e-5, form="auto"):
     assert x.dtype == torch.bfloat16 and x.shape == (B * Ns * T, 384) and x.stride(1) == 1
     assert w_q.shape == (384, 384) and w_o.shape == (384, 384) and kv.shape[0] == B * mtok and kv.stride(1) == 1
     check(lib().n1_op_dec_ca_block(c_void_p(x.data_ptr()), x.stride(0), ptr(ln_w), ptr(ln_b), float(eps), ptr(w_q), ptr(b_q),
-                                   ptr(w_o), ptr(b_o), c_void_p(kv.data_ptr()), kv.stride(0), mtok, B, Ns, T, stream_ptr()))
+                                   ptr(w_o), ptr(b_o), c_void_p(kv.data_ptr()), kv.stride(0), mtok, B, Ns, T,
+                                   DEC_FORMS[form], stream_ptr()))
     return x
diff --git a/internnav_b200/csrc/api.cu b/internnav_b200/csrc/api.cu
--- a/internnav_b200/csrc/api.cu
+++ b/internnav_b200/csrc/api.cu
@@ -787,16 +787,18 @@
 }
 
 int n1_op_dec_sa_block(void* x, int ldx, const float* ln_w, const float* ln_b, float eps, const void* w_qkv,
-                       const float* b_qkv, const void* w_o, const float* b_o, int B, int Ns, int T, int causal, void* stream) {
-  return guard([&] {
-    dec_sa_block(B16(x), ldx, ln_w, ln_b, eps, B16(w_qkv), b_qkv, B16(w_o), b_o, B, Ns, T, causal, S(stream));
+                       const float* b_qkv, const void* w_o, const float* b_o, int B, int Ns, int T, int causal, int form,
+                       void* stream) {
+  return guard([&] {
+    dec_sa_block(B16(x), ldx, ln_w, ln_b, eps, B16(w_qkv), b_qkv, B16(w_o), b_o, B, Ns, T, causal, form, S(stream));
   });
 }
 int n1_op_dec_ca_block(void* x, int ldx, const float* ln_w, const float* ln_b, float eps, const void* w_q, const float* b_q,
                        const void* w_o, const float* b_o, const void* kv, int ldkv, int mtok, int B, int Ns, int T,
-                       void* stream) {
-  return guard([&] {
-    dec_ca_block(B16(x), ldx, ln_w, ln_b, eps, B16(w_q), b_q, B16(w_o), b_o, B16(kv), ldkv, mtok, B, Ns, T, S(stream));
+                       int form, void* stream) {
+  return guard([&] {
+    dec_ca_block(B16(x), ldx, ln_w, ln_b, eps, B16(w_q), b_q, B16(w_o), b_o, B16(kv), ldkv, mtok, B, Ns, T, form,
+                 S(stream));
   });
 }
 
diff --git a/internnav_b200/csrc/dec_attn_block.cu b/internnav_b200/csrc/dec_attn_block.cu
--- a/internnav_b200/csrc/dec_attn_block.cu
+++ b/internnav_b200/csrc/dec_attn_block.cu
@@ -27,6 +27,7 @@
   int ldkv;
   int mtok;
   int Ns, T, tpt, tiles_per_env, tiles;
+  int pairs_per_env, pairs;
   int causal;
 };
 
@@ -165,18 +166,180 @@
   }
 }
 
+constexpr int kPairSlots = 4, kPairSlotBytes = 24576;
+static_assert(kPairSlots * kPairSlotBytes == kSlots * kSlotBytes, "dec_attn_block: the paired ring keeps the ring's bytes");
+constexpr int kPairProducerRegs = 24, kPairConsumerRegs = 240;
 template <bool kSelf>
-void launch_dec_attn(const bf16* w_in, const bf16* w_o, const DecAttnArgs& a, long rows, cudaStream_t stream) {
+constexpr int pair_out_cols() { return kSelf ? 64 : 96; }
+static_assert(pair_out_cols<false>() * 64 * 2 <= kPairSlotBytes, "dec_attn_block: a W_o k-block fits a slot");
+
+template <bool kSelf>
+__global__ void __launch_bounds__(kThreads, 1)
+dec_attn_pair_kernel(const __grid_constant__ CUtensorMap tmIn, const __grid_constant__ CUtensorMap tmO, const DecAttnArgs args) {
+  constexpr int kHeadBytes = HD * 64 * 2;
+  constexpr int kOutCols = pair_out_cols<kSelf>(), kOutParts = D / kOutCols;
+  extern __shared__ uint8_t smem_raw[];
+  uint8_t* smem = reinterpret_cast<uint8_t*>((reinterpret_cast<uintptr_t>(smem_raw) + 1023) & ~uintptr_t(1023));
+  uint8_t* sW = smem + 2 * kABytes;
+  uint8_t* sKV = sW + kPairSlots * kPairSlotBytes;
+  uint64_t* bars = reinterpret_cast<uint64_t*>(sKV + 4 * kKvBytes);
+  uint64_t* full = bars;
+  uint64_t* empty = bars + kPairSlots;
+
+  const int warp = threadIdx.x >> 5, lane = threadIdx.x & 31;
+  if (threadIdx.x == 0) {
+    tma_prefetch_desc(&tmIn), tma_prefetch_desc(&tmO);
+    for (int s = 0; s < kPairSlots; ++s) mbar_init(&full[s], 1), mbar_init(&empty[s], kConsumerWarps);
+    fence_mbar_init();
+  }
+  __syncthreads();
+
+  if (warp >= kConsumerWarps) {
+    setmaxnreg_dec<kPairProducerRegs>();
+    if (warp == kConsumerWarps && lane == 0) {
+      Ring<kPairSlots> r;
+      for (int p = blockIdx.x; p < args.pairs; p += gridDim.x) {
+        for (int h = 0; h < 8; ++h)
+          for (int part = kSelf ? 1 : 0; part < (kSelf ? 4 : 1); ++part)
+            for (int kb = 0; kb < D / 64; ++kb) {
+              mbar_wait(&empty[r.slot], r.phase ^ 1);
+              mbar_arrive_expect_tx(&full[r.slot], kHeadBytes);
+              tma_load_2d(sW + r.slot * kPairSlotBytes, &tmIn, &full[r.slot], kb * 64, part % 3 * D + h * HD);
+              r.advance();
+            }
+        for (int c = 0; c < kOutParts; ++c)
+          for (int kb = 0; kb < D / 64; ++kb) {
+            mbar_wait(&empty[r.slot], r.phase ^ 1);
+            mbar_arrive_expect_tx(&full[r.slot], kOutCols * 64 * 2);
+            tma_load_2d(sW + r.slot * kPairSlotBytes, &tmO, &full[r.slot], kb * 64, c * kOutCols);
+            r.advance();
+          }
+      }
+    }
+  } else {
+    setmaxnreg_inc<kPairConsumerRegs>();
+    const int cw = warp;
+    const int g = cw >> 2;
+    const int quad = lane & 3;
+    const int r0 = (cw & 3) * 16 + (lane >> 2);
+    uint8_t* sA = smem + g * kABytes;
+    const float sl2 = 0.14433756729740643f * 1.4426950408889634f;
+    int lo_key[2], hi_key[2];
+#pragma unroll
+    for (int r = 0; r < 2; ++r) {
+      const int qi = r0 + 8 * r;
+      if (kSelf) {
+        lo_key[r] = qi / args.T * args.T;
+        hi_key[r] = args.causal ? qi : lo_key[r] + args.T - 1;
+      } else {
+        lo_key[r] = 0, hi_key[r] = args.mtok - 1;
+      }
+    }
+    Ring<kPairSlots> ring;
+    for (int p = blockIdx.x; p < args.pairs; p += gridDim.x) {
+      const int env = p / args.pairs_per_env;
+      const int traj0 = (2 * (p - env * args.pairs_per_env) + g) * args.tpt;
+      const int ntraj = max(0, min(args.tpt, args.Ns - traj0));
+      const long row0 = ((long)env * args.Ns + traj0) * args.T;
+      const int nrows = ntraj * args.T;
+      auto stage_kv = [&](int h) {
+        const bf16* kb0 = args.kv + (long)env * args.mtok * args.ldkv + h * HD;
+        uint8_t* buf = sKV + (h & 1) * 2 * kKvBytes;
+#pragma unroll
+        for (int i = 0; i < 3; ++i) {
+          const int c = threadIdx.x + 256 * i;
+          const int v = c / (BM * 6), j = (c / 6) % BM, ch = c % 6;
+          const bool ok = j < args.mtok;
+          cp_async_16(buf + v * kKvBytes + j * kKvRow + ch * 16, kb0 + (long)(ok ? j : 0) * args.ldkv + v * D + ch * 8, ok);
+        }
+        cp_async_commit();
+      };
+      consumer_barrier();
+      if (!kSelf) stage_kv(0);
+      const float *ln_w = args.ln_w, *ln_b = args.ln_b;
+      asm volatile("" : "+l"(ln_w), "+l"(ln_b));
+#pragma unroll 1
+      for (int i = 0; i < 2; ++i)
+        ln384_to_tile<false>(sA, args.x, args.ldx, row0, nrows, ln_w, ln_b, args.eps, 2 * (cw & 3) + i, lane);
+      fence_proxy_async_smem();
+
+      uint32_t of[24][4];
+#pragma unroll
+      for (int h = 0; h < 8; ++h) {
+        uint8_t* sK = sKV + (kSelf ? g : h & 1) * 2 * kKvBytes;
+        const float* bh = args.b_in + h * HD + quad * 2;
+        asm volatile("" : "+l"(bh));
+        if (kSelf) {
+          warpgroup_barrier(g);
+#pragma unroll
+          for (int part = 1; part < 3; ++part) {
+            float kv[HD / 2];
+            mma_k384(kv, sA, sW, full, empty, ring, kPairSlotBytes, 0, lane, [] {});
+            uint8_t* buf = sK + (part - 1) * kKvBytes;
+#pragma unroll
+            for (int j = 0; j < HD / 8; ++j) {
+              const int c = j * 8 + quad * 2;
+              const float2 b = __ldg(reinterpret_cast<const float2*>(bh + part * D + j * 8));
+              *reinterpret_cast<uint32_t*>(buf + r0 * kKvRow + c * 2) = pack_bf16(kv[4 * j] + b.x, kv[4 * j + 1] + b.y);
+              *reinterpret_cast<uint32_t*>(buf + (r0 + 8) * kKvRow + c * 2) = pack_bf16(kv[4 * j + 2] + b.x, kv[4 * j + 3] + b.y);
+            }
+          }
+        } else {
+          cp_async_wait_all();
+          consumer_barrier();
+          if (h + 1 < 8) stage_kv(h + 1);
+        }
+        float acc[HD / 2];
+        mma_k384(acc, sA, sW, full, empty, ring, kPairSlotBytes, 0, lane, [] {});
+        uint32_t qf[3][4];
+#pragma unroll
+        for (int j = 0; j < HD / 8; ++j) {
+          const float2 b = __ldg(reinterpret_cast<const float2*>(bh + j * 8));
+          qf[j >> 1][(j & 1) * 2] = pack_bf16(acc[4 * j] + b.x, acc[4 * j + 1] + b.y);
+          qf[j >> 1][(j & 1) * 2 + 1] = pack_bf16(acc[4 * j + 2] + b.x, acc[4 * j + 3] + b.y);
+        }
+        if (kSelf) warpgroup_barrier(g);
+        float o[6][4], inv0, inv1;
+        attn_hd48_16rows<4>(qf, sK, sK + kKvBytes, kKvRow, lo_key, hi_key, sl2, lane, o, inv0, inv1);
+#pragma unroll
+        for (int j = 0; j < 3; ++j) {
+          of[3 * h + j][0] = pack_bf16(o[2 * j][0] * inv0, o[2 * j][1] * inv0);
+          of[3 * h + j][1] = pack_bf16(o[2 * j][2] * inv1, o[2 * j][3] * inv1);
+          of[3 * h + j][2] = pack_bf16(o[2 * j + 1][0] * inv0, o[2 * j + 1][1] * inv0);
+          of[3 * h + j][3] = pack_bf16(o[2 * j + 1][2] * inv1, o[2 * j + 1][3] * inv1);
+        }
+      }
+#pragma unroll
+      for (int c = 0; c < kOutParts; ++c) {
+        float y[kOutCols / 2];
+        mma_rs_k384(y, of, sW, full, empty, ring, kPairSlotBytes, lane);
+        residual_epilogue<false>(y, args.x, args.ldx, args.x, args.ldx, args.b_o, row0, nrows, c * kOutCols, r0, quad);
+      }
+    }
+  }
+}
+
+bool use_pairs(int pairs, int sms) { return pairs >= sms; }
+
+template <bool kSelf>
+void launch_dec_attn(const bf16* w_in, const bf16* w_o, const DecAttnArgs& a, long rows, bool paired, cudaStream_t stream) {
   static std::once_flag once;
-  std::call_once(once, [] { cudaFuncSetAttribute(dec_attn_kernel<kSelf>, cudaFuncAttributeMaxDynamicSharedMemorySize, kSmem); });
+  std::call_once(once, [] {
+    cudaFuncSetAttribute(dec_attn_kernel<kSelf>, cudaFuncAttributeMaxDynamicSharedMemorySize, kSmem);
+    cudaFuncSetAttribute(dec_attn_pair_kernel<kSelf>, cudaFuncAttributeMaxDynamicSharedMemorySize, kSmem);
+  });
   const CUtensorMap tmIn = tma_map_2d(w_in, kSelf ? 3 * D : D, D, D, HD, 64, true);
-  const CUtensorMap tmO = tma_map_2d(w_o, D, D, D, 192, 64, true);
+  const CUtensorMap tmO = tma_map_2d(w_o, D, D, D, paired ? pair_out_cols<kSelf>() : 192, 64, true);
   const int sms = device_sm_count();
-  const int grid = a.tiles < sms ? a.tiles : sms;
+  const int items = paired ? a.pairs : a.tiles;
+  const int grid = items < sms ? items : sms;
   const int N = kSelf ? 4 * D : 2 * D;
   const double flops = 2.0 * rows * (double)N * D;
   const int ticket = prof_begin(flops, (int)rows, N, D, stream);
-  dec_attn_kernel<kSelf><<<grid, kThreads, kSmem, stream>>>(tmIn, tmO, a);
+  if (paired)
+    dec_attn_pair_kernel<kSelf><<<grid, kThreads, kSmem, stream>>>(tmIn, tmO, a);
+  else
+    dec_attn_kernel<kSelf><<<grid, kThreads, kSmem, stream>>>(tmIn, tmO, a);
   prof_end(ticket, stream);
   prof_count_gemm(flops);
   N1_CUDA(cudaGetLastError());
@@ -194,28 +357,34 @@
   const long tiles = (long)B * a.tiles_per_env;
   N1_CHECK(tiles < (1L << 31), "dec_attn_block: too many tiles");
   a.tiles = (int)tiles;
+  a.pairs_per_env = (a.tiles_per_env + 1) / 2;
+  a.pairs = B * a.pairs_per_env;
   return a;
 }
 
 }
 
 void dec_sa_block(bf16* x, int ldx, const float* ln_w, const float* ln_b, float eps, const bf16* w_qkv, const float* b_qkv,
-                  const bf16* w_o, const float* b_o, int B, int Ns, int T, int causal, cudaStream_t stream) {
+                  const bf16* w_o, const float* b_o, int B, int Ns, int T, int causal, int form, cudaStream_t stream) {
   N1_CHECK(w_qkv && w_o, "dec_sa_block: null weights");
+  N1_CHECK(form >= 0 && form <= 2, "dec_sa_block: form is 0 (chosen from the size), 1 (single tiles) or 2 (pairs)");
   DecAttnArgs a = dec_args(x, ldx, ln_w, ln_b, eps, b_qkv, b_o, B, Ns, T);
   a.causal = causal ? 1 : 0;
-  launch_dec_attn<true>(w_qkv, w_o, a, (long)B * Ns * T, stream);
+  const bool paired = form == 0 ? use_pairs(a.pairs, device_sm_count()) : form == 2;
+  launch_dec_attn<true>(w_qkv, w_o, a, (long)B * Ns * T, paired, stream);
 }
 
 void dec_ca_block(bf16* x, int ldx, const float* ln_w, const float* ln_b, float eps, const bf16* w_q, const float* b_q,
-                  const bf16* w_o, const float* b_o, const bf16* kv, int ldkv, int mtok, int B, int Ns, int T,
+                  const bf16* w_o, const float* b_o, const bf16* kv, int ldkv, int mtok, int B, int Ns, int T, int form,
                   cudaStream_t stream) {
   N1_CHECK(w_q && w_o && kv, "dec_ca_block: null weights or K / V");
+  N1_CHECK(form >= 0 && form <= 2, "dec_ca_block: form is 0 (chosen from the size), 1 (single tiles) or 2 (pairs)");
   N1_CHECK(mtok >= 1 && mtok <= BM, "dec_ca_block: needs 1 <= condition tokens <= 64");
   N1_CHECK((reinterpret_cast<uintptr_t>(kv) & 15) == 0 && ldkv % 8 == 0 && ldkv >= 2 * D, "dec_ca_block: misaligned K / V");
   DecAttnArgs a = dec_args(x, ldx, ln_w, ln_b, eps, b_q, b_o, B, Ns, T);
   a.kv = kv, a.ldkv = ldkv, a.mtok = mtok;
-  launch_dec_attn<false>(w_q, w_o, a, (long)B * Ns * T, stream);
-}
-
-}
+  const bool paired = form == 0 ? use_pairs(a.pairs, device_sm_count()) : form == 2;
+  launch_dec_attn<false>(w_q, w_o, a, (long)B * Ns * T, paired, stream);
+}
+
+}
diff --git a/internnav_b200/csrc/dec_tile.cuh b/internnav_b200/csrc/dec_tile.cuh
--- a/internnav_b200/csrc/dec_tile.cuh
+++ b/internnav_b200/csrc/dec_tile.cuh
@@ -97,24 +97,50 @@
   if (lane == 0) mbar_arrive(&empty[prev]);
 }
 
+template <int N, int kS>
+__device__ __forceinline__ void mma_rs_k384(float (&acc)[N], const uint32_t (&a)[24][4], const uint8_t* ring,
+                                            uint64_t* full, uint64_t* empty, Ring<kS>& rs, int slot_bytes, int lane) {
+  int prev = -1;
+#pragma unroll
+  for (int kb = 0; kb < 6; ++kb) {
+    mbar_wait(&full[rs.slot], rs.phase);
+    const uint64_t bd = wgmma_desc_sw128(smem_u32(ring + rs.slot * slot_bytes));
+    wgmma_fence();
+#pragma unroll
+    for (int k = 0; k < 4; ++k) wgmma_rs<0>(acc, a[4 * kb + k], bd + 2 * k, (kb | k) != 0 ? 1u : 0u);
+    wgmma_commit();
+    wgmma_wait<1>();
+    if (lane == 0 && prev >= 0) mbar_arrive(&empty[prev]);
+    prev = rs.slot;
+    rs.advance();
+  }
+  wgmma_wait<0>();
+  if (lane == 0) mbar_arrive(&empty[prev]);
+}
+
+template <bool kNc, int N>
+__device__ __forceinline__ void residual_epilogue(const float (&y)[N], const bf16* x, long ldx, bf16* out, long ldo,
+                                                  const float* bias, long row0, int nrows, int col0, int r0, int quad) {
+#pragma unroll
+  for (int hh = 0; hh < 2; ++hh) {
+    const int r = r0 + hh * 8;
+    if (r >= nrows) continue;
+    const bf16* xr = x + (row0 + r) * ldx + col0 + quad * 2;
+    bf16* orow = out + (row0 + r) * ldo + col0 + quad * 2;
+#pragma unroll
+    for (int jj = 0; jj < N / 4; ++jj) {
+      const uint32_t* xp = reinterpret_cast<const uint32_t*>(xr + jj * 8);
+      const uint32_t xv = kNc ? __ldg(xp) : *xp;
+      const float2 b = __ldg(reinterpret_cast<const float2*>(bias + col0 + jj * 8 + quad * 2));
+      *reinterpret_cast<uint32_t*>(orow + jj * 8) =
+          pack_bf16(y[jj * 4 + 2 * hh] + bf16_lo(xv) + b.x, y[jj * 4 + 2 * hh + 1] + bf16_hi(xv) + b.y);
+    }
+  }
+}
 template <bool kNc>
 __device__ __forceinline__ void residual_epilogue_192(const float (&y)[96], const bf16* x, long ldx, bf16* out, long ldo,
                                                       const float* bias, long row0, int nrows, int g, int r0, int quad) {
-#pragma unroll
-  for (int hh = 0; hh < 2; ++hh) {
-    const int r = r0 + hh * 8;
-    if (r >= nrows) continue;
-    const bf16* xr = x + (row0 + r) * ldx + g * 192 + quad * 2;
-    bf16* orow = out + (row0 + r) * ldo + g * 192 + quad * 2;
-#pragma unroll
-    for (int jj = 0; jj < 24; ++jj) {
-      const uint32_t* xp = reinterpret_cast<const uint32_t*>(xr + jj * 8);
-      const uint32_t xv = kNc ? __ldg(xp) : *xp;
-      const float2 b = __ldg(reinterpret_cast<const float2*>(bias + g * 192 + jj * 8 + quad * 2));
-      *reinterpret_cast<uint32_t*>(orow + jj * 8) =
-          pack_bf16(y[jj * 4 + 2 * hh] + bf16_lo(xv) + b.x, y[jj * 4 + 2 * hh + 1] + bf16_hi(xv) + b.y);
-    }
-  }
+  residual_epilogue<kNc>(y, x, ldx, out, ldo, bias, row0, nrows, 192 * g, r0, quad);
 }
 
 template <int NKP>
diff --git a/internnav_b200/csrc/n1_ops.h b/internnav_b200/csrc/n1_ops.h
--- a/internnav_b200/csrc/n1_ops.h
+++ b/internnav_b200/csrc/n1_ops.h
@@ -119,9 +119,9 @@
 void ff_block_384(const bf16* x, int ldx, const float* ln_w, const float* ln_b, float eps, const bf16* w1, const float* b1,
                   const bf16* w2, const float* b2, bf16* out, int ldo, int M, cudaStream_t stream);
 void dec_sa_block(bf16* x, int ldx, const float* ln_w, const float* ln_b, float eps, const bf16* w_qkv, const float* b_qkv,
-                  const bf16* w_o, const float* b_o, int B, int Ns, int T, int causal, cudaStream_t stream);
+                  const bf16* w_o, const float* b_o, int B, int Ns, int T, int causal, int form, cudaStream_t stream);
 void dec_ca_block(bf16* x, int ldx, const float* ln_w, const float* ln_b, float eps, const bf16* w_q, const float* b_q,
-                  const bf16* w_o, const float* b_o, const bf16* kv, int ldkv, int mtok, int B, int Ns, int T,
+                  const bf16* w_o, const float* b_o, const bf16* kv, int ldkv, int mtok, int B, int Ns, int T, int form,
                   cudaStream_t stream);
 
 void mod_norm(const bf16* x, int ldx, const float* w, const bf16* mod, int ld_mod, int rows_per_group, const bf16* res, int ldr,
diff --git a/internnav_b200/csrc/n1_ptx.cuh b/internnav_b200/csrc/n1_ptx.cuh
--- a/internnav_b200/csrc/n1_ptx.cuh
+++ b/internnav_b200/csrc/n1_ptx.cuh
@@ -103,6 +103,13 @@
   asm volatile("cp.async.bulk.wait_group %0;" ::"n"(N) : "memory");
 }
 
+__device__ __forceinline__ void cp_async_16(void* smem_dst, const void* src, bool valid) {
+  asm volatile("cp.async.cg.shared.global [%0], [%1], 16, %2;" ::"r"(smem_u32(smem_dst)), "l"(src), "r"(valid ? 16 : 0)
+               : "memory");
+}
+__device__ __forceinline__ void cp_async_commit() { asm volatile("cp.async.commit_group;" ::: "memory"); }
+__device__ __forceinline__ void cp_async_wait_all() { asm volatile("cp.async.wait_group 0;" ::: "memory"); }
+
 __device__ __forceinline__ void wgmma_fence() { asm volatile("wgmma.fence.sync.aligned;" ::: "memory"); }
 __device__ __forceinline__ void wgmma_commit() { asm volatile("wgmma.commit_group.sync.aligned;" ::: "memory"); }
 template <int N>
@@ -163,6 +170,22 @@
       "{\n\t.reg .pred p;\n\tsetp.ne.b32 p, %69, 0;\n\t"
       "wgmma.mma_async.sync.aligned.m64n128k16.f32.bf16.bf16 {%0, %1, %2, %3, %4, %5, %6, %7, %8, %9, %10, %11, %12, %13, %14, %15, %16, %17, %18, %19, %20, %21, %22, %23, %24, %25, %26, %27, %28, %29, %30, %31, %32, %33, %34, %35, %36, %37, %38, %39, %40, %41, %42, %43, %44, %45, %46, %47, %48, %49, %50, %51, %52, %53, %54, %55, %56, %57, %58, %59, %60, %61, %62, %63}, {%64, %65, %66, %67}, %68, p, 1, 1, %70;\n\t}"
       : "+f"(d[0]), "+f"(d[1]), "+f"(d[2]), "+f"(d[3]), "+f"(d[4]), "+f"(d[5]), "+f"(d[6]), "+f"(d[7]), "+f"(d[8]), "+f"(d[9]), "+f"(d[10]), "+f"(d[11]), "+f"(d[12]), "+f"(d[13]), "+f"(d[14]), "+f"(d[15]), "+f"(d[16]), "+f"(d[17]), "+f"(d[18]), "+f"(d[19]), "+f"(d[20]), "+f"(d[21]), "+f"(d[22]), "+f"(d[23]), "+f"(d[24]), "+f"(d[25]), "+f"(d[26]), "+f"(d[27]), "+f"(d[28]), "+f"(d[29]), "+f"(d[30]), "+f"(d[31]), "+f"(d[32]), "+f"(d[33]), "+f"(d[34]), "+f"(d[35]), "+f"(d[36]), "+f"(d[37]), "+f"(d[38]), "+f"(d[39]), "+f"(d[40]), "+f"(d[41]), "+f"(d[42]), "+f"(d[43]), "+f"(d[44]), "+f"(d[45]), "+f"(d[46]), "+f"(d[47]), "+f"(d[48]), "+f"(d[49]), "+f"(d[50]), "+f"(d[51]), "+f"(d[52]), "+f"(d[53]), "+f"(d[54]), "+f"(d[55]), "+f"(d[56]), "+f"(d[57]), "+f"(d[58]), "+f"(d[59]), "+f"(d[60]), "+f"(d[61]), "+f"(d[62]), "+f"(d[63])
+      : "r"(a[0]), "r"(a[1]), "r"(a[2]), "r"(a[3]), "l"(bdesc), "r"(accumulate), "n"(TB));
+}
+template <int TB>
+__device__ __forceinline__ void wgmma_rs(float (&d)[32], const uint32_t (&a)[4], uint64_t bdesc, uint32_t accumulate) {
+  asm volatile(
+      "{\n\t.reg .pred p;\n\tsetp.ne.b32 p, %37, 0;\n\t"
+      "wgmma.mma_async.sync.aligned.m64n64k16.f32.bf16.bf16 {%0, %1, %2, %3, %4, %5, %6, %7, %8, %9, %10, %11, %12, %13, %14, %15, %16, %17, %18, %19, %20, %21, %22, %23, %24, %25, %26, %27, %28, %29, %30, %31}, {%32, %33, %34, %35}, %36, p, 1, 1, %38;\n\t}"
+      : "+f"(d[0]), "+f"(d[1]), "+f"(d[2]), "+f"(d[3]), "+f"(d[4]), "+f"(d[5]), "+f"(d[6]), "+f"(d[7]), "+f"(d[8]), "+f"(d[9]), "+f"(d[10]), "+f"(d[11]), "+f"(d[12]), "+f"(d[13]), "+f"(d[14]), "+f"(d[15]), "+f"(d[16]), "+f"(d[17]), "+f"(d[18]), "+f"(d[19]), "+f"(d[20]), "+f"(d[21]), "+f"(d[22]), "+f"(d[23]), "+f"(d[24]), "+f"(d[25]), "+f"(d[26]), "+f"(d[27]), "+f"(d[28]), "+f"(d[29]), "+f"(d[30]), "+f"(d[31])
+      : "r"(a[0]), "r"(a[1]), "r"(a[2]), "r"(a[3]), "l"(bdesc), "r"(accumulate), "n"(TB));
+}
+template <int TB>
+__device__ __forceinline__ void wgmma_rs(float (&d)[48], const uint32_t (&a)[4], uint64_t bdesc, uint32_t accumulate) {
+  asm volatile(
+      "{\n\t.reg .pred p;\n\tsetp.ne.b32 p, %53, 0;\n\t"
+      "wgmma.mma_async.sync.aligned.m64n96k16.f32.bf16.bf16 {%0, %1, %2, %3, %4, %5, %6, %7, %8, %9, %10, %11, %12, %13, %14, %15, %16, %17, %18, %19, %20, %21, %22, %23, %24, %25, %26, %27, %28, %29, %30, %31, %32, %33, %34, %35, %36, %37, %38, %39, %40, %41, %42, %43, %44, %45, %46, %47}, {%48, %49, %50, %51}, %52, p, 1, 1, %54;\n\t}"
+      : "+f"(d[0]), "+f"(d[1]), "+f"(d[2]), "+f"(d[3]), "+f"(d[4]), "+f"(d[5]), "+f"(d[6]), "+f"(d[7]), "+f"(d[8]), "+f"(d[9]), "+f"(d[10]), "+f"(d[11]), "+f"(d[12]), "+f"(d[13]), "+f"(d[14]), "+f"(d[15]), "+f"(d[16]), "+f"(d[17]), "+f"(d[18]), "+f"(d[19]), "+f"(d[20]), "+f"(d[21]), "+f"(d[22]), "+f"(d[23]), "+f"(d[24]), "+f"(d[25]), "+f"(d[26]), "+f"(d[27]), "+f"(d[28]), "+f"(d[29]), "+f"(d[30]), "+f"(d[31]), "+f"(d[32]), "+f"(d[33]), "+f"(d[34]), "+f"(d[35]), "+f"(d[36]), "+f"(d[37]), "+f"(d[38]), "+f"(d[39]), "+f"(d[40]), "+f"(d[41]), "+f"(d[42]), "+f"(d[43]), "+f"(d[44]), "+f"(d[45]), "+f"(d[46]), "+f"(d[47])
       : "r"(a[0]), "r"(a[1]), "r"(a[2]), "r"(a[3]), "l"(bdesc), "r"(accumulate), "n"(TB));
 }
 __device__ __forceinline__ uint64_t wgmma_desc_sw128(uint32_t smem_addr, uint32_t lbo_bytes = 16) {
diff --git a/internnav_b200/csrc/s1_model.cu b/internnav_b200/csrc/s1_model.cu
--- a/internnav_b200/csrc/s1_model.cu
+++ b/internnav_b200/csrc/s1_model.cu
@@ -408,9 +408,9 @@
   if (!critic && fused_attn(T)) {
     for (int l = 0; l < dims.layers; ++l) {
       const DecLayer& L = dec_[l];
-      dec_sa_block(xc, D, L.n1.w, L.n1.b, 1e-5f, L.sa_qkv.w, L.sa_qkv.b, L.sa_out.w, L.sa_out.b, B, Ns, T, 1, s);
+      dec_sa_block(xc, D, L.n1.w, L.n1.b, 1e-5f, L.sa_qkv.w, L.sa_qkv.b, L.sa_out.w, L.sa_out.b, B, Ns, T, 1, 0, s);
       dec_ca_block(xc, D, L.n2.w, L.n2.b, 1e-5f, L.ca_q.w, L.ca_q.b, L.ca_out.w, L.ca_out.b, d.ckv + (long)l * 2 * D, ldkv,
-                   Mtok, B, Ns, T, s);
+                   Mtok, B, Ns, T, 0, s);
       ff_block_384(xc, D, L.n3.w, L.n3.b, 1e-5f, L.ff1.w, L.ff1.b, L.ff2.w, L.ff2.b, xc, D, (int)R, s);
     }
     head_ddpm(xc, final_ln_.w, final_ln_.b, head_w_, head_b_, R, mode, x_io, noise, eps, cf, s);
```

After: 70.10 (median of 6 runs). 1.4% lower.
